# kaistmm/Audio-Mamba-AuM

Hardware: AMD Instinct MI355X
Metric: clips/sec/node AuM-Base 128x1024 fwd+bwd (higher is better)
Workload: dtype bf16; 1 GPU; AuM-Base (d_model=768, 24 Fo-Bi blocks, d_state=16, 92.1M params) 128-mel x 1024-frame clips, L=513 tokens, fwd+bwd+Adam, bf16 autocast / fp32 master weights, input = 160000-sample waveforms through the one-launch HIP frontend (log-mel + 16x16 patch embedding + position rows); per_gpu_batch=64, global_batch=64, parallelism=dp1

## Files before the change

### audio-mamba-aum_amd/aum/model.py

```python
import math

import torch
import torch.nn as nn
import torch.nn.functional as F

from mamba_ssm.modules.mamba_simple import Mamba
from mamba_ssm.ops.selective_scan_interface import _autocast_dtype, step_cache
from mamba_ssm.ops.triton.layernorm import RMSNorm, rms_norm_fn

AUM_SIZES = {"base": 768, "small": 384, "tiny": 192}


class PatchEmbed(nn.Module):

    def __init__(self, patch_size, strides, in_chans, embed_dim):
        super().__init__()
        self.proj = nn.Conv2d(in_chans, embed_dim, kernel_size=patch_size, stride=strides)
        fan_in = in_chans * patch_size[0] * patch_size[1]
        nn.init.trunc_normal_(self.proj.weight, std=math.sqrt(1.0 / fan_in) / 0.87962566103423978)
        nn.init.zeros_(self.proj.bias)

    def forward(self, x):
        Bsz, C, Fd, Td = x.shape
        ph, pw = self.proj.kernel_size
        nf, nt = Fd // ph, Td // pw
        cols = x[:, :, :nf * ph, :nt * pw].reshape(Bsz, C, nf, ph, nt, pw).permute(0, 2, 4, 1, 3, 5)
        cols = cols.reshape(Bsz * nf * nt, C * ph * pw)
        out = F.linear(cols, self.proj.weight.reshape(self.proj.out_channels, -1), self.proj.bias)
        return out.reshape(Bsz, nf * nt, -1)


class FrontendTokensFn(torch.autograd.Function):

    @staticmethod
    def forward(ctx, wave, weight, bias, pos_embed, cls_token, fe, dtype, cls_pos, time_major):
        import aum_hip
        Dm = weight.shape[0]
        w16 = weight.detach().reshape(Dm, -1).to(dtype).contiguous()
        pe = pos_embed.detach().float()
        cls_row = (cls_token.detach().float() + pe[:, :1]).reshape(Dm).contiguous()
        need = any(ctx.needs_input_grad[1:5])
        tokens, patches = aum_hip.frontend_tokens(
            wave, fe.tables.tables, fe.target_length, fe.norm_mean, fe.norm_std, w16, bias.detach().float().contiguous(),
            pe[0, 1:].contiguous(), cls_row, cls_pos, time_major=time_major, save_patches=need, aug=fe.aug, noise=fe.noise)
        ctx.save_for_backward(patches)
        ctx.cfg = (weight.shape, weight.dtype, dtype, cls_pos, time_major, fe.target_length // 16)
        return tokens

    @staticmethod
    def backward(ctx, g):
        (patches,) = ctx.saved_tensors
        wshape, wdtype, dtype, cls_pos, time_major, nt = ctx.cfg
        Bsz, _, Dm = g.shape
        gp = torch.cat((g[:, :cls_pos], g[:, cls_pos + 1:]), dim=1)
        if time_major:
            gp = gp.reshape(Bsz, nt, -1, Dm).transpose(1, 2).reshape(Bsz, -1, Dm)
        g16 = gp.to(dtype).reshape(-1, Dm)
        import aum_hip
        if g16.is_cuda and aum_hip.gemm_wgrad_supported(g16, patches):
            dweight = aum_hip.gemm_wgrad(g16, patches).to(wdtype).reshape(wshape)
        else:
            dweight = (g16.t() @ patches).to(wdtype).reshape(wshape)
        dbias = g16.sum(0).to(wdtype)
        dcls = g[:, cls_pos].sum(0)
        dpos = torch.cat((dcls[None], gp.sum(0)), dim=0)[None]
        return None, dweight, dbias, dpos.to(wdtype), dcls.reshape(1, 1, Dm).to(wdtype), None, None, None, None


class PosEmbed(nn.Module):

    def __init__(self, n_tokens, embed_dim):
        super().__init__()
        self.pos_embed = nn.Parameter(torch.zeros(1, n_tokens, embed_dim))
        nn.init.trunc_normal_(self.pos_embed, std=0.02)


class Block(nn.Module):

    def __init__(self, dim, mixer, eps):
        super().__init__()
        self.mixer = mixer
        self.norm = RMSNorm(dim, eps=eps)

    def forward(self, hidden_states, residual=None, inference_params=None, *, time_reversed=False):
        hidden_states, residual = rms_norm_fn(hidden_states, self.norm.weight, self.norm.bias, residual=residual,
                                              prenorm=True, residual_in_fp32=True, eps=self.norm.eps)
        if time_reversed:
            return self.mixer(hidden_states, inference_params=inference_params, time_reversed=True), residual
        return self.mixer(hidden_states, inference_params=inference_params), residual


class ParkedSessions:
    WAVE_KEYS = ("tail_len", "samples", "frames", "ended")

    def __init__(self, blob, columns, wave, signature):
        self.blob, self.columns, self.wave, self.signature = blob, list(columns), wave, tuple(signature)

    def __len__(self):
        return len(self.columns)

    def select(self, idx):
        idx = [int(i) for i in idx]
        if not idx or min(idx) < -len(self) or max(idx) >= len(self):
            raise IndexError(f"ParkedSessions.select: {idx} of {len(self)} sessions")
        idx = [i % len(self) for i in idx]
        if len(set(idx)) == 1:
            blob = self.blob[idx[0]:idx[0] + 1].expand(len(idx), -1)
        else:
            blob = self.blob.index_select(0, torch.tensor(idx, dtype=torch.int64).to(self.blob.device))
        wave = None if self.wave is None else {k: [v[i] for i in idx] for k, v in self.wave.items()}
        return ParkedSessions(blob, [self.columns[i] for i in idx], wave, self.signature)

    def __getitem__(self, i):
        return self.select([i])


class StreamStack:
    MAX_TOTAL = 512

    def __init__(self, model, dtype):
        import aum_hip
        self.dtype, self.depth = dtype, len(model.layers)
        self.sources = [(d, n, p, None if p is None else (p._version, p.dtype, p.device)) for d, n, p in model._stack_sources()]
        self.gens = [(layer.mixer.__dict__, layer.mixer.__dict__.get("_stream_gen", 0)) for layer in model.layers]
        m0 = model.layers[0].mixer
        self.d_model, self.dim, self.eps = m0.d_model, m0.d_inner, model.layers[0].norm.eps
        self.plans, self.keep, recs = [], [], []
        for layer in model.layers:
            mx = layer.mixer
            plan = mx.stream_params(dtype)
            w_in = aum_hip._al16(mx.in_proj.weight.detach().to(dtype).contiguous())
            w_out = aum_hip._al16(mx.out_proj.weight.detach().to(dtype).contiguous())
            nw = aum_hip._al16(aum_hip._f32c(layer.norm.weight))
            self.plans.append(plan)
            self.keep.append((w_in, w_out, nw))
            recs.append({"norm_weight": nw, "w_in": w_in, "conv_weight": plan.conv_w, "conv_bias": plan.conv_b, "wx": plan.w_x, "wdt": plan.w_dt,
                         "A": plan.A, "D": plan.D, "delta_bias": plan.dt_bias, "w_out": w_out, "conv_state": None, "state": None})
        p0 = self.plans[0]
        self.rank, self.ncols, self.ldwx, self.ldwdt = p0.w_dt.shape[1], p0.w_x.shape[0], p0.w_x.stride(0), p0.w_dt.stride(0)
        self.table = aum_hip.stream_layers_table(recs)
        self.records_ok = aum_hip.stream_layers_records_ok(self.table, self.depth)
        self.workspace = None

    def fresh(self):
        for d, n, p, sig in self.sources:
            q = d.get(n)
            if q is not p or (p is not None and (p._version, p.dtype, p.device) != sig):
                return False
        return all(d.get("_stream_gen", 0) == g for d, g in self.gens)

    def takes(self, total, max_len):
        import aum_hip
        return 1 <= max_len <= aum_hip.STREAM_BLOCK_MAX_T and 1 <= total <= self.MAX_TOTAL

    def pools_ok(self, layer_caches):
        if len(layer_caches) != self.depth:
            return False
        n = layer_caches[0][0].shape[0]
        return all(c.dtype == torch.float32 and s.dtype == torch.float32 and c.is_contiguous() and s.is_contiguous()
                   and tuple(c.shape) == (n, self.dim, 4) and tuple(s.shape) == (n, self.dim, 16) and c.data_ptr() % 16 == 0 and s.data_ptr() % 16 == 0
                   for c, s in (layer_caches[i] for i in range(self.depth)))

    def run(self, rows, layer_caches, smap, commit=True, peek=False):
        import aum_hip
        rows = rows.to(self.dtype).contiguous()
        for i in range(self.depth):
            self.table[i].conv_state, self.table[i].state = layer_caches[i][0].data_ptr(), layer_caches[i][1].data_ptr()
        need = aum_hip.stream_layers_scratch_layout(rows.shape[0], self.d_model, self.dim, self.ncols)[2]
        if self.workspace is None or self.workspace.numel() < need or self.workspace.device != rows.device:
            self.workspace = torch.empty(need, dtype=torch.uint8, device=rows.device)
        return aum_hip.stream_layers(rows, self.table, self.depth, layer_caches[0][0], smap, dim=self.dim, rank=self.rank, ncols=self.ncols,
                                     ldwx=self.ldwx, ldwdt=self.ldwdt, eps=self.eps, commit=commit, peek=peek, workspace=self.workspace,
                                     records_ok=self.records_ok)


class AudioMamba(nn.Module):
    def __init__(self, spectrogram_size=(128, 1024), patch_size=(16, 16), strides=(16, 16), depth=24, embed_dim=768,
                 channels=1, num_classes=527, norm_epsilon=1e-5, bimamba_type="v1", if_devide_out=True,
                 use_middle_cls_token=True, use_end_cls_token=False, transpose_token_sequence=False,
                 if_bidirectional=False, ssm_cfg=None, device=None, dtype=None, imagenet_pretrain=False,
                 imagenet_pretrain_path=None, imagenet_pretrain_modelkey="model", imagenet_load_middle_cls_token=True,
                 imagenet_load_double_cls_token=False, **unsupported):
        super().__init__()
        on = {k: v for k, v in unsupported.items() if v not in (None, False, 0, 0.0, -1.0)
              and k not in ("if_cls_token", "rms_norm", "fused_add_norm", "residual_in_fp32", "if_abs_pos_embed", "final_pool_type",
                            "use_PI_for_patch_embed")}
        if imagenet_load_double_cls_token:
            on["imagenet_load_double_cls_token"] = imagenet_load_double_cls_token
        if on:
            raise NotImplementedError(f"AudioMamba options outside the accelerated path: {sorted(on)}")
        if tuple(patch_size) != tuple(strides):
            raise NotImplementedError("overlapping patches are off the default path")
        self.embed_dim = self.d_model = embed_dim
        self.num_classes = num_classes
        self.use_middle_cls_token = use_middle_cls_token
        self.use_end_cls_token = use_end_cls_token
        self.transpose_token_sequence = transpose_token_sequence
        self.if_bidirectional = if_bidirectional
        if if_bidirectional and depth % 2:
            raise ValueError("if_bidirectional pairs the layers: depth must be even")
        fdim = (spectrogram_size[0] - patch_size[0]) // strides[0] + 1
        tdim = (spectrogram_size[1] - patch_size[1]) // strides[1] + 1
        self.patch_grid_size = (fdim, tdim)
        self.num_patches = fdim * tdim
        self.num_tokens = 1
        self.cls_token = nn.Parameter(torch.zeros(1, 1, embed_dim))
        self.head = nn.Linear(embed_dim, num_classes) if num_classes > 0 else nn.Identity()
        self.layers = nn.ModuleList([
            Block(embed_dim, Mamba(embed_dim, layer_idx=i, bimamba_type=bimamba_type, if_devide_out=if_devide_out,
                                   **(ssm_cfg or {})), norm_epsilon)
            for i in range(depth)])
        self.norm_f = RMSNorm(embed_dim, eps=norm_epsilon)
        if isinstance(self.head, nn.Linear):
            nn.init.trunc_normal_(self.head.weight, std=0.02)
            nn.init.zeros_(self.head.bias)
        nn.init.trunc_normal_(self.cls_token, std=0.02)
        self.apply(lambda m: _init_weights(m, depth))
        self.patch_embed = PatchEmbed(tuple(patch_size), tuple(strides), channels, embed_dim)
        self.pos_embed = PosEmbed(self.num_patches + self.num_tokens, embed_dim)
        if imagenet_pretrain:
            from .checkpoint import load_imagenet_checkpoint
            print(load_imagenet_checkpoint(self, imagenet_pretrain_path, imagenet_pretrain_modelkey,
                                           imagenet_load_middle_cls_token, imagenet_load_double_cls_token))
        if device is not None or dtype is not None:
            self.to(device=device, dtype=dtype)

    def no_weight_decay(self):
        return {"pos_embed", "cls_token"}

    def tokens(self, x):
        x = x.unsqueeze(1).transpose(2, 3)
        x = self.patch_embed(x)
        Bsz, Np, _ = x.shape
        pe = self.pos_embed.pos_embed
        pos = Np // 2 if self.use_middle_cls_token else (Np if self.use_end_cls_token else 0)
        cls = (self.cls_token + pe[:, :1]).expand(Bsz, -1, -1)
        x = x + pe[:, 1:]
        if self.transpose_token_sequence:
            nf, nt = self.patch_grid_size
            x = x.reshape(Bsz, nf, nt, -1).transpose(1, 2).reshape(Bsz, nt * nf, -1)
        return torch.cat((x[:, :pos], cls.to(x.dtype), x[:, pos:]), dim=1), pos

    def tokens_from_wave(self, wave, fe):
        import aum_hip
        dtype = torch.get_autocast_dtype(wave.device.type) if torch.is_autocast_enabled(wave.device.type) else None
        ps = self.patch_embed.proj
        if (dtype is None or tuple(ps.kernel_size) != (16, 16) or ps.in_channels != 1 or self.patch_grid_size[0] != 8
                or self.patch_grid_size[1] * 16 != fe.target_length
                or not aum_hip.frontend_tokens_supported(fe.tables.tables, fe.target_length, self.embed_dim, dtype)):
            return self.tokens(fe.spectrogram(wave))
        Np = self.num_patches
        pos = Np // 2 if self.use_middle_cls_token else (Np if self.use_end_cls_token else 0)
        tok = FrontendTokensFn.apply(wave, ps.weight, ps.bias, self.pos_embed.pos_embed, self.cls_token, fe, dtype, pos,
                                     self.transpose_token_sequence)
        return tok, pos

    def forward_features(self, x, frontend=None):
        hidden, pos = self.tokens(x) if frontend is None else self.tokens_from_wave(x, frontend)
        with step_cache([layer.mixer for layer in self.layers], _autocast_dtype()):
            hidden, residual = self._run_layers(hidden)
        return rms_norm_fn(hidden[:, pos], self.norm_f.weight, self.norm_f.bias, eps=self.norm_f.eps,
                           residual=None if residual is None else residual[:, pos], prenorm=False, residual_in_fp32=True)

    def _run_layers(self, hidden):
        residual = None
        if not self.if_bidirectional:
            for layer in self.layers:
                hidden, residual = layer(hidden, residual)
        else:
            for i in range(len(self.layers) // 2):
                hf, rf = self.layers[2 * i](hidden, residual)
                hb, rb = self.layers[2 * i + 1](hidden, residual, time_reversed=True)
                hidden, residual = hf + hb, rf + rb
        return hidden, residual

    def _check_streamable(self):
        bt = self.layers[0].mixer.bimamba_type if len(self.layers) else "none"
        if bt != "none":
            raise ValueError(f"streaming inference needs bimamba_type='none' (causal blocks), not {bt!r}")
        if self.if_bidirectional:
            raise ValueError("streaming inference needs if_bidirectional=False")
        if self.use_middle_cls_token:
            raise ValueError("streaming inference needs use_middle_cls_token=False (the cls token must close the sequence)")
        if not self.use_end_cls_token:
            raise ValueError("streaming inference needs use_end_cls_token=True (the cls token must close the sequence)")
        if not self.transpose_token_sequence:
            raise ValueError("streaming inference needs transpose_token_sequence=True (time-major token order)")

    def allocate_inference_cache(self, batch_size, max_seqlen=0, dtype=None, **kwargs):
        self._check_streamable()
        dtype = torch.float32 if dtype is None else dtype
        return {"layers": {i: layer.mixer.allocate_inference_cache(batch_size, max_seqlen, dtype=dtype, **kwargs)
                           for i, layer in enumerate(self.layers)},
                "columns": 0, "batch": batch_size}

    def _stack_sources(self):
        out = []
        for layer in self.layers:
            mx = layer.mixer
            for mod, names in ((mx, ("A_log", "D")), (mx.conv1d, ("weight", "bias")), (mx.x_proj, ("weight",)), (mx.dt_proj, ("weight", "bias")),
                               (mx.in_proj, ("weight", "bias")), (mx.out_proj, ("weight", "bias")), (layer.norm, ("weight", "bias"))):
                out += [(mod._parameters, n, mod._parameters.get(n)) for n in names]
        return out

    @torch.no_grad()
    def stream_stack(self, dtype=None):
        import aum_hip
        hit = self.__dict__.get("_stream_stack")
        if hit is not None and (dtype is None or dtype == hit.dtype) and hit.fresh() and (
                dtype is not None or hit.dtype == self.layers[0].mixer.in_proj.weight.dtype):
            return hit
        self._check_streamable()
        if not len(self.layers):
            raise ValueError("stream_stack: the model has no blocks")
        dtype = self.layers[0].mixer.in_proj.weight.dtype if dtype is None else dtype
        if dtype not in (torch.bfloat16, torch.float16):
            raise ValueError(f"stream_stack: the projection kernels run in bf16 or fp16, not {dtype}")
        for i, layer in enumerate(self.layers):
            mx = layer.mixer
            if mx.in_proj.bias is not None or mx.out_proj.bias is not None:
                raise ValueError(f"stream_stack: block {i} has projection biases (bias=True); the projection kernels add none")
            if getattr(layer.norm, "bias", None) is not None:
                raise ValueError(f"stream_stack: block {i}'s norm has a bias")
            if mx.d_conv != 4 or mx.d_state != 16:
                raise ValueError(f"stream_stack: block {i} has d_conv {mx.d_conv}, d_state {mx.d_state}; the middle kernel is built for 4 and 16")
            if (mx.d_model, mx.d_inner) not in aum_hip.STREAM_STACK_WIDTHS:
                raise ValueError(f"stream_stack: block {i} has widths ({mx.d_model}, {mx.d_inner}); the kernels are built for {aum_hip.STREAM_STACK_WIDTHS}")
            if layer.norm.eps != self.layers[0].norm.eps:
                raise ValueError("stream_stack: the blocks' norms differ in eps")
        stack = StreamStack(self, dtype)
        if not aum_hip.xdt_fwd_shape_ok(stack.ncols, stack.dim) or stack.rank % 8 or stack.rank + 32 > stack.ncols:
            raise ValueError(f"stream_stack: dt_rank {self.layers[0].mixer.dt_rank} gives x/dt rows of {stack.ncols} columns, which the middle kernel does not take")
        self.__dict__["_stream_stack"] = stack
        return stack

    def _stack_for(self, stack, hidden, layer_caches, seq_map, prefill, peek_every):
        if stack is None or prefill or peek_every is not None:
            return None
        if not isinstance(stack, StreamStack):
            raise TypeError("stack= takes what AudioMamba.stream_stack() returns")
        stack = self.stream_stack(stack.dtype)
        total = hidden.shape[0] * hidden.shape[1]
        max_len = hidden.shape[1] if seq_map is None else max(seq_map.lens)
        return stack if stack.takes(total, max_len) and stack.pools_ok(layer_caches) else None

    def _stream_layers(self, hidden, layer_caches, seq_map=None, commit=True, peek=False, prefill=False, peek_every=None, stack=None):
        st = self._stack_for(stack, hidden, layer_caches, seq_map, prefill, peek_every)
        if st is not None:
            return self._run_stack(st, hidden, layer_caches, seq_map, commit, peek)
        residual = None
        for i, layer in enumerate(self.layers):
            hidden, residual = rms_norm_fn(hidden, layer.norm.weight, layer.norm.bias, residual=residual, prenorm=True,
                                           residual_in_fp32=True, eps=layer.norm.eps)
            conv_state, ssm_state = layer_caches[i]
            if prefill:
                hidden, _, _ = (layer.mixer.prefill_chunk(hidden, conv_state, ssm_state) if seq_map is None else
                                layer.mixer.prefill_chunk(hidden, conv_state, ssm_state, seq_map=seq_map))
            else:
                hidden, _, _ = layer.mixer.step_chunk(hidden, conv_state, ssm_state, seq_map=seq_map, commit=commit, peek=peek,
                                                      **({} if peek_every is None else {"peek_every": peek_every}))
        return hidden, residual

    @staticmethod
    def _run_stack(st, hidden, layer_caches, seq_map, commit, peek):
        import aum_hip
        batch, T, Dm = hidden.shape
        if seq_map is not None:
            aum_hip.check_seq_map("stream_layers", seq_map, T, layer_caches[0][0].shape[0], hidden.device)
        smap = seq_map if seq_map is not None else aum_hip.fixed_seq_map(batch, T, hidden.device)
        h, r = st.run(hidden.reshape(batch * T, Dm), layer_caches, smap, commit=commit, peek=peek)
        return h.view(batch, T, Dm), r.view(batch, T, Dm)

    def _read_in_place(self, cls, cache, rows):
        import aum_hip
        n = cls.shape[0]
        if cls.device.type != "cuda" or not aum_hip.debug.stream_fused:
            return None
        smap = aum_hip.fixed_seq_map(n, 1, cls.device) if rows is None else aum_hip.seq_map((1,) * n, rows, device=cls.device)
        try:
            hidden, residual = self._stream_layers(cls.reshape(1, n, -1), cache["layers"], smap, commit=False)
        except NotImplementedError:
            return None
        return hidden.reshape(n, 1, -1), residual.reshape(n, 1, -1)

    def allocate_stream_pool(self, sessions, dtype=None):
        if int(sessions) < 1:
            raise ValueError("allocate_stream_pool: at least one session")
        pool = self.allocate_inference_cache(int(sessions), dtype=dtype)
        pool["columns"] = [0] * int(sessions)
        return pool

    @staticmethod
    def _is_pool(cache):
        return isinstance(cache["columns"], list)

    def _check_sessions(self, what, cache, sessions, writes=True):
        if writes and not self._is_pool(cache):
            raise ValueError(f"{what} takes a pool from allocate_stream_pool")
        rows = [int(r) for r in sessions]
        if writes and len(set(rows)) != len(rows):
            raise ValueError(f"{what}: the sessions {rows} are not distinct")
        if rows and (min(rows) < 0 or max(rows) >= cache["batch"]):
            raise ValueError(f"{what}: the sessions {rows} are not all rows of a cache of {cache['batch']}")
        return rows

    def _embed_columns(self, spec4d, cols):
        nf, nt = self.patch_grid_size
        x = self.patch_embed(spec4d)
        Bsz, k = x.shape[0], x.shape[1] // nf
        pe = self.pos_embed.pos_embed[:, 1:].reshape(1, nf, nt, -1)
        pe = pe[:, :, cols] if isinstance(cols, slice) else pe.index_select(2, cols)
        return (x.reshape(Bsz, nf, k, -1) + pe).transpose(1, 2).reshape(Bsz, k * nf, -1)

    def _cls_row(self):
        return self.cls_token + self.pos_embed.pos_embed[:, :1]

    def _head_rows(self, hidden, residual, return_features):
        f = rms_norm_fn(hidden, self.norm_f.weight, self.norm_f.bias, eps=self.norm_f.eps, residual=residual, prenorm=False,
                        residual_in_fp32=True)
        return f if return_features else self.head(f)

# ... 435 lines not shown
```

### audio-mamba-aum_amd/aum_hip/__init__.py

```python
import ctypes as C
import math
import os
import typing

import torch

_HERE = os.path.dirname(os.path.abspath(__file__))
_SO = os.path.join(_HERE, "libaum_hip.so")

AUM_F32, AUM_BF16, AUM_F16 = 0, 1, 2
SCAN_SOFTPLUS, SCAN_REVERSE, SCAN_GENERIC, SCAN_ROWPAIR, SCAN_ACCUMULATE = 1, 2, 4, 8, 16
SCAN_DELTA_ACTIVATED = 32
XDT_DELTA_SOFTPLUS = 1
CONV_SILU, CONV_REVERSE = 1, 2
_DT = {torch.float32: AUM_F32, torch.bfloat16: AUM_BF16, torch.float16: AUM_F16}
_ERR = {-1: "AUM_E_NULL", -2: "AUM_E_SHAPE", -3: "AUM_E_DTYPE", -4: "AUM_E_UNSUPPORTED", -5: "AUM_E_WORKSPACE",
        -6: "AUM_E_LAUNCH"}

_i64, _i32, _u32, _vp, _fp = C.c_int64, C.c_int32, C.c_uint32, C.c_void_p, C.c_void_p
ABI_VERSION = 13


class _Debug:

# ... 145 lines not shown


SUM_MAX_JOBS = 8


class SumJob(C.Structure):
    _fields_ = [("src", C.c_void_p), ("dst", C.c_void_p), ("outer", C.c_int64), ("inner", C.c_int64), ("tr_cols", C.c_int32), ("reserved", C.c_int32)]


class ConvUpdateArgs(C.Structure):
    _fields_ = [("x", C.c_void_p), ("conv_state", C.c_void_p), ("weight", C.c_void_p), ("bias", C.c_void_p), ("out", C.c_void_p),
                ("batch", C.c_int32), ("dim", C.c_int32), ("width", C.c_int32), ("dtype", C.c_int32), ("flags", C.c_uint32)]


class StateUpdateArgs(C.Structure):
    _fields_ = [("state", C.c_void_p), ("x", C.c_void_p), ("dt", C.c_void_p), ("z", C.c_void_p), ("B", C.c_void_p), ("C", C.c_void_p),
                ("A", C.c_void_p), ("D", C.c_void_p), ("dt_bias", C.c_void_p), ("out", C.c_void_p),
                ("batch", C.c_int32), ("dim", C.c_int32), ("dstate", C.c_int32), ("dtype", C.c_int32), ("flags", C.c_uint32)]


class ConvTmChunkArgs(C.Structure):
    _fields_ = ([(n, _vp) for n in ("x", "conv_state", "weight", "bias", "y")] + [(n, _i64) for n in ("x_bs", "x_ts", "y_bs", "y_ts")]
                + [(n, _i32) for n in ("batch", "dim", "len", "width", "dtype")] + [("flags", _u32)])


class ScanTmChunkArgs(C.Structure):
    _fields_ = ([(n, _vp) for n in ("u", "delta", "z", "B", "C", "A", "D", "delta_bias", "state", "out")]
                + [(n, _i64) for n in ("u_bs", "u_ts", "delta_bs", "delta_ts", "z_bs", "z_ts", "B_bs", "B_ts", "C_bs", "C_ts", "out_bs", "out_ts")]
                + [(n, _i32) for n in ("batch", "dim", "len", "dstate", "dtype")] + [("flags", _u32)])


class ConvTmChunkVarArgs(C.Structure):
    _fields_ = ([(n, _vp) for n in ("x", "conv_state", "weight", "bias", "y", "cu_seqlens", "state_indices")] + [(n, _i64) for n in ("x_ts", "y_ts")]
                + [(n, _i32) for n in ("total", "nseq", "nrows", "dim", "width", "dtype")] + [("flags", _u32)])


class ScanTmChunkVarArgs(C.Structure):
    _fields_ = ([(n, _vp) for n in ("u", "delta", "z", "B", "C", "A", "D", "delta_bias", "state", "out", "cu_seqlens", "state_indices")]
                + [(n, _i64) for n in ("u_ts", "delta_ts", "z_ts", "B_ts", "C_ts", "out_ts")]
                + [(n, _i32) for n in ("total", "nseq", "nrows", "dim", "dstate", "dtype")] + [("flags", _u32)])


class ConvTmChunkPeeksArgs(C.Structure):
    _fields_ = [("base", ConvTmChunkVarArgs), ("peek_every", _i32), ("reserved", _i32)]


class ScanTmChunkPeeksArgs(C.Structure):
    _fields_ = [("base", ScanTmChunkVarArgs), ("peek_every", _i32), ("reserved", _i32)]


class ScanTmPeeksFwdArgs(C.Structure):
    _fields_ = [("base", ScanTmChunkVarArgs), ("ckpt", _vp), ("ckpt_bytes", _i64), ("peek_every", _i32), ("reserved", _i32)]


class ScanTmPeeksBwdArgs(C.Structure):
    _fields_ = ([("base", ScanTmChunkVarArgs)] + [(n, _vp) for n in ("ckpt", "du", "ddelta", "dz", "workspace")]
                + [(n, _i64) for n in ("ckpt_bytes", "workspace_bytes", "du_ts", "ddelta_ts", "dz_ts")] + [("peek_every", _i32), ("reserved", _i32)])


class ConvTmPeeksBwdArgs(C.Structure):
    _fields_ = ([(n, _vp) for n in ("x", "dy", "weight", "bias", "dx", "workspace", "cu_seqlens")]
                + [(n, _i64) for n in ("workspace_bytes", "x_ts", "dy_ts", "dx_ts")]
                + [(n, _i32) for n in ("total", "nseq", "dim", "width", "dtype")] + [("flags", _u32), ("peek_every", _i32), ("reserved", _i32)])


class ConvTmPrefillVarArgs(C.Structure):
    _fields_ = ([(n, _vp) for n in ("x", "conv_state", "weight", "bias", "y", "cu_seqlens", "state_indices")] + [(n, _i64) for n in ("x_ts", "y_ts")]
                + [(n, _i32) for n in ("total", "nseq", "nrows", "dim", "width", "dtype")] + [("flags", _u32), ("max_len", _i32)])


class ScanTmFwdStateVarArgs(C.Structure):
    _fields_ = ([(n, _vp) for n in ("u", "delta", "z", "B", "C", "A", "D", "delta_bias", "state", "out", "cu_seqlens", "state_indices")]
                + [(n, _i64) for n in ("u_ts", "delta_ts", "z_ts", "B_ts", "C_ts", "out_ts")]
                + [(n, _i32) for n in ("total", "nseq", "nrows", "dim", "dstate", "dtype")] + [("flags", _u32)]
                + [(n, _i32) for n in ("range_len", "max_len", "reserved")] + [("carry", _vp), ("carry_bytes", _i64)])


class StreamBlockArgs(C.Structure):
    _fields_ = ([(n, _vp) for n in ("x", "z", "conv_state", "state", "conv_weight", "conv_bias", "wx", "wdt", "A", "D", "delta_bias", "y", "scratch",
                                    "cu_seqlens", "state_indices")]
                + [(n, _i64) for n in ("x_ts", "z_ts", "y_ts", "scratch_bytes")]
                + [(n, _i32) for n in ("total", "nseq", "nrows", "max_len", "dim", "width", "dstate", "rank", "ncols", "ldwx", "ldwdt", "dtype")]
                + [("flags", _u32)])


class DtProjArgs(C.Structure):
    _fields_ = ([(n, _vp) for n in ("x", "w", "out")] + [("ntok", _i64)] + [(n, _i32) for n in ("dim", "rank", "ldx", "ldw", "ldo", "dtype")])


class XdtArgs(C.Structure):
    _fields_ = ([(n, _vp) for n in ("u", "wx", "wdt", "x_dbl", "delta")] + [("ntok", _i64)]
                + [(n, _i32) for n in ("dim", "rank", "ncols", "ldu", "ldwx", "ldwdt", "ldx", "ldd", "dtype")]
                + [("delta_bias", _vp), ("flags", _u32)])


PARK_MAX_TENSORS = 64
PARK_RESTORE = 1


class ParkArgs(C.Structure):
    _fields_ = ([("base", _vp * PARK_MAX_TENSORS)] + [(n, _i64 * PARK_MAX_TENSORS) for n in ("row_stride", "row_bytes", "blob_off")]
                + [("rows", _vp), ("blob", _vp), ("blob_stride", _i64), ("n_tensors", _i32), ("n_sessions", _i32), ("flags", _u32)])


class StreamInArgs(C.Structure):
    _fields_ = ([(n, _vp) for n in ("hidden", "residual_in", "norm_weight", "w_in", "residual_out", "xz")] + [("hidden_ts", _i64), ("xz_ts", _i64)]
                + [(n, _i32) for n in ("total", "d_model", "dim", "ldw", "dtype")] + [("eps", C.c_float)])


class StreamOutArgs(C.Structure):
    _fields_ = ([(n, _vp) for n in ("y", "w_out", "out")] + [("y_ts", _i64), ("out_ts", _i64)]
                + [(n, _i32) for n in ("total", "d_model", "dim", "ldw", "dtype", "reserved")])


STREAM_LAYER_POINTERS = ("norm_weight", "w_in", "conv_weight", "conv_bias", "wx", "wdt", "A", "D", "delta_bias", "w_out", "conv_state", "state")


class StreamLayer(C.Structure):
    _fields_ = [(n, _vp) for n in STREAM_LAYER_POINTERS]


class StreamLayersArgs(C.Structure):
    _fields_ = ([(n, _vp) for n in ("layers", "hidden", "residual_in", "hidden_out", "residual_out", "workspace", "cu_seqlens", "state_indices")]
                + [("hidden_ts", _i64), ("workspace_bytes", _i64)]
                + [(n, _i32) for n in ("depth", "total", "nseq", "nrows", "max_len", "d_model", "dim", "rank", "ncols", "ldwx", "ldwdt", "dtype")]
                + [("flags", _u32), ("eps", C.c_float)])


_SIGNATURES = {name: ([_vp, _vp], C.c_int) for name in (
    "aum_selective_scan_fwd", "aum_selective_scan_bwd", "aum_causal_conv1d_fwd", "aum_causal_conv1d_bwd", "aum_rmsnorm_fwd", "aum_rmsnorm_bwd",
    "aum_fbank_fwd", "aum_frontend_tokens_fwd", "aum_stft_logmel_fwd", "aum_spec_time_warp", "aum_proj_fwd", "aum_proj_bwd_data",
    "aum_proj_bwd_weight", "aum_scan_tm_fwd", "aum_scan_tm_bwd", "aum_scan_tm_seg_fwd", "aum_scan_tm_seg_bwd", "aum_conv1d_tm_fwd",
    "aum_conv1d_tm_bwd", "aum_gemm_tn", "aum_gemm_wgrad", "aum_dtproj_tm_fwd", "aum_xdt_tm_fwd", "aum_xdt_tm_bwd", "aum_causal_conv1d_update",
    "aum_selective_state_update", "aum_conv1d_tm_chunk", "aum_scan_tm_chunk", "aum_conv1d_tm_chunk_var", "aum_scan_tm_chunk_var", "aum_stream_block_tm", "aum_scan_tm_fwd_state",
    "aum_conv1d_tm_prefill_var", "aum_scan_tm_fwd_state_var", "aum_conv1d_tm_chunk_peeks", "aum_scan_tm_chunk_peeks", "aum_fbank_stream_fwd",
    "aum_scan_tm_peeks_fwd_ckpt", "aum_scan_tm_peeks_bwd", "aum_conv1d_tm_peeks_bwd", "aum_stream_park", "aum_stream_in_tm", "aum_stream_out_tm",
    "aum_stream_layers")}
_SIGNATURES.update({
    "aum_abi_version": ([], C.c_int), "aum_scan_max_single_pass_len": ([], C.c_int),
    "aum_selective_scan_workspace_bytes": ([_i32] * 6, _i64), "aum_selective_scan_ckpt_bytes": ([_i32] * 4, _i64),
    "aum_selective_scan_lane_ckpt_bytes": ([_i32] * 5, _i64), "aum_scan_tm_workspace_bytes": ([_i32] * 5, _i64),
    "aum_scan_tm_seg_carry_bytes": ([_i32] * 6, _i64), "aum_scan_tm_seg_workspace_bytes": ([_i32] * 6, _i64),
    "aum_rmsnorm_bwd_partials": ([_i32], C.c_int), "aum_rmsnorm_bwd_partial_rows": ([_i32, _i32, _u32], C.c_int),
    "aum_scan_tm_nck": ([_i32], _i32), "aum_scan_tm_ckpt_rows": ([_i32], _i32), "aum_conv1d_tm_nparts": ([_i32, _i32], _i32),
    "aum_proj_bwd_weight_splits": ([_i32, _i64], C.c_int), "aum_hbm_copy": ([_vp, _vp, _i64, _vp], C.c_int),
    "aum_selftest_wave_scan": ([_vp, _vp, C.c_int, _vp], C.c_int), "aum_selftest_wave_sum32": ([_vp, _vp, _vp], C.c_int),
    "aum_sum_rows": ([_vp, _vp, _i64, _i64, _i64, _i32, _vp], C.c_int), "aum_sum_rows_multi": ([_vp, _i32, _vp], C.c_int),
    "aum_cast_bank": ([_vp, _i32, _i32, _i32, _vp, _vp, _i32, _vp], C.c_int),
    "aum_stream_block_scratch_bytes": ([_i32] * 3, _i64), "aum_stream_block_max_len": ([], _i32),
    "aum_scan_tm_fwd_state_var_carry_bytes": ([_i32] * 4, _i64),
    "aum_scan_tm_peeks_ckpt_bytes": ([_i32] * 4, _i64), "aum_scan_tm_peeks_bwd_workspace_bytes": ([_i32] * 4, _i64),
    "aum_conv1d_tm_peeks_bwd_workspace_bytes": ([_i32] * 3, _i64),
    "aum_stream_layers_scratch_bytes": ([_i32] * 4, _i64),
})
EXPORTS = list(_SIGNATURES)


class Lib:

    def __init__(self, path, host=False):
        if not os.path.exists(path):
            raise ImportError(
                f"{path} not found: the HIP extension is not built.  Run `python audio-mamba-aum_amd/csrc/build.py` "
                "(hipcc, gfx950).  There is no CPU fallback on the product path.")
        self.path, self.host = path, host
        self.c = C.CDLL(path)
        for name, (argtypes, restype) in _SIGNATURES.items():
            fn = getattr(self.c, name)
            fn.argtypes, fn.restype = argtypes, restype
        if self.c.aum_abi_version() != ABI_VERSION:
            raise RuntimeError(f"{path}: ABI version {self.c.aum_abi_version()}, this binding speaks {ABI_VERSION} -- rebuild the library "
                               "(python audio-mamba-aum_amd/csrc/build.py)")
        self.max_single_pass_len = int(self.c.aum_scan_max_single_pass_len())

    def stream(self, t):
        if self.host:
            return None
        return C.c_void_p(torch.cuda.current_stream(t.device).cuda_stream)

    def check_tensor(self, t):
        if t is None:
            return
        if self.host:
            if t.device.type != "cpu":
                raise RuntimeError("lane-array (test) library takes host tensors")
        elif t.device.type != "cuda":
            raise RuntimeError("libaum_hip.so needs device (HIP) tensors; there is no CPU path in the product library")


_product = None


def get():
    global _product
    if _product is None:
        so = _SO
        if os.environ.get("AUM_DEBUG") == "1" and os.environ.get("AUM_HIP_LIB"):
            so = os.environ["AUM_HIP_LIB"]
        _product = Lib(so, host=False)
    return _product


def _chk(rc, what):
    if rc != 0:
        raise RuntimeError(f"{what} failed: {_ERR.get(rc, rc)}")


class LaunchTimer:

    def __init__(self):
        self.enabled = False
        self.only = None
        self.every = 1
        self.records = {}
        self.seen = {}

    def reset(self):
        self.records = {}
        self.seen = {}

    def want(self, name):
        n = self.seen.get(name, 0)
        self.seen[name] = n + 1
        return n % self.every == 0

    def summary(self):
        torch.cuda.synchronize()
        out = {}
        for name, evs in self.records.items():
            ms = [a.elapsed_time(b) for a, b, _ in evs]
            out[name] = {"launches": len(ms), "avg_ms": sum(ms) / max(len(ms), 1), "meta": evs[-1][2] if evs else None}
        return out


timer = LaunchTimer()


def C_byref(s):
    return C.cast(C.byref(s), C.c_void_p)


def _launch(fn, args, stream_tensor, lib, name, meta=None):
    if timer.enabled and not lib.host and (timer.only is None or name in timer.only) and timer.want(name):
        a, b = torch.cuda.Event(enable_timing=True), torch.cuda.Event(enable_timing=True)
        a.record()
        rc = fn(C_byref(args), lib.stream(stream_tensor))
        b.record()
        timer.records.setdefault(name, []).append((a, b, meta))
    else:
        rc = fn(C_byref(args), lib.stream(stream_tensor))
    _chk(rc, name)


def _ptr(t):
    return None if t is None else t.data_ptr()


def _unit(t, name):
    if t is not None and t.stride(-1) != 1 and t.shape[-1] != 1:
        raise RuntimeError(f"{name}: the time axis must be unit-stride (SSI:19-30)")


def _f32c(t):
    return None if t is None else t.detach().to(torch.float32).contiguous()


def _bc3(t):
    if t.dim() == 4:
        if t.shape[1] != 1:
            raise RuntimeError("only one B/C group is supported (G=1), as used by Mamba (SSI:473-493)")
        t = t[:, 0]
    return t


def _alloc(batch, dim, length, dtype, device, dmajor):
    if dmajor:
        return torch.empty((dim, batch, length), dtype=dtype, device=device).permute(1, 0, 2)
    return torch.empty((batch, dim, length), dtype=dtype, device=device)


def scan_ckpt(u, dstate, lib=None):
    lib = lib or get()
    batch, dim, length = u.shape
    if debug.rowpair or debug.no_ckpt:
        return None
    if lib.c.aum_selective_scan_ckpt_bytes(batch, dim, length, dstate) <= 0:
        return None
    return torch.empty((batch, dim, length // 512, dstate), dtype=torch.float32, device=u.device)


def scan_lane_ckpt(u, dstate, bidir, lib=None):
    lib = lib or get()
    batch, dim, length = u.shape
    if debug.rowpair or debug.no_lane_ckpt:
        return None
    if lib.c.aum_selective_scan_lane_ckpt_bytes(batch, dim, length, dstate, int(bool(bidir))) <= 0:
        return None
    return torch.empty((batch, dim, 2 if bidir else 1, dstate, 64), dtype=torch.float32, device=u.device)


def scan_accumulates(u, dstate, lib=None):
    lib = lib or get()
    batch, dim, length = u.shape
    if debug.rowpair or debug.no_accumulate:
        return False
    return lib.c.aum_selective_scan_ckpt_bytes(batch, dim, length, dstate) > 0
# ... 53 lines not shown
    B, C = _bc3(B), _bc3(C)
    for n, t in (("u", u), ("delta", delta), ("z", z), ("B", B), ("C", C), ("dout", dout), ("out_pre", out_pre)):
        _unit(t, n)
        lib.check_tensor(t)
    batch, dim, length = u.shape
    dstate = A.shape[1]
    dev = u.device
    A, A_b, D, delta_bias = _f32c(A), _f32c(A_b), _f32c(D), _f32c(delta_bias)
    acc = accumulate_into
    du = acc["du"] if acc else _alloc(batch, dim, length, u.dtype, dev, dmajor)
    ddelta = acc["ddelta"] if acc else _alloc(batch, dim, length, u.dtype, dev, dmajor)
    dz = None
    if z is not None:
        dz = acc["dz"] if acc else dz_out if dz_out is not None else _alloc(batch, dim, length, u.dtype, dev, dmajor)
        _unit(dz, "dz")
    f32 = dict(dtype=torch.float32, device=dev)
    nA, nBC = dim * dstate, batch * dstate * length
    sizes = [nA, nA if A_b is not None else 0, dim if D is not None and not acc else 0,
             dim if delta_bias is not None and not acc else 0, 0 if acc else nBC, 0 if acc else nBC]
    zbuf = torch.zeros((sum(sizes),), **f32)
    parts = torch.split(zbuf, sizes)
    dA = parts[0].view(dim, dstate)
    dA_b = parts[1].view(dim, dstate) if A_b is not None else None
    dD = parts[2] if D is not None else None
    dbias = parts[3] if delta_bias is not None else None
    dB = parts[4].view(batch, dstate, length) if not acc else None
    dC = parts[5].view(batch, dstate, length) if not acc else None
    if acc:
        assert A_b is None
        dB, dC, dD, dbias = acc["dB"], acc["dC"], acc["dD"], acc["ddelta_bias"]
    ws_bytes = int(lib.c.aum_selective_scan_workspace_bytes(batch, dim, length, dstate, int(A_b is not None), 1))
    ws = torch.empty((max(ws_bytes, 4) // 4,), **f32) if ws_bytes else None
    a = ScanBwdArgs()
    a.u, a.delta, a.z, a.B, a.C, a.dout, a.out_pre = map(_ptr, (u, delta, z, B, C, dout, out_pre))
    a.A, a.A_b, a.D, a.delta_bias = _ptr(A), _ptr(A_b), _ptr(D), _ptr(delta_bias)
    a.du, a.ddelta, a.dz = _ptr(du), _ptr(ddelta), _ptr(dz)
    a.dA, a.dA_b, a.dB, a.dC, a.dD, a.ddelta_bias = map(_ptr, (dA, dA_b, dB, dC, dD, dbias))
    a.workspace, a.workspace_bytes = _ptr(ws), ws_bytes
    if x_ck is not None:
        assert x_ck.dtype == torch.float32 and x_ck.is_contiguous() and x_ck.shape == (batch, dim, length // 512, dstate)
        a.x_ck = _ptr(x_ck)
    if x_lane is not None:
        assert x_lane.dtype == torch.float32 and x_lane.is_contiguous() and x_lane.shape == (batch, dim, 2 if A_b is not None else 1, dstate, 64)
        lib.check_tensor(x_lane)
        a.x_lane = _ptr(x_lane)
    a.u_bs, a.u_ds = u.stride(0), u.stride(1)
    a.delta_bs, a.delta_ds = delta.stride(0), delta.stride(1)
    if z is not None:
        a.z_bs, a.z_ds = z.stride(0), z.stride(1)
        a.out_bs, a.out_ds = out_pre.stride(0), out_pre.stride(1)
        a.dz_bs, a.dz_ds = dz.stride(0), dz.stride(1)
    a.B_bs, a.B_ns, a.C_bs, a.C_ns = B.stride(0), B.stride(1), C.stride(0), C.stride(1)
    a.dout_bs, a.dout_ds = dout.stride(0), dout.stride(1)
    a.du_bs, a.du_ds = du.stride(0), du.stride(1)
    a.ddelta_bs, a.ddelta_ds = ddelta.stride(0), ddelta.stride(1)
    a.dB_bs, a.dB_ns, a.dC_bs, a.dC_ns = dB.stride(0), dB.stride(1), dC.stride(0), dC.stride(1)
    a.batch, a.dim, a.len, a.dstate, a.dtype = batch, dim, length, dstate, _DT[u.dtype]
    a.flags = ((SCAN_SOFTPLUS if delta_softplus else 0) | (SCAN_REVERSE if reverse else 0) | (SCAN_GENERIC if generic else 0)
               | (SCAN_ROWPAIR if rowpair or debug.rowpair else 0)
               | (SCAN_ACCUMULATE if acc else 0)
               | (debug.ablate << 16))
    _launch(lib.c.aum_selective_scan_bwd, a, u, lib, "scan_bwd_bidir" if A_b is not None else "scan_bwd",
            (batch, dim, length, dstate, u.element_size(), True))
    return dict(du=du, ddelta=ddelta, dA=dA, dA_b=dA_b, dB=dB, dC=dC, dD=dD, dz=dz, ddelta_bias=dbias)


SCAN_TM_CK = 8


def scan_tm_supported(dim, dstate):
    return dstate == 16 and dim % 64 == 0


def _tm3(t, name, last):
    if t.dim() != 3 or t.shape[2] != last or (t.stride(2) != 1 and last != 1):
        raise RuntimeError(f"{name}: expected (batch, len, {last}) with the last axis contiguous (token-major)")
    ts = t.stride(1) if t.shape[1] > 1 else last
    bs = t.stride(0) if t.shape[0] > 1 else ts * t.shape[1]
    return bs, ts


def scan_tm_ckpt(batch, length, dim, dstate, bidir, device, lib=None, dtype=torch.float32):
    lib = lib or get()
    nck = int(lib.c.aum_scan_tm_nck(length))
    rows = int(lib.c.aum_scan_tm_ckpt_rows(_DT[dtype])) if dstate == 16 else dstate
    return torch.empty((2 if bidir else 1, batch, max(nck, 1), rows, dim), dtype=torch.float32, device=device)


SCAN_TM_MAX_SEGMENTS = 32


def scan_tm_segments(batch, dim, length, bidir, training=False, nsimd=None, device=None):
    nsimd = 4 * cu_count(device) if nsimd is None else nsimd
    per_dir = batch * (dim // 64)
    waves = per_dir * (2 if bidir else 1)
    if per_dir <= 0 or waves * 2 > nsimd or length < 1024:
        return 1
    want = -(-nsimd * 3 // per_dir)
    seg = min(want, length // 128, SCAN_TM_MAX_SEGMENTS)
    return seg if seg >= 2 else 1


def scan_tm_fwd(u, delta, A, B, C, D=None, z=None, delta_bias=None, delta_softplus=False, reverse=False, A_b=None,
                want_out_pre=False, ckpt=None, out=None, lib=None, segments=1, delta_activated=False):
    lib = lib or get()
    batch, length, dim = u.shape
    dstate = A.shape[1]
    for t in (u, delta, z, B, C):
        lib.check_tensor(t)
    if u.dtype not in _DT or delta.dtype != u.dtype or (z is not None and z.dtype != u.dtype):
        raise RuntimeError("u, delta, z must share one dtype in {fp32, bf16, fp16}")
    if B.dtype != u.dtype or C.dtype != u.dtype:
        raise RuntimeError("B, C must have u's dtype")
    A, A_b, D, delta_bias = _f32c(A), _f32c(A_b), _f32c(D), _f32c(delta_bias)
    a = ScanTmFwdArgs()
    a.u_bs, a.u_ts = _tm3(u, "u", dim)
    a.delta_bs, a.delta_ts = _tm3(delta, "delta", dim)
    if z is not None:
        a.z_bs, a.z_ts = _tm3(z, "z", dim)
    a.B_bs, a.B_ts = _tm3(B, "B", dstate)
    a.C_bs, a.C_ts = _tm3(C, "C", dstate)
    if out is None:
        out = torch.empty((batch, length, dim), dtype=u.dtype, device=u.device)
    out_pre = torch.empty((batch, length, dim), dtype=u.dtype, device=u.device) if want_out_pre else None
    a.out_bs, a.out_ts = _tm3(out, "out", dim)
    if out_pre is not None:
        a.pre_bs, a.pre_ts = _tm3(out_pre, "out_pre", dim)
    a.u, a.delta, a.z, a.B, a.C = _ptr(u), _ptr(delta), _ptr(z), _ptr(B), _ptr(C)
    a.A, a.A_b, a.D, a.delta_bias = _ptr(A), _ptr(A_b), _ptr(D), _ptr(delta_bias)
    a.out, a.out_pre = _ptr(out), _ptr(out_pre)
    if ckpt is not None:
        assert ckpt.dtype == torch.float32 and ckpt.is_contiguous()
        rows = int(lib.c.aum_scan_tm_ckpt_rows(_DT[u.dtype])) if dstate == 16 else dstate
        assert ckpt.numel() >= (2 if A_b is not None else 1) * batch * max(int(lib.c.aum_scan_tm_nck(length)), 1) * rows * dim, "ckpt too small"
        lib.check_tensor(ckpt)
        a.ckpt = _ptr(ckpt)
    a.batch, a.dim, a.len, a.dstate, a.dtype = batch, dim, length, dstate, _DT[u.dtype]
    a.flags = (SCAN_SOFTPLUS if delta_softplus else 0) | (SCAN_REVERSE if reverse else 0) | (SCAN_DELTA_ACTIVATED if delta_activated else 0)
    if segments > 1:
        sa = ScanTmSegFwdArgs()
        sa.base = a
        sa.segments = int(segments)
        sa.carry_bytes = int(lib.c.aum_scan_tm_seg_carry_bytes(batch, dim, length, dstate, int(A_b is not None), int(segments)))
        if sa.carry_bytes <= 0:
            raise RuntimeError(f"scan_tm_fwd: segments={segments} not supported for this shape")
        carry = torch.empty((sa.carry_bytes // 4,), dtype=torch.float32, device=u.device)
        sa.carry = _ptr(carry)
        _launch(lib.c.aum_scan_tm_seg_fwd, sa, u, lib, "scan_tm_seg_fwd_bidir" if A_b is not None else "scan_tm_seg_fwd",
                (batch, dim, length, dstate, u.element_size(), want_out_pre, int(segments)))
        return out, out_pre
    _launch(lib.c.aum_scan_tm_fwd, a, u, lib, "scan_tm_fwd_bidir" if A_b is not None else "scan_tm_fwd",
            (batch, dim, length, dstate, u.element_size(), want_out_pre))
    return out, out_pre


def scan_state_supported(t, batch, dim, dstate):
    return t is None or (t.dim() == 3 and tuple(t.shape) == (batch, dim, dstate) and t.dtype == torch.float32 and t.is_contiguous()
                         and t.data_ptr() % 16 == 0)


def scan_tm_fwd_state_supported(u, delta, A, B, C, D=None, z=None, delta_bias=None, delta_softplus=False, delta_activated=False,
                                state_in=None, state_out=None, segments=1):
    if u.dim() != 3 or A.dim() != 2 or u.shape[1] < 1 or not scan_tm_supported(u.shape[2], A.shape[1]) or u.dtype not in _DT:
        return False
    batch, length, dim = u.shape
    dstate, es = A.shape[1], u.element_size()
    if not (1 <= int(segments) <= SCAN_TM_MAX_SEGMENTS) or A.shape[0] != dim:
        return False
    for t, last in ((u, dim), (delta, dim), (z, dim), (B, dstate), (C, dstate)):
        if t is None:
            continue
        if t.dtype != u.dtype or t.dim() != 3 or tuple(t.shape) != (batch, length, last) or (t.stride(2) != 1 and last != 1):
            return False
        bs, ts = _tm3(t, "operand", last)
        if last == dim and (t.data_ptr() % 16 or (ts * es) % 16 or (bs * es) % 16):
            return False
        if last == dstate and es == 2 and (t.data_ptr() % 4 or ts % 2 or bs % 2):
            return False
        if ts < 0 or ts * es * length >= 2 ** 31:
            return False
    if delta_activated and (es == 4 or z is None):
        return False
    return scan_state_supported(state_in, batch, dim, dstate) and scan_state_supported(state_out, batch, dim, dstate)


def scan_tm_fwd_state(u, delta, A, B, C, D=None, z=None, delta_bias=None, delta_softplus=False, delta_activated=False, state_in=None,
                      state_out=None, segments=1, out=None, lib=None):
    lib = lib or get()
    for t in (u, delta, z, B, C, state_in, state_out, out):
        lib.check_tensor(t)
    if not scan_tm_fwd_state_supported(u, delta, A, B, C, D, z, delta_bias, delta_softplus, delta_activated, state_in, state_out, segments):
        raise RuntimeError(f"scan_tm_fwd_state: unsupported operands u {tuple(u.shape)} {u.dtype} strides {u.stride()}, A {tuple(A.shape)}, state_in "
                           f"{None if state_in is None else (tuple(state_in.shape), state_in.dtype)}, state_out "
                           f"{None if state_out is None else (tuple(state_out.shape), state_out.dtype)}, segments {segments} "
                           "(need token-major 16-byte rows of one dtype, dim % 64 == 0, dstate 16, fp32 contiguous (batch, dim, 16) states)")
    batch, length, dim = u.shape
    dstate = A.shape[1]
    A, D, delta_bias = _f32c(A), _f32c(D), _f32c(delta_bias)
    for t in (A, D, delta_bias):
        lib.check_tensor(t)
    if out is None:
        out = torch.empty((batch, length, dim), dtype=u.dtype, device=u.device)
    if out.dtype != u.dtype or tuple(out.shape) != (batch, length, dim):
        raise RuntimeError("scan_tm_fwd_state: out must have u's shape and dtype")
    sa = ScanTmFwdStateArgs()
    a = sa.base
    a.u_bs, a.u_ts = _tm3(u, "u", dim)
    a.delta_bs, a.delta_ts = _tm3(delta, "delta", dim)
    if z is not None:
        a.z_bs, a.z_ts = _tm3(z, "z", dim)
    a.B_bs, a.B_ts = _tm3(B, "B", dstate)
    a.C_bs, a.C_ts = _tm3(C, "C", dstate)
    a.out_bs, a.out_ts = _tm3(out, "out", dim)
    a.u, a.delta, a.z, a.B, a.C = _ptr(u), _ptr(delta), _ptr(z), _ptr(B), _ptr(C)
    a.A, a.D, a.delta_bias, a.out = _ptr(A), _ptr(D), _ptr(delta_bias), _ptr(out)
    a.batch, a.dim, a.len, a.dstate, a.dtype = batch, dim, length, dstate, _DT[u.dtype]
    a.flags = (SCAN_SOFTPLUS if delta_softplus else 0) | (SCAN_DELTA_ACTIVATED if delta_activated else 0)
    sa.state_in, sa.state_out, sa.segments = _ptr(state_in), _ptr(state_out), int(segments)
    carry = None
    if segments > 1:
        sa.carry_bytes = int(lib.c.aum_scan_tm_seg_carry_bytes(batch, dim, length, dstate, 0, int(segments)))
        carry = torch.empty((sa.carry_bytes // 4,), dtype=torch.float32, device=u.device)
        sa.carry = _ptr(carry)
    _launch(lib.c.aum_scan_tm_fwd_state, sa, u, lib, "scan_tm_fwd_state", (batch, dim, length, dstate, u.element_size(), int(segments)))
    return out


def scan_tm_bwd(u, delta, A, B, C, D, z, delta_bias, dout, out_pre, ckpt, delta_softplus=False, reverse=False, A_b=None, dz_out=None,
                lib=None, segments=1, want_dA_xA=False, param_out=None, delta_activated=False):
    lib = lib or get()
    batch, length, dim = u.shape
    dstate = A.shape[1]
    dev = u.device
    for t in (u, delta, z, B, C, dout, out_pre, ckpt):
        lib.check_tensor(t)
    if u.dtype not in _DT:
        raise RuntimeError("u must be fp32, bf16 or fp16")
    for name, t in (("delta", delta), ("z", z), ("B", B), ("C", C), ("dout", dout), ("out_pre", out_pre), ("dz_out", dz_out)):
        if t is not None and t.dtype != u.dtype:
            raise RuntimeError(f"{name} must have u's dtype ({u.dtype}), got {t.dtype}")
    for name, t in (("delta", delta), ("z", z), ("dout", dout), ("out_pre", out_pre), ("dz_out", dz_out)):
        if t is not None and tuple(t.shape) != (batch, length, dim):
            raise RuntimeError(f"{name}: expected shape {(batch, length, dim)}, got {tuple(t.shape)}")
    if z is not None and out_pre is None:
        raise RuntimeError("out_pre (the forward's pre-gate sum) is required when z is given")
    A, A_b, D, delta_bias = _f32c(A), _f32c(A_b), _f32c(D), _f32c(delta_bias)
    bidir = A_b is not None
    if ckpt is None or ckpt.dtype != torch.float32 or not ckpt.is_contiguous():
        raise RuntimeError("ckpt: the contiguous fp32 tensor scan_tm_fwd filled")
    rows_ = int(lib.c.aum_scan_tm_ckpt_rows(_DT[u.dtype])) if dstate == 16 else dstate
    if ckpt.numel() < (2 if bidir else 1) * batch * max(int(lib.c.aum_scan_tm_nck(length)), 1) * rows_ * dim:
        raise RuntimeError("ckpt too small for this launch")
    du = torch.empty((batch, length, dim), dtype=u.dtype, device=dev)
    ddelta = torch.empty((batch, length, dim), dtype=u.dtype, device=dev)
    dz = None
    if z is not None:
        dz = dz_out if dz_out is not None else torch.empty((batch, length, dim), dtype=u.dtype, device=dev)
    f32 = dict(dtype=torch.float32, device=dev)
    dBC = torch.empty((batch, length, 2 * dstate), **f32)
    po = param_out or {}
    dA = torch.empty((dim, dstate), **f32)
    dA_b = torch.empty((dim, dstate), **f32) if bidir else None
    dD = _sum_out(po.get("dD"), (dim,), dev) if D is not None else None
    dbias = _sum_out(po.get("ddelta_bias"), (dim,), dev) if delta_bias is not None else None
    dA_xA = _sum_out(po.get("dA_xA"), (dim, dstate), dev) if want_dA_xA else None
    dA_b_xA = _sum_out(po.get("dA_b_xA"), (dim, dstate), dev) if want_dA_xA and bidir else None
    if segments > 1:
        ws_bytes = int(lib.c.aum_scan_tm_seg_workspace_bytes(batch, dim, length, dstate, int(bidir), int(segments)))
        if ws_bytes <= 0:
            raise RuntimeError(f"scan_tm_bwd: segments={segments} not supported for this shape")
    else:
        ws_bytes = int(lib.c.aum_scan_tm_workspace_bytes(batch, dim, length, dstate, int(bidir)))
    ws = torch.empty((max(ws_bytes, 4) // 4,), **f32)
    a = ScanTmBwdArgs()
    a.u, a.delta, a.z, a.B, a.C, a.dout, a.out_pre = map(_ptr, (u, delta, z, B, C, dout, out_pre))
    a.A, a.A_b, a.D, a.delta_bias, a.ckpt = _ptr(A), _ptr(A_b), _ptr(D), _ptr(delta_bias), _ptr(ckpt)
    a.du, a.ddelta, a.dz = _ptr(du), _ptr(ddelta), _ptr(dz)
    a.dA, a.dA_b, a.dBC, a.dD, a.ddelta_bias = map(_ptr, (dA, dA_b, dBC, dD, dbias))
    a.dA_xA, a.dA_b_xA = _ptr(dA_xA), _ptr(dA_b_xA)
    a.workspace, a.workspace_bytes = _ptr(ws), ws_bytes
    a.u_bs, a.u_ts = _tm3(u, "u", dim)
    a.delta_bs, a.delta_ts = _tm3(delta, "delta", dim)
    a.B_bs, a.B_ts = _tm3(B, "B", dstate)
    a.C_bs, a.C_ts = _tm3(C, "C", dstate)
    a.dout_bs, a.dout_ts = _tm3(dout, "dout", dim)
    a.du_bs, a.du_ts = _tm3(du, "du", dim)
    a.ddelta_bs, a.ddelta_ts = _tm3(ddelta, "ddelta", dim)
    if z is not None:
        a.z_bs, a.z_ts = _tm3(z, "z", dim)
        a.pre_bs, a.pre_ts = _tm3(out_pre, "out_pre", dim)
        a.dz_bs, a.dz_ts = _tm3(dz, "dz", dim)
    a.batch, a.dim, a.len, a.dstate, a.dtype = batch, dim, length, dstate, _DT[u.dtype]
    a.flags = (SCAN_SOFTPLUS if delta_softplus else 0) | (SCAN_REVERSE if reverse else 0) | (SCAN_DELTA_ACTIVATED if delta_activated else 0)
    if segments > 1:
        sa = ScanTmSegBwdArgs()
        sa.base = a
        sa.segments = int(segments)
        _launch(lib.c.aum_scan_tm_seg_bwd, sa, u, lib, "scan_tm_seg_bwd_bidir" if bidir else "scan_tm_seg_bwd",
                (batch, dim, length, dstate, u.element_size(), True, int(segments)))
    else:
        _launch(lib.c.aum_scan_tm_bwd, a, u, lib, "scan_tm_bwd_bidir" if bidir else "scan_tm_bwd", (batch, dim, length, dstate, u.element_size(), True))
    return dict(du=du, ddelta=ddelta, dz=dz, dBC=dBC, dA=dA, dA_b=dA_b, dD=dD, ddelta_bias=dbias, dA_xA=dA_xA, dA_b_xA=dA_b_xA, _ws=ws)


GEMM_BN, GEMM_BK = 256, 64

# ... 1773 lines not shown
```

### audio-mamba-aum_amd/csrc/aum_api_tm.inc

```
#include "scan_tm_kernels.h"
#include "conv_tm_kernels.h"
#include "stream_tm_kernels.h"
#include "stream_train_kernels.h"
#include "stream_block_kernels.h"
#include "stream_prefill_kernels.h"

namespace aum {

#ifndef AUM_SCANT_FWD_MINW
#define AUM_SCANT_FWD_MINW 3
#endif

int scan_tm_fwd_f32(const AumScanTmFwdArgs& a, aum_stream_t s);
int scan_tm_fwd_bf16(const AumScanTmFwdArgs& a, aum_stream_t s);
int scan_tm_fwd_f16(const AumScanTmFwdArgs& a, aum_stream_t s);
int scan_tm_bwd_f32(const AumScanTmBwdArgs& a, const ScanTBwdOut& wo, aum_stream_t s);
int scan_tm_bwd_bf16(const AumScanTmBwdArgs& a, const ScanTBwdOut& wo, aum_stream_t s);
int scan_tm_bwd_f16(const AumScanTmBwdArgs& a, const ScanTBwdOut& wo, aum_stream_t s);
int scan_tm_seg_fwd_f32(const AumScanTmFwdArgs& a, const ScanTSeg& sg, int phase, aum_stream_t s);
int scan_tm_seg_fwd_bf16(const AumScanTmFwdArgs& a, const ScanTSeg& sg, int phase, aum_stream_t s);
int scan_tm_seg_fwd_f16(const AumScanTmFwdArgs& a, const ScanTSeg& sg, int phase, aum_stream_t s);
int scan_tm_fwd_state_f32(const AumScanTmFwdArgs& a, const ScanTState& st, const ScanTSeg* sg, int phase, aum_stream_t s);
int scan_tm_fwd_state_bf16(const AumScanTmFwdArgs& a, const ScanTState& st, const ScanTSeg* sg, int phase, aum_stream_t s);
int scan_tm_fwd_state_f16(const AumScanTmFwdArgs& a, const ScanTState& st, const ScanTSeg* sg, int phase, aum_stream_t s);
int scan_tm_fwd_state_var_f32(const AumScanTmFwdArgs& a, const ScanTVar& v, const ScanTSeg* sg, int phase, aum_stream_t s);
int scan_tm_fwd_state_var_bf16(const AumScanTmFwdArgs& a, const ScanTVar& v, const ScanTSeg* sg, int phase, aum_stream_t s);
int scan_tm_fwd_state_var_f16(const AumScanTmFwdArgs& a, const ScanTVar& v, const ScanTSeg* sg, int phase, aum_stream_t s);
int scan_tm_seg_bwd_f32(const AumScanTmBwdArgs& a, const ScanTBwdOut& wo, const ScanTSeg& sg, int phase, aum_stream_t s);
int scan_tm_seg_bwd_bf16(const AumScanTmBwdArgs& a, const ScanTBwdOut& wo, const ScanTSeg& sg, int phase, aum_stream_t s);
int scan_tm_seg_bwd_f16(const AumScanTmBwdArgs& a, const ScanTBwdOut& wo, const ScanTSeg& sg, int phase, aum_stream_t s);

struct ScanTWs { int64_t dbc, dA, dD, dbias, carry, total, trace; int nparts, ndir; };
static ScanTWs scant_ws_layout(int batch, int dim, int len, int dstate, bool bidir, int nseg = 1) {
    ScanTWs w;
    w.ndir = bidir ? 2 : 1;
    w.nparts = dim / WAVE * w.ndir;
    w.dbc = 0;
    w.dA = w.dbc + (int64_t)batch * len * w.nparts * 2 * dstate;
    w.dD = w.dA + (int64_t)w.ndir * batch * nseg * dstate * dim;
    w.dbias = w.dD + (int64_t)w.ndir * batch * nseg * dim;
    w.carry = w.dbias + (int64_t)w.ndir * batch * nseg * dim;
    if (nseg > 1) w.total = w.carry + scant_seg_carry_floats(batch, dim, nseg, bidir);
    else w.total = w.carry + (bidir ? (int64_t)scant_bwd_wgs<true>(batch * (dim / WAVE)) * 2 * (2 * dstate + 2) * WAVE : 0);
    w.trace = 0;
#ifdef AUM_SCANT_TRACE
    w.trace = (w.total + 1) / 2 * 2;
    w.total = w.trace + (int64_t)(bidir ? scant_bwd_wgs<true>(batch * (dim / WAVE)) : scant_bwd_wgs<false>(batch * (dim / WAVE))) * SCANT_NW * 16 * 2;
#endif
    return w;
}

template <class T> using ScanTFwdLds = Lds<float, SCANT_NW * scant_lds_wave_floats<T>()>;
template <class T> using ScanTBwdLds = Lds<float, SCANT_NW * scant_bwd_lds_wave_floats<T>()>;
#if AUM_API_PART == 5 || AUM_API_PART == 0
#ifndef AUM_EMU
template <class T, bool SP, bool HAS_Z, bool HAS_PRE, bool BIDIR>
__global__ __launch_bounds__(SCANT_NW * 64, AUM_SCANT_FWD_MINW) void k_scant_fwd(AumScanTmFwdArgs a) {
    __shared__ __attribute__((aligned(16))) float lds[ScanTFwdLds<T>::n];
#ifdef AUM_SCANT_TRACE
    unsigned long long* tr = reinterpret_cast<unsigned long long*>(a.ckpt) + ((size_t)blockIdx.x * SCANT_NW + threadIdx.x / 64) * 12;
    const unsigned long long t_begin = __builtin_amdgcn_s_memrealtime();
    a.ckpt = nullptr;
    unsigned long long tacc[8] = {0, 0, 0, 0, 0, 0, 0, 0};
    scant_fwd<T, SP, HAS_Z, HAS_PRE, BIDIR>(a, (int)blockIdx.x, lds, tacc);
    if ((threadIdx.x & 63) == 0) {
        tr[0] = __builtin_amdgcn_s_getreg((31 << 11) | 4);
        tr[1] = __builtin_amdgcn_s_getreg((31 << 11) | 20);
        tr[2] = t_begin;
        tr[3] = __builtin_amdgcn_s_memrealtime();
        for (int k = 0; k < 8; ++k) tr[4 + k] = tacc[k];
    }
#else
    scant_fwd<T, SP, HAS_Z, HAS_PRE, BIDIR>(a, (int)blockIdx.x, lds);
#endif
}
#endif
template <class T, bool SP, bool HAS_Z, bool HAS_PRE, bool BIDIR> static int launch_scant_fwd(const AumScanTmFwdArgs& a, aum_stream_t s) {
    constexpr int UPW = scant_units_per_wg<BIDIR>();
    const int grid = (a.batch * (a.dim / WAVE) + UPW - 1) / UPW;
    return AUM_LAUNCH(grid, SCANT_NW * 64, s, (ScanTFwdLds<T>{}), (k_scant_fwd<T, SP, HAS_Z, HAS_PRE, BIDIR>), (scant_fwd<T, SP, HAS_Z, HAS_PRE, BIDIR>(a, wg, lds)), a);
}
template <class T> static int scan_tm_fwd_t(const AumScanTmFwdArgs& a, aum_stream_t s) {
    return with_bool((a.flags & AUM_SCAN_SOFTPLUS) != 0, [&](auto sp) { return with_bool(a.z != nullptr, [&](auto hz) {
        return with_bool(a.out_pre != nullptr, [&](auto pre) { return with_bool(a.A_b != nullptr, [&](auto bidir) {
            return launch_scant_fwd<T, sp, hz, pre, bidir>(a, s); }); }); }); });
}
#ifndef AUM_EMU
template <class T, int PHASE, bool SP, bool HAS_Z, bool HAS_PRE>
__global__ __launch_bounds__(SCANT_NW * 64, AUM_SCANT_FWD_MINW) void k_scant_seg_fwd(AumScanTmFwdArgs a, ScanTSeg sg) {
    __shared__ __attribute__((aligned(16))) float lds[ScanTFwdLds<T>::n];
    scant_seg_fwd<T, PHASE, SP, HAS_Z, HAS_PRE>(a, sg, (int)blockIdx.x, lds);
}
#endif
template <class T, int PHASE, bool SP, bool HAS_Z, bool HAS_PRE> static int launch_scant_seg_fwd(const AumScanTmFwdArgs& a, const ScanTSeg& sg, aum_stream_t s) {
    const int grid = (a.batch * (a.dim / WAVE) * sg.nseg * sg.ndl + SCANT_NW - 1) / SCANT_NW;
    return AUM_LAUNCH(grid, SCANT_NW * 64, s, (ScanTFwdLds<T>{}), (k_scant_seg_fwd<T, PHASE, SP, HAS_Z, HAS_PRE>), (scant_seg_fwd<T, PHASE, SP, HAS_Z, HAS_PRE>(a, sg, wg, lds)), a, sg);
}
template <class T> static int scan_tm_seg_fwd_t(const AumScanTmFwdArgs& a, const ScanTSeg& sg, int phase, aum_stream_t s) {
    return with_bool((a.flags & AUM_SCAN_SOFTPLUS) != 0, [&](auto sp) {
        if (phase == 3) return launch_scant_seg_fwd<T, 3, sp, false, false>(a, sg, s);
        return with_bool(a.z != nullptr, [&](auto hz) {
            if (phase == 4) return launch_scant_seg_fwd<T, 4, sp, hz, false>(a, sg, s);
            return with_bool(a.out_pre != nullptr, [&](auto pre) {
                return with_int<0, 1, 2>(phase, [&](auto ph) { return launch_scant_seg_fwd<T, ph, sp, hz, pre>(a, sg, s); }); });
        });
    });
}
#ifndef AUM_EMU
template <class T, bool SP, bool HAS_Z>
__global__ __launch_bounds__(SCANT_NW * 64, AUM_SCANT_FWD_MINW) void k_scant_fwd_state(AumScanTmFwdArgs a, ScanTState st) {
    __shared__ __attribute__((aligned(16))) float lds[ScanTFwdLds<T>::n];
    scant_fwd_state<T, SP, HAS_Z>(a, st, (int)blockIdx.x, lds);
}
template <class T, int PHASE, bool SP, bool HAS_Z>
__global__ __launch_bounds__(SCANT_NW * 64, AUM_SCANT_FWD_MINW) void k_scant_seg_fwd_state(AumScanTmFwdArgs a, ScanTSeg sg, ScanTState st) {
    __shared__ __attribute__((aligned(16))) float lds[ScanTFwdLds<T>::n];
    scant_seg_fwd_state<T, PHASE, SP, HAS_Z>(a, sg, st, (int)blockIdx.x, lds);
}
#endif
template <class T, bool SP, bool HAS_Z> static int launch_scant_fwd_state(const AumScanTmFwdArgs& a, const ScanTState& st, aum_stream_t s) {
    const int grid = (a.batch * (a.dim / WAVE) + SCANT_NW - 1) / SCANT_NW;
    return AUM_LAUNCH(grid, SCANT_NW * 64, s, (ScanTFwdLds<T>{}), (k_scant_fwd_state<T, SP, HAS_Z>), (scant_fwd_state<T, SP, HAS_Z>(a, st, wg, lds)), a, st);
}
template <class T, int PHASE, bool SP, bool HAS_Z>
static int launch_scant_seg_fwd_state(const AumScanTmFwdArgs& a, const ScanTSeg& sg, const ScanTState& st, aum_stream_t s) {
    const int grid = (a.batch * (a.dim / WAVE) * sg.nseg + SCANT_NW - 1) / SCANT_NW;
    return AUM_LAUNCH(grid, SCANT_NW * 64, s, (ScanTFwdLds<T>{}), (k_scant_seg_fwd_state<T, PHASE, SP, HAS_Z>), (scant_seg_fwd_state<T, PHASE, SP, HAS_Z>(a, sg, st, wg, lds)), a, sg, st);
}
template <class T> static int scan_tm_fwd_state_t(const AumScanTmFwdArgs& a, const ScanTState& st, const ScanTSeg* sg, int phase, aum_stream_t s) {
    if (sg && phase != 3 && phase != 0) return AUM_E_UNSUPPORTED;
    return with_bool((a.flags & AUM_SCAN_SOFTPLUS) != 0, [&](auto sp) {
        if (sg && phase == 3) return launch_scant_seg_fwd_state<T, 3, sp, false>(a, *sg, st, s);
        return with_bool(a.z != nullptr, [&](auto hz) {
            return sg ? launch_scant_seg_fwd_state<T, 0, sp, hz>(a, *sg, st, s) : launch_scant_fwd_state<T, sp, hz>(a, st, s);
        });
    });
}
#ifndef AUM_EMU
template <class T, bool SP, bool HAS_Z>
__global__ __launch_bounds__(SCANT_NW * 64, AUM_SCANT_FWD_MINW) void k_scant_fwd_state_var(AumScanTmFwdArgs a, ScanTVar v) {
    __shared__ __attribute__((aligned(16))) float lds[ScanTFwdLds<T>::n];
    scant_fwd_state_var<T, SP, HAS_Z>(a, v, (int)blockIdx.x, lds);
}
template <class T, int PHASE, bool SP, bool HAS_Z>
__global__ __launch_bounds__(SCANT_NW * 64, AUM_SCANT_FWD_MINW) void k_scant_seg_fwd_state_var(AumScanTmFwdArgs a, ScanTSeg sg, ScanTVar v) {
    __shared__ __attribute__((aligned(16))) float lds[ScanTFwdLds<T>::n];
    scant_seg_fwd_state_var<T, PHASE, SP, HAS_Z>(a, sg, v, (int)blockIdx.x, lds);
}
#endif
template <class T, bool SP, bool HAS_Z> static int launch_scant_fwd_state_var(const AumScanTmFwdArgs& a, const ScanTVar& v, aum_stream_t s) {
    const int grid = (v.nseq * (a.dim / WAVE) + SCANT_NW - 1) / SCANT_NW;
    return AUM_LAUNCH(grid, SCANT_NW * 64, s, (ScanTFwdLds<T>{}), (k_scant_fwd_state_var<T, SP, HAS_Z>), (scant_fwd_state_var<T, SP, HAS_Z>(a, v, wg, lds)), a, v);
}
template <class T, int PHASE, bool SP, bool HAS_Z>
static int launch_scant_seg_fwd_state_var(const AumScanTmFwdArgs& a, const ScanTSeg& sg, const ScanTVar& v, aum_stream_t s) {
    const int grid = (v.nseq * (a.dim / WAVE) * sg.nseg + SCANT_NW - 1) / SCANT_NW;
    return AUM_LAUNCH(grid, SCANT_NW * 64, s, (ScanTFwdLds<T>{}), (k_scant_seg_fwd_state_var<T, PHASE, SP, HAS_Z>), (scant_seg_fwd_state_var<T, PHASE, SP, HAS_Z>(a, sg, v, wg, lds)), a, sg, v);
}
template <class T> static int scan_tm_fwd_state_var_t(const AumScanTmFwdArgs& a, const ScanTVar& v, const ScanTSeg* sg, int phase, aum_stream_t s) {
    if (sg && phase != 3 && phase != 0) return AUM_E_UNSUPPORTED;
    return with_bool((a.flags & AUM_SCAN_SOFTPLUS) != 0, [&](auto sp) {
        if (sg && phase == 3) return launch_scant_seg_fwd_state_var<T, 3, sp, false>(a, *sg, v, s);
        return with_bool(a.z != nullptr, [&](auto hz) {
            return sg ? launch_scant_seg_fwd_state_var<T, 0, sp, hz>(a, *sg, v, s) : launch_scant_fwd_state_var<T, sp, hz>(a, v, s);
        });
    });
}
#if AUM_HAS_DTYPE(0)
int scan_tm_fwd_f32(const AumScanTmFwdArgs& a, aum_stream_t s) { return scan_tm_fwd_t<float>(a, s); }
int scan_tm_seg_fwd_f32(const AumScanTmFwdArgs& a, const ScanTSeg& sg, int phase, aum_stream_t s) { return scan_tm_seg_fwd_t<float>(a, sg, phase, s); }
int scan_tm_fwd_state_f32(const AumScanTmFwdArgs& a, const ScanTState& st, const ScanTSeg* sg, int phase, aum_stream_t s) { return scan_tm_fwd_state_t<float>(a, st, sg, phase, s); }
int scan_tm_fwd_state_var_f32(const AumScanTmFwdArgs& a, const ScanTVar& v, const ScanTSeg* sg, int phase, aum_stream_t s) { return scan_tm_fwd_state_var_t<float>(a, v, sg, phase, s); }
#endif
#if AUM_HAS_DTYPE(1)
int scan_tm_fwd_bf16(const AumScanTmFwdArgs& a, aum_stream_t s) { return scan_tm_fwd_t<bf16_t>(a, s); }
int scan_tm_seg_fwd_bf16(const AumScanTmFwdArgs& a, const ScanTSeg& sg, int phase, aum_stream_t s) { return scan_tm_seg_fwd_t<bf16_t>(a, sg, phase, s); }
int scan_tm_fwd_state_bf16(const AumScanTmFwdArgs& a, const ScanTState& st, const ScanTSeg* sg, int phase, aum_stream_t s) { return scan_tm_fwd_state_t<bf16_t>(a, st, sg, phase, s); }
int scan_tm_fwd_state_var_bf16(const AumScanTmFwdArgs& a, const ScanTVar& v, const ScanTSeg* sg, int phase, aum_stream_t s) { return scan_tm_fwd_state_var_t<bf16_t>(a, v, sg, phase, s); }
#endif
#if AUM_HAS_DTYPE(2)
int scan_tm_fwd_f16(const AumScanTmFwdArgs& a, aum_stream_t s) { return scan_tm_fwd_t<f16_t>(a, s); }
int scan_tm_seg_fwd_f16(const AumScanTmFwdArgs& a, const ScanTSeg& sg, int phase, aum_stream_t s) { return scan_tm_seg_fwd_t<f16_t>(a, sg, phase, s); }
int scan_tm_fwd_state_f16(const AumScanTmFwdArgs& a, const ScanTState& st, const ScanTSeg* sg, int phase, aum_stream_t s) { return scan_tm_fwd_state_t<f16_t>(a, st, sg, phase, s); }
int scan_tm_fwd_state_var_f16(const AumScanTmFwdArgs& a, const ScanTVar& v, const ScanTSeg* sg, int phase, aum_stream_t s) { return scan_tm_fwd_state_var_t<f16_t>(a, v, sg, phase, s); }
#endif
#endif

#ifndef AUM_SCANT_BWD_MINW
#define AUM_SCANT_BWD_MINW 2
#endif
#if AUM_API_PART == 6 || AUM_API_PART == 0
#ifndef AUM_EMU
template <class T, int SP, bool HAS_Z, bool BIDIR>
__global__ __launch_bounds__(SCANT_NW * 64, AUM_SCANT_BWD_MINW) void k_scant_bwd(AumScanTmBwdArgs a, ScanTBwdOut wo) {
    __shared__ __attribute__((aligned(16))) float lds[ScanTBwdLds<T>::n];
#ifdef AUM_SCANT_TRACE
    unsigned long long* tr = wo.trace + ((size_t)blockIdx.x * SCANT_NW + threadIdx.x / 64) * 16;
    const unsigned long long t_begin = __builtin_amdgcn_s_memrealtime();
    unsigned long long tacc[12] = {0, 0, 0, 0, 0, 0, 0, 0, 0, 0, 0, 0};
    scant_bwd<T, SP, HAS_Z, BIDIR>(a, wo, (int)blockIdx.x, lds, tacc);
    if ((threadIdx.x & 63) == 0) {
        tr[0] = __builtin_amdgcn_s_getreg((31 << 11) | 4);
        tr[1] = __builtin_amdgcn_s_getreg((31 << 11) | 20);
        tr[2] = t_begin;
        tr[3] = __builtin_amdgcn_s_memrealtime();
        for (int k = 0; k < 12; ++k) tr[4 + k] = tacc[k];
    }
#else
    scant_bwd<T, SP, HAS_Z, BIDIR>(a, wo, (int)blockIdx.x, lds);
#endif
}
#endif
template <class T, int SP, bool HAS_Z, bool BIDIR> static int launch_scant_bwd(const AumScanTmBwdArgs& a, const ScanTBwdOut& wo, aum_stream_t s) {
    const int grid = scant_bwd_wgs<BIDIR>(a.batch * (a.dim / WAVE));
    return AUM_LAUNCH(grid, SCANT_NW * 64, s, (ScanTBwdLds<T>{}), (k_scant_bwd<T, SP, HAS_Z, BIDIR>), (scant_bwd<T, SP, HAS_Z, BIDIR>(a, wo, wg, lds)), a, wo);
}
template <class T> static int scan_tm_bwd_t(const AumScanTmBwdArgs& a, const ScanTBwdOut& wo, aum_stream_t s) {
    if (a.flags & AUM_SCAN_DELTA_ACTIVATED) {
        if constexpr (sizeof(T) == 2)
            return with_bool(a.A_b != nullptr, [&](auto bidir) { return launch_scant_bwd<T, SCANT_SP_ACT, true, bidir>(a, wo, s); });
        return AUM_E_UNSUPPORTED;
    }
    return with_bool((a.flags & AUM_SCAN_SOFTPLUS) != 0, [&](auto sp) { return with_bool(a.z != nullptr, [&](auto hz) {
        return with_bool(a.A_b != nullptr, [&](auto bidir) { return launch_scant_bwd<T, sp ? SCANT_SP_IN : SCANT_SP_NONE, hz, bidir>(a, wo, s); }); }); });
}
#ifndef AUM_EMU
template <class T, int PHASE, int SP, bool HAS_Z>
__global__ __launch_bounds__(SCANT_NW * 64, AUM_SCANT_BWD_MINW) void k_scant_seg_bwd(AumScanTmBwdArgs a, ScanTBwdOut wo, ScanTSeg sg) {
    __shared__ __attribute__((aligned(16))) float lds[ScanTBwdLds<T>::n];
    scant_seg_bwd<T, PHASE, SP, HAS_Z>(a, wo, sg, (int)blockIdx.x, lds);
}
#endif
template <class T, int PHASE, int SP, bool HAS_Z>
static int launch_scant_seg_bwd(const AumScanTmBwdArgs& a, const ScanTBwdOut& wo, const ScanTSeg& sg, aum_stream_t s) {
    const int grid = (a.batch * (a.dim / WAVE) * sg.nseg + SCANT_NW - 1) / SCANT_NW;
    return AUM_LAUNCH(grid, SCANT_NW * 64, s, (ScanTBwdLds<T>{}), (k_scant_seg_bwd<T, PHASE, SP, HAS_Z>), (scant_seg_bwd<T, PHASE, SP, HAS_Z>(a, wo, sg, wg, lds)), a, wo, sg);
}
template <class T> static int scan_tm_seg_bwd_t(const AumScanTmBwdArgs& a, const ScanTBwdOut& wo, const ScanTSeg& sg, int phase, aum_stream_t s) {
    if (a.flags & AUM_SCAN_DELTA_ACTIVATED) {
        if constexpr (sizeof(T) == 2) return with_int<0, 1, 2>(phase, [&](auto ph) { return launch_scant_seg_bwd<T, ph, SCANT_SP_ACT, true>(a, wo, sg, s); });
        return AUM_E_UNSUPPORTED;
    }
    return with_bool((a.flags & AUM_SCAN_SOFTPLUS) != 0, [&](auto sp) { return with_bool(a.z != nullptr, [&](auto hz) {
        return with_int<0, 1, 2>(phase, [&](auto ph) { return launch_scant_seg_bwd<T, ph, sp ? SCANT_SP_IN : SCANT_SP_NONE, hz>(a, wo, sg, s); }); }); });
}
#if AUM_HAS_DTYPE(0)
int scan_tm_bwd_f32(const AumScanTmBwdArgs& a, const ScanTBwdOut& wo, aum_stream_t s) { return scan_tm_bwd_t<float>(a, wo, s); }
int scan_tm_seg_bwd_f32(const AumScanTmBwdArgs& a, const ScanTBwdOut& wo, const ScanTSeg& sg, int phase, aum_stream_t s) { return scan_tm_seg_bwd_t<float>(a, wo, sg, phase, s); }
#endif
#if AUM_HAS_DTYPE(1)
int scan_tm_bwd_bf16(const AumScanTmBwdArgs& a, const ScanTBwdOut& wo, aum_stream_t s) { return scan_tm_bwd_t<bf16_t>(a, wo, s); }
int scan_tm_seg_bwd_bf16(const AumScanTmBwdArgs& a, const ScanTBwdOut& wo, const ScanTSeg& sg, int phase, aum_stream_t s) { return scan_tm_seg_bwd_t<bf16_t>(a, wo, sg, phase, s); }
#endif
#if AUM_HAS_DTYPE(2)
int scan_tm_bwd_f16(const AumScanTmBwdArgs& a, const ScanTBwdOut& wo, aum_stream_t s) { return scan_tm_bwd_t<f16_t>(a, wo, s); }
int scan_tm_seg_bwd_f16(const AumScanTmBwdArgs& a, const ScanTBwdOut& wo, const ScanTSeg& sg, int phase, aum_stream_t s) { return scan_tm_seg_bwd_t<f16_t>(a, wo, sg, phase, s); }
#endif
#endif

}

#if AUM_API_PART == 3 || AUM_API_PART == 0
AUM_API int32_t aum_scan_tm_nck(int32_t len) { return len > 0 ? scant_nck(len) : 0; }
AUM_API int32_t aum_scan_tm_ckpt_rows(int32_t dtype) {
    return dtype == AUM_F32 ? scant_ck_rows<float>() : (dtype == AUM_BF16 || dtype == AUM_F16) ? scant_ck_rows<bf16_t>() : 0;
}

static bool scan_tm_act_ok(uint32_t flags, int32_t dtype, const void* z) { return !(flags & AUM_SCAN_DELTA_ACTIVATED) || (dtype != AUM_F32 && z); }
template <class A> static A scan_tm_fwd_resolve(const A& a) {
    A r = a;
    if (a.flags & AUM_SCAN_DELTA_ACTIVATED) {
        r.delta_bias = nullptr;
        r.flags &= ~(AUM_SCAN_SOFTPLUS | AUM_SCAN_DELTA_ACTIVATED);
    }
    return r;
}
static int scan_tm_fwd_check(const AumScanTmFwdArgs* a) {
    if (!a) return AUM_E_NULL;
    if (!a->u || !a->delta || !a->B || !a->C || !a->A || !a->out) return AUM_E_NULL;
    if (a->batch <= 0 || a->dim <= 0 || a->len <= 0 || a->dstate <= 0) return AUM_E_SHAPE;
    if (a->dtype < 0 || a->dtype > 2) return AUM_E_DTYPE;
    if (!scant_supported(a->dim, a->dstate)) return AUM_E_UNSUPPORTED;
    if (!scan_tm_act_ok(a->flags, a->dtype, a->z)) return AUM_E_UNSUPPORTED;
    if (a->A_b && (a->flags & AUM_SCAN_REVERSE)) return AUM_E_UNSUPPORTED;
    if (a->dtype != AUM_F32) {
        if ((a->B_bs | a->B_ts | a->C_bs | a->C_ts) & 1) return AUM_E_UNSUPPORTED;
        if ((((uintptr_t)a->B) | ((uintptr_t)a->C)) & 3) return AUM_E_UNSUPPORTED;
    }
    {
        const int64_t es = a->dtype == AUM_F32 ? 4 : 2, lim = ((int64_t)1 << 31) - 1;
        const int64_t ts[] = {a->u_ts, a->delta_ts, a->z ? a->z_ts : 0, a->out_ts, a->out_pre ? a->pre_ts : 0, a->B_ts, a->C_ts};
        for (int64_t t : ts)
            if (t < 0 || t * es * a->len > lim) return AUM_E_UNSUPPORTED;
        if ((int64_t)scant_nck(a->len) * a->dstate * a->dim * 4 > lim) return AUM_E_UNSUPPORTED;
        const uintptr_t ptrs = (uintptr_t)a->u | (uintptr_t)a->delta | (uintptr_t)a->z | (uintptr_t)a->out | (uintptr_t)a->out_pre;
        const int64_t strides = a->u_bs | a->u_ts | a->delta_bs | a->delta_ts | (a->z ? (a->z_bs | a->z_ts) : 0) | a->out_bs | a->out_ts |
                                (a->out_pre ? (a->pre_bs | a->pre_ts) : 0);
        if ((ptrs & 15) || ((strides * es) & 15)) return AUM_E_UNSUPPORTED;
    }
    return AUM_OK;
}
AUM_API int aum_scan_tm_fwd(const AumScanTmFwdArgs* a, void* stream) {
    const int rc = scan_tm_fwd_check(a);
    if (rc != AUM_OK) return rc;
    aum_stream_t s = (aum_stream_t)stream;
    const AumScanTmFwdArgs k = scan_tm_fwd_resolve(*a);
    return AUM_BY_DTYPE_X(k.dtype, scan_tm_fwd, k, s);
}
static int scan_tm_seg_fwd_any(const AumScanTmFwdArgs& a, const ScanTSeg& sg, int phase, aum_stream_t s) {
    return AUM_BY_DTYPE_X(a.dtype, scan_tm_seg_fwd, a, sg, phase, s);
}
AUM_API int64_t aum_scan_tm_seg_carry_bytes(int32_t batch, int32_t dim, int32_t len, int32_t dstate, int32_t bidirectional, int32_t segments) {
    if (batch <= 0 || dim <= 0 || len <= 0 || segments < 2 || !scant_supported(dim, dstate)) return 0;
    return scant_seg_carry_floats(batch, dim, segments, bidirectional != 0) * (int64_t)sizeof(float);
}
AUM_API int aum_scan_tm_seg_fwd(const AumScanTmSegFwdArgs* sa, void* stream) {
    if (!sa) return AUM_E_NULL;
    const AumScanTmFwdArgs* a = &sa->base;
    const int rc = scan_tm_fwd_check(a);
    if (rc != AUM_OK) return rc;
    if (sa->segments < 2 || sa->segments > AUM_SCAN_TM_MAX_SEGMENTS) return AUM_E_SHAPE;
    if (!sa->carry) return AUM_E_NULL;
    const bool bidir = a->A_b != nullptr;
    if (sa->carry_bytes < scant_seg_carry_floats(a->batch, a->dim, sa->segments, bidir) * (int64_t)sizeof(float)) return AUM_E_WORKSPACE;
    aum_stream_t s = (aum_stream_t)stream;
    ScanTSeg sg;
    sg.carry = sa->carry;
    sg.nseg = sa->segments;
    sg.seg_len = scant_seg_len(a->len, sa->segments);
    sg.dir0 = 0;
    sg.ndl = bidir ? 2 : 1;
    const AumScanTmFwdArgs k = scan_tm_fwd_resolve(*a);
    int r = scan_tm_seg_fwd_any(k, sg, 3, s);
    if (r != AUM_OK) return r;
    sg.ndl = 1;
    if (!bidir) return scan_tm_seg_fwd_any(k, sg, 0, s);
    r = scan_tm_seg_fwd_any(k, sg, 1, s);
    if (r != AUM_OK) return r;
    sg.dir0 = 1;
    return scan_tm_seg_fwd_any(k, sg, 2, s);
}
AUM_API int aum_scan_tm_fwd_state(const AumScanTmFwdStateArgs* sa, void* stream) {
    if (!sa) return AUM_E_NULL;
    const AumScanTmFwdArgs* a = &sa->base;
    const int rc = scan_tm_fwd_check(a);
    if (rc != AUM_OK) return rc;
    if (a->A_b || a->ckpt || a->out_pre || (a->flags & AUM_SCAN_REVERSE)) return AUM_E_UNSUPPORTED;
    if ((((uintptr_t)sa->state_in) | ((uintptr_t)sa->state_out)) & 15) return AUM_E_UNSUPPORTED;
    if ((int64_t)a->dim * a->dstate * 4 > (((int64_t)1 << 31) - 1)) return AUM_E_UNSUPPORTED;
    if (sa->segments < 1 || sa->segments > AUM_SCAN_TM_MAX_SEGMENTS) return AUM_E_SHAPE;
    aum_stream_t s = (aum_stream_t)stream;
    const AumScanTmFwdArgs k = scan_tm_fwd_resolve(*a);
    const ScanTState st = {sa->state_in, sa->state_out};
    auto run = [&](const ScanTSeg* sg, int phase) {
        return AUM_BY_DTYPE_X(k.dtype, scan_tm_fwd_state, k, st, sg, phase, s);
    };
    if (sa->segments == 1) return run(nullptr, 0);
    if (!sa->carry) return AUM_E_NULL;
    if (sa->carry_bytes < scant_seg_carry_floats(a->batch, a->dim, sa->segments, false) * (int64_t)sizeof(float)) return AUM_E_WORKSPACE;
    ScanTSeg sg;
    sg.carry = sa->carry;
    sg.nseg = sa->segments;
    sg.seg_len = scant_seg_len(a->len, sa->segments);
    sg.dir0 = 0;
    sg.ndl = 1;
    const int r = run(&sg, 3);
    if (r != AUM_OK) return r;
    return run(&sg, 0);
}
AUM_API int64_t aum_scan_tm_workspace_bytes(int32_t batch, int32_t dim, int32_t len, int32_t dstate, int32_t bidirectional) {
    if (batch <= 0 || dim <= 0 || len <= 0 || dstate <= 0 || !scant_supported(dim, dstate)) return 0;
    return scant_ws_layout(batch, dim, len, dstate, bidirectional != 0).total * (int64_t)sizeof(float);
}

struct ScanTReduceArgs {
    const float* ws;
    float *dBC, *dA, *dA_b, *dD, *dbias;
    const float *A, *A_b;
    float *dAx, *dAx_b;
    int64_t o_dA, o_dD, o_dbias;
    int32_t batch, pbatch, dim, len, dstate, nparts, ndir;
    int32_t nsum;
};
#ifndef AUM_EMU
__global__ __launch_bounds__(256) void k_scant_bwd_reduce(ScanTReduceArgs a) {
    const int64_t ntok = (int64_t)a.batch * a.len;
    const int k4 = 2 * a.dstate / 4;
    const int64_t n_bc = ntok * k4;
    const int64_t n_a = (int64_t)a.ndir * a.dim * a.dstate;
    const int64_t n_d = 2 * (int64_t)a.dim;
    for (int64_t i = (int64_t)blockIdx.x * blockDim.x + threadIdx.x; i < n_bc + n_a + n_d; i += (int64_t)gridDim.x * blockDim.x) {
        if (i < n_bc) {
            const int64_t tok = i / k4;
            const int c = (int)(i % k4);
            const float4* src = reinterpret_cast<const float4*>(a.ws) + (tok * a.nparts) * k4 + c;
            float4 acc = make_float4(0.f, 0.f, 0.f, 0.f);
#pragma unroll 8
            for (int q = 0; q < a.nsum; ++q) {
                const float4 v = src[(int64_t)q * k4];
                acc.x += v.x; acc.y += v.y; acc.z += v.z; acc.w += v.w;
            }
            reinterpret_cast<float4*>(a.dBC)[i] = acc;
        } else if (i < n_bc + n_a) {
            const int64_t r = i - n_bc;
            const int d = (int)(r / ((int64_t)a.dim * a.dstate));
            const int64_t en = r % ((int64_t)a.dim * a.dstate);
            const int e = (int)(en / a.dstate), n = (int)(en % a.dstate);
            const float* src = a.ws + a.o_dA + (int64_t)d * a.pbatch * a.dstate * a.dim + (int64_t)n * a.dim + e;
            float acc = 0.f;
#pragma unroll 16
            for (int b = 0; b < a.pbatch; ++b) acc += src[(int64_t)b * a.dstate * a.dim];
            (d ? a.dA_b : a.dA)[en] = acc;
            float* px = d ? a.dAx_b : a.dAx;
            if (px) px[en] = acc * (d ? a.A_b : a.A)[en];
        } else {
            const int64_t r = i - n_bc - n_a;
            const bool is_bias = r >= a.dim;
            const int e = (int)(r % a.dim);
            float* dst = is_bias ? a.dbias : a.dD;
            if (!dst) continue;
            const float* src = a.ws + (is_bias ? a.o_dbias : a.o_dD) + e;
            float acc = 0.f;
#pragma unroll 16
            for (int q = 0; q < a.ndir * a.pbatch; ++q) acc += src[(int64_t)q * a.dim];
            dst[e] = acc;
        }
    }
}
#endif
#ifdef AUM_EMU
static void scant_reduce_host(const ScanTReduceArgs& a) {
    const int64_t ntok = (int64_t)a.batch * a.len;
    const int K = 2 * a.dstate;
    for (int64_t tok = 0; tok < ntok; ++tok)
        for (int k = 0; k < K; ++k) {
            float acc = 0.f;
            for (int q = 0; q < a.nsum; ++q) acc += a.ws[(tok * a.nparts + q) * K + k];
            a.dBC[tok * K + k] = acc;
        }
    for (int d = 0; d < a.ndir; ++d)
        for (int e = 0; e < a.dim; ++e)
            for (int n = 0; n < a.dstate; ++n) {
                float acc = 0.f;
                for (int b = 0; b < a.pbatch; ++b) acc += a.ws[a.o_dA + (((int64_t)d * a.pbatch + b) * a.dstate + n) * a.dim + e];
                (d ? a.dA_b : a.dA)[(int64_t)e * a.dstate + n] = acc;
                float* px = d ? a.dAx_b : a.dAx;
                if (px) px[(int64_t)e * a.dstate + n] = acc * (d ? a.A_b : a.A)[(int64_t)e * a.dstate + n];
            }
    for (int e = 0; e < a.dim; ++e) {
        float accD = 0.f, accb = 0.f;
        for (int q = 0; q < a.ndir * a.pbatch; ++q) {
            accD += a.ws[a.o_dD + (int64_t)q * a.dim + e];
            accb += a.ws[a.o_dbias + (int64_t)q * a.dim + e];
        }
        if (a.dD) a.dD[e] = accD;
        if (a.dbias) a.dbias[e] = accb;
    }
}
#endif
static int scant_reduce_launch(const ScanTReduceArgs& a, aum_stream_t s) {
// ... 679 lines not shown
```

### audio-mamba-aum_amd/csrc/scan_tm_kernels.h

```cpp
#pragma once
#include "scan_kernels.h"

namespace aum {

#ifndef AUM_SCANT_ABL
#define AUM_SCANT_ABL 0
#endif
#ifndef AUM_SCANT_FWD_PAIRS
#define AUM_SCANT_FWD_PAIRS 1
#endif
constexpr int SCANT_N = 16;
constexpr int SCANT_CK = AUM_SCAN_TM_CK;
constexpr int SCANT_G = SCANT_CK / 2;
AUM_HOSTDEV constexpr int scant_nblocks(int len) { return (len + SCANT_CK - 1) / SCANT_CK; }
AUM_HOSTDEV constexpr int scant_nck(int len) { return scant_nblocks(len + SCANT_CK - 1) - 1; }
#ifdef AUM_SCANT_CK_F32
template <class T> AUM_HOSTDEV constexpr int scant_ck_rows() { return SCANT_N; }
#else
template <class T> AUM_HOSTDEV constexpr int scant_ck_rows() { return sizeof(T) == 2 ? SCANT_N / 2 : SCANT_N; }
#endif
AUM_HOSTDEV bool scant_supported(int dim, int dstate) { return dstate == SCANT_N && dim % WAVE == 0; }

template <bool V> struct ScanTTag { static constexpr bool value = V; };
template <class T> struct ScanTTile {
    static constexpr int ES = (int)sizeof(T);
    static constexpr int ROWB = WAVE * ES;
    static constexpr int NLD = ES / 2;
    static constexpr int FLOATS = SCANT_CK * ROWB / 4;
};
constexpr int SCANT_BC_ROW = 2 * SCANT_N;
constexpr int SCANT_BC_BLOCK = SCANT_CK * SCANT_BC_ROW;
template <class T> AUM_HOSTDEV constexpr int scant_lds_wave_floats() { return 6 * ScanTTile<T>::FLOATS + 2 * SCANT_BC_BLOCK; }

template <class T> struct ScanTStage { vq q[ScanTTile<T>::NLD]; };
struct ScanTRaw { vi u, d, z, part; };

template <class T, int N, int PHASE, bool SP, bool HAS_Z, bool HAS_PRE>
AUM_DEV void scant_fwd_run(const AumScanTmFwdArgs& p, int b, int e0, int dir, int t0, int tstep, int it0, int it1, const float* Aptr,
                           float dmul, vf2 (&x)[N / 2], float* lds, unsigned long long* scant_trace_acc = nullptr, vf2* pacc = nullptr) {
    using TL = ScanTTile<T>;
    constexpr int ES = TL::ES, ROWB = TL::ROWB, NLD = TL::NLD;
    static_assert(N == 16 && SCANT_CK == 8, "lane = (row, chunk) staging below assumes 8 steps x 8 chunks / state pairs");
    constexpr bool CARRY = PHASE >= 3;
    constexpr bool LD_Z = HAS_Z && PHASE != 1 && PHASE != 3, LD_PART = PHASE == 2, ST_PRE = HAS_PRE && PHASE != 1 && !CARRY;
    const int L = p.len;
    const vi lane = lane_id();
    const vi ec = lane + e0;
    vf2 A2[N / 2];
    AUM_UNROLL
    for (int j = 0; j < N / 2; ++j) A2[j] = mk2(gload_u(Aptr, ec * N + 2 * j) * LOG2E, gload_u(Aptr, ec * N + 2 * j + 1) * LOG2E);
    const vf biasv = p.delta_bias ? gload_u(p.delta_bias, ec) : splat(0.f);
    const vf Dv = p.D ? gload_u(p.D, ec) * dmul : splat(0.f);
    const gbuf<T> ubuf = make_gbuf(row_ptr<T>(p.u, (int64_t)b * p.u_bs));
    const gbuf<T> dbuf = make_gbuf(row_ptr<T>(p.delta, (int64_t)b * p.delta_bs));
    const gbuf<T> zbuf = make_gbuf(HAS_Z ? row_ptr<T>(p.z, (int64_t)b * p.z_bs) : row_ptr<T>(p.u, 0));
    const gbuf<T> obuf = make_gbuf(row_ptr<T>(p.out, (int64_t)b * p.out_bs));
    const gbuf<T> pbuf = make_gbuf(HAS_PRE ? row_ptr<T>(p.out_pre, (int64_t)b * p.pre_bs) : row_ptr<T>(p.out, 0));
    const gbuf<T> Bbuf = make_gbuf(row_ptr<T>(p.B, (int64_t)b * p.B_bs));
    const gbuf<T> Cbuf = make_gbuf(row_ptr<T>(p.C, (int64_t)b * p.C_bs));
    const int nck = scant_nck(L);
    const bool want_ck = p.ckpt != nullptr;
    constexpr int CKR = scant_ck_rows<T>();
    const gbuf<float> ckbuf = make_gbuf(want_ck ? p.ckpt + ((int64_t)dir * p.batch + b) * nck * CKR * p.dim : (const float*)Aptr);
    const int u_tb = (int)p.u_ts * ES, d_tb = (int)p.delta_ts * ES, z_tb = HAS_Z ? (int)p.z_ts * ES : 0, o_tb = (int)p.out_ts * ES,
              p_tb = HAS_PRE ? (int)p.pre_ts * ES : 0, B_tb = (int)p.B_ts * ES, C_tb = (int)p.C_ts * ES;
    auto tok = [&](int it) { return t0 + it * tstep; };
    float* t_u = lds;
    float* t_d = lds + TL::FLOATS;
    float* t_z = lds + 2 * TL::FLOATS;
    float* t_p = lds + 3 * TL::FLOATS;
    float* t_o = lds + 4 * TL::FLOATS;
    float* t_pre = lds + 5 * TL::FLOATS;
    float* t_bc = lds + 6 * TL::FLOATS;
    const vi st_r = lane >> 3, st_c = lane & 7;
    const vi st_i = tstep > 0 ? st_r : (SCANT_CK - 1) - st_r;
    const vi st_gcol = st_c * 16 + e0 * ES;
    const vi st_lds = st_i * ROWB + st_c * 16;
    const vi el_off = lane * ES;
    const vi bc_slot = st_i * SCANT_BC_ROW + st_c * 2;
    const vi vo4 = ec * 4;

    struct Next { ScanTStage<T> u, d, z, part; vpair_raw bp, cp; };
    auto request = [&](int blk, Next& n) {
        const int base = blk * SCANT_CK;
        const bool inside = base >= it0 && base + SCANT_CK <= it1;
        vi rowt;
        int t_lo = 0;
        if (inside) {
            t_lo = tstep > 0 ? tok(base) : tok(base + SCANT_CK - 1);
            rowt = st_r;
        } else {
            const vi it = vmax_i(vmin_i(st_i + base, it1 - 1), it0);
            rowt = it * tstep + t0;
        }
        AUM_UNROLL
        for (int i = 0; i < NLD; ++i) {
            const vi col = st_gcol + 128 * i;
            if (!(AUM_SCANT_ABL & 8)) {
                n.u.q[i] = gbuf_load16(ubuf, rowt * u_tb + col, t_lo * u_tb);
                n.d.q[i] = gbuf_load16(dbuf, rowt * d_tb + col, t_lo * d_tb);
                if (LD_Z) n.z.q[i] = gbuf_load16(zbuf, rowt * z_tb + col, t_lo * z_tb);
                if (LD_PART) n.part.q[i] = gbuf_load16(obuf, rowt * o_tb + col, t_lo * o_tb);
            } else {
                AUM_UNROLL
                for (int k = 0; k < 4; ++k) n.u.q[i].w[k] = n.d.q[i].w[k] = n.z.q[i].w[k] = n.part.q[i].w[k] = spl_i(0x3c003c00);
            }
        }
        n.bp = gbuf_load_pair_raw(Bbuf, rowt * B_tb + st_c * (2 * ES), t_lo * B_tb);
        n.cp = gbuf_load_pair_raw(Cbuf, rowt * C_tb + st_c * (2 * ES), t_lo * C_tb);
    };
    auto park = [&](int blk, const Next& n) {
        AUM_UNROLL
        for (int i = 0; i < NLD; ++i) {
            const vi off = st_lds + 128 * i;
            lds_write16(t_u, off, n.u.q[i]);
            lds_write16(t_d, off, n.d.q[i]);
            if (LD_Z) lds_write16(t_z, off, n.z.q[i]);
            if (LD_PART) lds_write16(t_p, off, n.part.q[i]);
        }
        float* bc = t_bc + (blk & 1) * SCANT_BC_BLOCK;
        vf b0, b1, c0, c1;
        pair_raw_to_f32<T>(n.bp, b0, b1);
        pair_raw_to_f32<T>(n.cp, c0, c1);
        if (AUM_SCANT_ABL & 2) b0 = b1 = c0 = c1 = splat(1.f);
        lds_write2(bc, bc_slot, b0, b1);
        lds_write2(bc, bc_slot + N, c0, c1);
        wave_lds_fence();
    };
    auto flush = [&](int blk) {
        if ((AUM_SCANT_ABL & 4) || CARRY) return;
        const int base = blk * SCANT_CK;
        const bool inside = base >= it0 && base + SCANT_CK <= it1;
        wave_lds_fence();
        vi rowt;
        int t_lo = 0;
        vm valid = lane >= 0;
        if (inside) {
            t_lo = tstep > 0 ? tok(base) : tok(base + SCANT_CK - 1);
            rowt = st_r;
        } else {
            const vi it = st_i + base;
            valid = (it >= it0) && (it < it1);
            rowt = vmax_i(vmin_i(it, it1 - 1), it0) * tstep + t0;
        }
        AUM_UNROLL
        for (int i = 0; i < NLD; ++i) {
            const vi off = st_lds + 128 * i, col = st_gcol + 128 * i;
            const vq qo = lds_read16(t_o, off);
            if (inside) {
                gbuf_store16(obuf, rowt * o_tb + col, t_lo * o_tb, qo);
                if (ST_PRE) gbuf_store16(pbuf, rowt * p_tb + col, t_lo * p_tb, lds_read16(t_pre, off));
            } else if (any_lane(valid)) {
                vq qp = qo;
                if (ST_PRE) qp = lds_read16(t_pre, off);
                gbuf_store16_m(obuf, rowt * o_tb + col, 0, qo, valid);
                if (ST_PRE) gbuf_store16_m(pbuf, rowt * p_tb + col, 0, qp, valid);
            }
        }
    };
    auto read_B = [&](const float* bcrow, vf2 (&Bp)[N / 2]) {
        AUM_UNROLL
        for (int k = 0; k < N / 4; ++k) {
            vf q[4];
            if (AUM_SCANT_ABL & 16) q[0] = q[1] = q[2] = q[3] = splat(1.f);
            else lds_read4_u(bcrow, 4 * k, q);
            Bp[2 * k] = mk2(q[0], q[1]);
            Bp[2 * k + 1] = mk2(q[2], q[3]);
        }
    };
    auto read_raw = [&](int s, ScanTRaw& r) {
        const vi off = el_off + s * ROWB;
        if (AUM_SCANT_ABL & 16) {
            r.u = r.d = r.z = r.part = lane + s;
            return;
        }
        r.u = lds_read_raw<T>(t_u, off);
        r.d = lds_read_raw<T>(t_d, off);
        if (LD_Z) r.z = lds_read_raw<T>(t_z, off);
        if (LD_PART) r.part = lds_read_raw<T>(t_p, off);
    };
    auto delta_of = [&](const ScanTRaw& r) {
        vf dl = raw_to_f32<T>(r.d) + biasv;
        if (SP) dl = vsoftplus(dl);
        return dl;
    };
    vf dsum = splat(0.f);
    auto step = [&](int s, const float* bc, bool prefetch, const ScanTRaw& r, vf dl, vf2 (&Bp)[N / 2], ScanTRaw& rn, vf& dln, vf2 (&Bn)[N / 2]) {
        const float* bcrow = bc + s * SCANT_BC_ROW;
        vf2 Cp[N / 2];
        if (!CARRY) {
            AUM_UNROLL
            for (int k = 0; k < N / 4; ++k) {
                vf q[4];
                if (AUM_SCANT_ABL & 16) q[0] = q[1] = q[2] = q[3] = splat(1.f);
                else lds_read4_u(bcrow, N + 4 * k, q);
                Cp[2 * k] = mk2(q[0], q[1]);
                Cp[2 * k + 1] = mk2(q[2], q[3]);
            }
        }
        if (prefetch) {
            read_B(bcrow + SCANT_BC_ROW, Bn);
            read_raw(s + 1, rn);
        }
        AUM_SCHED_FENCE();
        const vf uu = raw_to_f32<T>(r.u);
        const vf du = dl * uu;
        const vf2 dl2 = spl2(dl), du2 = spl2(du);
        vf2 a[N / 2];
        AUM_UNROLL
        for (int j = 0; j < N / 2; ++j) a[j] = dl2 * A2[j];
        if (CARRY) {
            AUM_UNROLL
            for (int j = 0; j < N / 2; ++j) a[j] = vexp2_2(a[j]);
            if (PHASE == 3) {
                AUM_UNROLL
                for (int j = 0; j < N / 2; ++j) x[j] = vfma2(a[j], x[j], du2 * Bp[j]);
            } else {
                vf dy = uu;
                if (LD_Z) {
                    const vf zz = raw_to_f32<T>(r.z);
                    dy = uu * (zz * vsigmoid(zz));
                }
                const vf2 dy2 = spl2(dy);
                AUM_UNROLL
                for (int j = 0; j < N / 2; ++j) x[j] = a[j] * vfma2(dy2, Bp[j], x[j]);
            }
            dsum = dsum + dl;
            if (prefetch) dln = delta_of(rn);
            return;
        }
        vf zz = splat(0.f), ez = splat(0.f);
        if (LD_Z) {
            zz = raw_to_f32<T>(r.z);
            ez = zz * (-LOG2E);
        }
        AUM_UNROLL
        for (int j = 0; j < N / 2; ++j) Bp[j] = du2 * Bp[j];
        if (!(AUM_SCANT_ABL & 1)) {
            AUM_UNROLL
            for (int j = 0; j < N / 2; ++j) a[j] = vexp2_2(a[j]);
        }
        if (LD_Z) ez = vexp2(ez);
        AUM_UNROLL
        for (int j = 0; j < N / 2; ++j) x[j] = vfma2(a[j], x[j], Bp[j]);
        vf sg = splat(1.f);
        if (LD_Z) sg = vrcp(ez + 1.0f);
        vf2 y2[4];
        AUM_UNROLL
        for (int j = 0; j < 4; ++j) y2[j] = x[j] * Cp[j];
        AUM_UNROLL
        for (int j = 4; j < N / 2; ++j) y2[j & 3] = vfma2(x[j], Cp[j], y2[j & 3]);
        if (prefetch) dln = delta_of(rn);
        const vf2 ysum = (y2[0] + y2[1]) + (y2[2] + y2[3]);
        const vf ys = lo2(ysum) + hi2(ysum);
        const vi off = el_off + s * ROWB;
        if (PHASE == 1) {
            if (!(AUM_SCANT_ABL & 32)) lds_write_elem<T>(t_o, off, ys);
            else x[0] = x[0] + spl2(ys * 1e-30f);
            return;
        }
        vf tot = vfma(uu, Dv, ys);
        if (PHASE == 2) tot = tot + raw_to_f32<T>(r.part);
        if (ST_PRE && !(AUM_SCANT_ABL & 32)) lds_write_elem<T>(t_pre, off, tot);
        if (HAS_Z) tot = tot * (zz * sg);
        if (!(AUM_SCANT_ABL & 32)) lds_write_elem<T>(t_o, off, tot);
        else x[0] = x[0] + spl2(tot * 1e-30f);
    };
    auto steps4 = [&](int s0, const float* bc, vf2 (&Bq)[N / 2], bool more_b) {
        vi ru[4], rd[4], rz[4], rp[4];
        AUM_UNROLL
        for (int q = 0; q < 4; ++q) {
            const vi off = el_off + (s0 + q) * ROWB;
            ru[q] = lds_read_raw<T>(t_u, off);
            rd[q] = lds_read_raw<T>(t_d, off);
            if (LD_Z) rz[q] = lds_read_raw<T>(t_z, off);
            if (LD_PART) rp[q] = lds_read_raw<T>(t_p, off);
        }
        vf2 Pd[2], Pu[2], Us[2], G[2];
        const vf2 bias2 = spl2(biasv), Dv2 = spl2(Dv);
        AUM_UNROLL
        for (int i = 0; i < 2; ++i) {
            Us[i] = mk2(raw_to_f32<T>(ru[2 * i]), raw_to_f32<T>(ru[2 * i + 1]));
            vf2 d = mk2(raw_to_f32<T>(rd[2 * i]), raw_to_f32<T>(rd[2 * i + 1])) + bias2;
            if (SP) d = vsoftplus2(d);
            Pd[i] = d;
            Pu[i] = d * Us[i];
            if (LD_Z) {
                const vf2 zz = mk2(raw_to_f32<T>(rz[2 * i]), raw_to_f32<T>(rz[2 * i + 1]));
                G[i] = zz * vsigmoid2(zz);
            }
        }
        vf ys_even = splat(0.f);
        AUM_UNROLL
        for (int q = 0; q < 4; ++q) {
            const int s = s0 + q;
// ... 18 lines not shown
            for (int j = 0; j < N / 2; ++j) Bq[j] = du2 * Bq[j];
            AUM_UNROLL
            for (int j = 0; j < N / 2; ++j) a[j] = vexp2_2(a[j]);
            AUM_UNROLL
            for (int j = 0; j < N / 2; ++j) x[j] = vfma2(a[j], x[j], Bq[j]);
            vf2 y2[4];
            AUM_UNROLL
            for (int j = 0; j < 4; ++j) y2[j] = x[j] * Cp[j];
            AUM_UNROLL
            for (int j = 4; j < N / 2; ++j) y2[j & 3] = vfma2(x[j], Cp[j], y2[j & 3]);
            const vf2 ysum = (y2[0] + y2[1]) + (y2[2] + y2[3]);
            const vf ys = lo2(ysum) + hi2(ysum);
            if (PHASE == 1) {
                lds_write_elem<T>(t_o, el_off + s * ROWB, ys);
            } else if ((q & 1) == 0) {
                ys_even = ys;
            } else {
                const int i = q >> 1;
                const vi off0 = el_off + (s - 1) * ROWB, off1 = el_off + s * ROWB;
                vf2 tot = vfma2(Us[i], Dv2, mk2(ys_even, ys));
                if (PHASE == 2) tot = tot + mk2(raw_to_f32<T>(rp[q - 1]), raw_to_f32<T>(rp[q]));
                if (ST_PRE) {
                    lds_write_elem<T>(t_pre, off0, lo2(tot));
                    lds_write_elem<T>(t_pre, off1, hi2(tot));
                }
                if (HAS_Z) tot = tot * G[i];
                lds_write_elem<T>(t_o, off0, lo2(tot));
                lds_write_elem<T>(t_o, off1, hi2(tot));
            }
            if (pf) {
                AUM_UNROLL
                for (int j = 0; j < N / 2; ++j) Bq[j] = Bn[j];
            }
        }
    };
    auto ckpt_store = [&](int blk) {
        int off = blk * CKR * p.dim * 4;
        if constexpr (CKR == N) {
            AUM_UNROLL
            for (int n = 0; n < N; ++n) {
                gbuf_store(ckbuf, vo4, off, (n & 1) ? hi2(x[n >> 1]) : lo2(x[n >> 1]));
                off += p.dim * 4;
            }
        } else {
            AUM_UNROLL
            for (int j = 0; j < N / 2; ++j) {
                gbuf_store_pair16<T>(ckbuf, vo4, off, lo2(x[j]), hi2(x[j]));
                off += p.dim * 4;
            }
        }
    };

    if (it0 >= it1) return;
    const int blk0 = it0 / SCANT_CK, blk1 = (it1 + SCANT_CK - 1) / SCANT_CK;
#if defined(AUM_SCANT_TRACE) && !defined(AUM_EMU)
#define AUM_TM_STAMP(k) do { const unsigned long long now_ = __builtin_readcyclecounter(); scant_trace_acc[k] += now_ - stamp_; stamp_ = now_; } while (0)
    unsigned long long stamp_ = __builtin_readcyclecounter();
#else
#define AUM_TM_STAMP(k) do { } while (0)
#endif
    Next nx;
    request(blk0, nx);
    park(blk0, nx);
    AUM_TM_STAMP(0);
#ifndef AUM_SCANT_PRIO
#define AUM_SCANT_PRIO 1
#endif
#ifndef AUM_SCANT_PRIO_SHIFT
#define AUM_SCANT_PRIO_SHIFT 0
#endif
#ifndef AUM_SCANT_PRIO_A
#define AUM_SCANT_PRIO_A 2
#endif
#ifndef AUM_SCANT_PRIO_B
#define AUM_SCANT_PRIO_B 1
#endif
    const int wslot = AUM_SCANT_PRIO ? wave_slot_on_simd() : 0;
    for (int blk = blk0; blk < blk1; ++blk) {
        const int base = blk * SCANT_CK;
        const bool more = blk + 1 < blk1;
        if (AUM_SCANT_PRIO) {
            const int turn = ((blk >> AUM_SCANT_PRIO_SHIFT) + wslot) % 3;
            if (turn == 0) AUM_SET_PRIO(AUM_SCANT_PRIO_A);
            else if (turn == 1) AUM_SET_PRIO(AUM_SCANT_PRIO_B);
            else AUM_SET_PRIO(0);
        }
        if (more) request(blk + 1, nx);
        AUM_TM_STAMP(1);
        const float* bc = t_bc + (blk & 1) * SCANT_BC_BLOCK;
        if (base >= it0 && base + SCANT_CK <= it1 && !CARRY && !AUM_SCANT_ABL && AUM_SCANT_FWD_PAIRS) {
            vf2 Bq[N / 2];
            read_B(bc, Bq);
            steps4(0, bc, Bq, true);
            steps4(4, bc, Bq, false);
            if (want_ck && blk < nck) ckpt_store(blk);
        } else if (base >= it0 && base + SCANT_CK <= it1) {
            ScanTRaw r;
            vf2 Bq[N / 2];
            read_raw(0, r);
            read_B(bc, Bq);
            vf dl = delta_of(r);
            AUM_UNROLL
            for (int s = 0; s < SCANT_CK; ++s) {
                ScanTRaw rn;
                vf2 Bn[N / 2];
                vf dln;
                step(s, bc, s + 1 < SCANT_CK, r, dl, Bq, rn, dln, Bn);
                if (s + 1 < SCANT_CK) {
                    r = rn;
                    dl = dln;
                    AUM_UNROLL
                    for (int j = 0; j < N / 2; ++j) Bq[j] = Bn[j];
                }
            }
            if (want_ck && !CARRY && blk < nck && !(AUM_SCANT_ABL & 64) && !((AUM_SCANT_ABL & 128) && (blk & 1) == 0)) ckpt_store(blk);
        } else {
            for (int s = 0; s < SCANT_CK; ++s) {
                if (base + s < it0 || base + s >= it1) continue;
                ScanTRaw r, rn;
                vf2 Bq[N / 2], Bn[N / 2];
                vf dln;
                read_raw(s, r);
                read_B(bc + s * SCANT_BC_ROW, Bq);
                step(s, bc, false, r, delta_of(r), Bq, rn, dln, Bn);
            }
            if (want_ck && !CARRY && blk < nck && base + SCANT_CK - 1 >= it0 && base + SCANT_CK - 1 < it1) ckpt_store(blk);
        }
        AUM_TM_STAMP(2);
        flush(blk);
        AUM_TM_STAMP(3);
        if (more) park(blk + 1, nx);
        AUM_TM_STAMP(4);
    }
#undef AUM_TM_STAMP
    if (CARRY) {
        const vf2 ds2 = spl2(dsum);
        AUM_UNROLL
        for (int j = 0; j < N / 2; ++j) pacc[j] = vexp2_2(ds2 * A2[j]);
    }
}

AUM_HOSTDEV constexpr int scant_first_half(int len, int dir) { return dir == 0 ? len / 2 : len - len / 2; }
#ifndef AUM_SCANT_GRID_SHIFT
#define AUM_SCANT_GRID_SHIFT 1
#endif
AUM_HOSTDEV constexpr int scant_grid_shift(int len, int dir) {
    return AUM_SCANT_GRID_SHIFT && len >= 8 * SCANT_CK ? (SCANT_CK - scant_first_half(len, dir) % SCANT_CK) % SCANT_CK : 0;
}

constexpr int SCANT_NW = 4;
template <bool BIDIR> AUM_HOSTDEV constexpr int scant_units_per_wg() { return BIDIR ? SCANT_NW / 2 : SCANT_NW; }
template <bool BIDIR> AUM_HOSTDEV constexpr int scant_bwd_wgs(int units) { return BIDIR ? (units + 2) / 3 : (units + SCANT_NW - 1) / SCANT_NW; }

template <class T, bool SP, bool HAS_Z, bool HAS_PRE, bool BIDIR>
AUM_DEV void scant_fwd(const AumScanTmFwdArgs& p, int wg, float* lds, unsigned long long* tacc = nullptr) {
    constexpr int N = SCANT_N;
    constexpr int NW = SCANT_NW;
    constexpr int UPW = scant_units_per_wg<BIDIR>();
    const int gpb = p.dim / WAVE;
    const int units = p.batch * gpb;
    const int L = p.len;
    vf2 x[AUM_PER_WAVE(NW)][N / 2];
    if (!BIDIR) {
        const bool rev = (p.flags & AUM_SCAN_REVERSE) != 0;
        AUM_FOR_EACH_WAVE(w, NW) {
            const int unit = wg * UPW + w;
            if (unit < units) {
                AUM_UNROLL
                for (int j = 0; j < N / 2; ++j) x[AUM_W(w)][j] = spl2(splat(0.f));
                scant_fwd_run<T, N, 0, SP, HAS_Z, HAS_PRE>(p, unit / gpb, (unit % gpb) * WAVE, 0, rev ? L - 1 : 0, rev ? -1 : 1, 0, L, p.A, 1.f,
                                                           x[AUM_W(w)], lds + w * scant_lds_wave_floats<T>(), tacc);
            }
        }
        return;
    }
    AUM_FOR_EACH_WAVE(w, NW) {
        const int unit = wg * UPW + (w >> 1), d = w & 1, io = scant_grid_shift(L, d);
        if (unit < units) {
            AUM_UNROLL
            for (int j = 0; j < N / 2; ++j) x[AUM_W(w)][j] = spl2(splat(0.f));
            scant_fwd_run<T, N, 1, SP, HAS_Z, HAS_PRE>(p, unit / gpb, (unit % gpb) * WAVE, d, d ? L - 1 + io : -io, d ? -1 : 1, io, scant_first_half(L, d) + io,
                                                       d ? p.A_b : p.A, 2.f, x[AUM_W(w)], lds + w * scant_lds_wave_floats<T>(), tacc);
        }
    }
    AUM_WG_BARRIER();
    AUM_FOR_EACH_WAVE(w, NW) {
        const int unit = wg * UPW + (w >> 1), d = w & 1, io = scant_grid_shift(L, d);
        if (unit < units)
            scant_fwd_run<T, N, 2, SP, HAS_Z, HAS_PRE>(p, unit / gpb, (unit % gpb) * WAVE, d, d ? L - 1 + io : -io, d ? -1 : 1, scant_first_half(L, d) + io, L + io,
                                                       d ? p.A_b : p.A, 2.f, x[AUM_W(w)], lds + w * scant_lds_wave_floats<T>(), tacc);
    }
}


struct ScanTSeg {
    float* carry;
    int nseg, seg_len;
    int dir0, ndl;
};
AUM_HOSTDEV constexpr int scant_seg_len(int len, int nseg) { return ((len + nseg - 1) / nseg + SCANT_CK - 1) / SCANT_CK * SCANT_CK; }
AUM_HOSTDEV constexpr int64_t scant_seg_carry_floats(int batch, int dim, int nseg, bool bidir) {
    return (int64_t)(bidir ? 2 : 1) * batch * nseg * 2 * SCANT_N * dim;
}

template <class T, int PHASE, bool SP, bool HAS_Z, bool HAS_PRE>
AUM_DEV void scant_seg_fwd(const AumScanTmFwdArgs& p, const ScanTSeg& sg, int wg, float* lds) {
    constexpr int N = SCANT_N;
    constexpr int NW = SCANT_NW;
    const int gpb = p.dim / WAVE;
    const int L = p.len;
    const int items = p.batch * gpb * sg.nseg * sg.ndl;
    const bool bidir = p.A_b != nullptr;
    vf2 x[AUM_PER_WAVE(NW)][N / 2], P[AUM_PER_WAVE(NW)][N / 2];
    AUM_FOR_EACH_WAVE(w, NW) {
        const int item = wg * NW + w;
        const int s = item < items ? (item / sg.ndl) % sg.nseg : 0;
        const bool idle = item >= items || (PHASE == 3 && s == sg.nseg - 1) || (PHASE == 4 && s == 0);
        if (!idle) {
            const int d = sg.dir0 + item % sg.ndl, unit = item / (sg.ndl * sg.nseg);
            const int b = unit / gpb, e0 = (unit % gpb) * WAVE;
            const bool rev = bidir ? d == 1 : (p.flags & AUM_SCAN_REVERSE) != 0;
            const float* Aptr = d ? p.A_b : p.A;
            const int it0 = s * sg.seg_len < L ? s * sg.seg_len : L;
            const int it1 = it0 + sg.seg_len < L ? it0 + sg.seg_len : L;
            const vi ec = lane_id() + e0;
            float* cb = sg.carry + ((int64_t)d * p.batch + b) * sg.nseg * (2 * N) * p.dim;
            float* lw = lds + w * scant_lds_wave_floats<T>();
            AUM_UNROLL
            for (int j = 0; j < N / 2; ++j) x[AUM_W(w)][j] = spl2(splat(0.f));
            if (PHASE >= 3) {
                AUM_UNROLL
                for (int j = 0; j < N / 2; ++j) P[AUM_W(w)][j] = spl2(splat(1.f));
                if (PHASE == 3)
                    scant_fwd_run<T, N, 3, SP, HAS_Z, HAS_PRE>(p, b, e0, d, rev ? L - 1 : 0, rev ? -1 : 1, it0, it1, Aptr, 1.f, x[AUM_W(w)], lw, nullptr,
                                                               P[AUM_W(w)]);
                else
                    scant_fwd_run<T, N, 4, SP, HAS_Z, HAS_PRE>(p, b, e0, d, rev ? 0 : L - 1, rev ? 1 : -1, L - it1, L - it0, Aptr, 1.f, x[AUM_W(w)], lw,
                                                               nullptr, P[AUM_W(w)]);
                float* cs = cb + (int64_t)s * (2 * N) * p.dim;
                AUM_UNROLL
                for (int n = 0; n < N; ++n) {
                    gstore(cs + (int64_t)n * p.dim, ec, (n & 1) ? hi2(P[AUM_W(w)][n >> 1]) : lo2(P[AUM_W(w)][n >> 1]), ec >= 0);
                    gstore(cs + (int64_t)(N + n) * p.dim, ec, (n & 1) ? hi2(x[AUM_W(w)][n >> 1]) : lo2(x[AUM_W(w)][n >> 1]), ec >= 0);
                }
            } else {
                for (int sp = 0; sp < s; ++sp) {
                    const float* cs = cb + (int64_t)sp * (2 * N) * p.dim;
                    AUM_UNROLL
                    for (int j = 0; j < N / 2; ++j) {
                        const vf2 pj = mk2(gload_u(cs + (int64_t)(2 * j) * p.dim, ec), gload_u(cs + (int64_t)(2 * j + 1) * p.dim, ec));
                        const vf2 xj = mk2(gload_u(cs + (int64_t)(N + 2 * j) * p.dim, ec), gload_u(cs + (int64_t)(N + 2 * j + 1) * p.dim, ec));
                        x[AUM_W(w)][j] = vfma2(pj, x[AUM_W(w)][j], xj);
                    }
                }
                scant_fwd_run<T, N, PHASE, SP, HAS_Z, HAS_PRE>(p, b, e0, d, rev ? L - 1 : 0, rev ? -1 : 1, it0, it1, Aptr, bidir ? 2.f : 1.f,
                                                               x[AUM_W(w)], lw);
            }
        }
    }
}

struct ScanTState {
    const float* in;
    float* out;
};
template <int N> AUM_DEV void scant_state_load(const float* row, vi ec, vf2 (&x)[N / 2]) {
    const gbuf<float> sbuf = make_gbuf(row);
    const vi st_off = ec * (N * 4);
    AUM_UNROLL
    for (int i = 0; i < N / 4; ++i) {
        vf t[4];
        vq_unpack<float>(gbuf_load16(sbuf, st_off + 16 * i, 0), t);
        x[2 * i] = mk2(t[0], t[1]);
        x[2 * i + 1] = mk2(t[2], t[3]);
    }
}
template <int N> AUM_DEV void scant_state_store(float* row, vi ec, const vf2 (&x)[N / 2]) {
    const gbuf<float> sbuf = make_gbuf(row);
    const vi st_off = ec * (N * 4);
    AUM_UNROLL
    for (int i = 0; i < N / 4; ++i) {
        const vf t[4] = {lo2(x[2 * i]), hi2(x[2 * i]), lo2(x[2 * i + 1]), hi2(x[2 * i + 1])};
        gbuf_store16(sbuf, st_off + 16 * i, 0, vq_pack<float>(t));
    }
}

template <class T, bool SP, bool HAS_Z>
AUM_DEV void scant_fwd_state(const AumScanTmFwdArgs& p, const ScanTState& st, int wg, float* lds) {
    constexpr int N = SCANT_N;
    constexpr int NW = SCANT_NW;
    const int gpb = p.dim / WAVE;
    const int units = p.batch * gpb;
    vf2 x[AUM_PER_WAVE(NW)][N / 2];
    AUM_FOR_EACH_WAVE(w, NW) {
        const int unit = wg * NW + w;
        if (unit < units) {
            const int b = unit / gpb, e0 = (unit % gpb) * WAVE;
            const vi ec = lane_id() + e0;
            const int64_t row = (int64_t)b * p.dim * N;
            if (st.in) {
                scant_state_load<N>(st.in + row, ec, x[AUM_W(w)]);
            } else {
                AUM_UNROLL
                for (int j = 0; j < N / 2; ++j) x[AUM_W(w)][j] = spl2(splat(0.f));
            }
            scant_fwd_run<T, N, 0, SP, HAS_Z, false>(p, b, e0, 0, 0, 1, 0, p.len, p.A, 1.f, x[AUM_W(w)], lds + w * scant_lds_wave_floats<T>());
            if (st.out) scant_state_store<N>(st.out + row, ec, x[AUM_W(w)]);
        }
    }
}

template <class T, int PHASE, bool SP, bool HAS_Z>
AUM_DEV void scant_seg_fwd_state(const AumScanTmFwdArgs& p, const ScanTSeg& sg, const ScanTState& st, int wg, float* lds) {
    static_assert(PHASE == 0 || PHASE == 3, "carry launch or main launch");
    constexpr int N = SCANT_N;
    constexpr int NW = SCANT_NW;
    const int gpb = p.dim / WAVE;
    const int L = p.len;
    const int items = p.batch * gpb * sg.nseg;
    vf2 x[AUM_PER_WAVE(NW)][N / 2], P[AUM_PER_WAVE(NW)][N / 2];
    AUM_FOR_EACH_WAVE(w, NW) {
        const int item = wg * NW + w;
        if (item < items) {
            const int s = item % sg.nseg, unit = item / sg.nseg;
            const int b = unit / gpb, e0 = (unit % gpb) * WAVE;
            const int it0 = s * sg.seg_len < L ? s * sg.seg_len : L;
            const int it1 = it0 + sg.seg_len < L ? it0 + sg.seg_len : L;
            const vi ec = lane_id() + e0;
            float* cb = sg.carry + (int64_t)b * sg.nseg * (2 * N) * p.dim;
            float* entry = cb + (int64_t)(sg.nseg - 1) * (2 * N) * p.dim + (int64_t)N * p.dim;
            float* lw = lds + w * scant_lds_wave_floats<T>();
            const int64_t row = (int64_t)b * p.dim * N;
            AUM_UNROLL
            for (int j = 0; j < N / 2; ++j) x[AUM_W(w)][j] = spl2(splat(0.f));
            if (PHASE == 3) {
                if (s == sg.nseg - 1) {
                    if (st.in) scant_state_load<N>(st.in + row, ec, x[AUM_W(w)]);
                    AUM_UNROLL
                    for (int n = 0; n < N; ++n)
                        gstore(entry + (int64_t)n * p.dim, ec, (n & 1) ? hi2(x[AUM_W(w)][n >> 1]) : lo2(x[AUM_W(w)][n >> 1]), ec >= 0);
                } else {
                    AUM_UNROLL
                    for (int j = 0; j < N / 2; ++j) P[AUM_W(w)][j] = spl2(splat(1.f));
// ... 616 lines not shown
```

### audio-mamba-aum_amd/mamba_ssm/modules/mamba_simple.py

```python
import collections
import contextlib
import math

import torch
import torch.nn as nn
import torch.nn.functional as F

from mamba_ssm.ops.selective_scan_interface import (InProjFn, bimamba_inner_fn, mamba_inner_fn, mamba_inner_fn_no_out_proj,
                                                    neg_exp, selective_scan_fn)
import mamba_ssm.ops.selective_scan_interface as ssi
from causal_conv1d import causal_conv1d_fn, causal_conv1d_update
from mamba_ssm.ops.triton.selective_state_update import selective_state_update


StreamParams = collections.namedtuple("StreamParams", "conv_w conv_b A D dt_bias w_x w_dt dtype b_off")


class Mamba(nn.Module):
    def __init__(self, d_model, d_state=16, d_conv=4, expand=2, dt_rank="auto", dt_min=0.001, dt_max=0.1,
                 dt_init="random", dt_scale=1.0, dt_init_floor=1e-4, conv_bias=True, bias=False, use_fast_path=True,
                 layer_idx=None, device=None, dtype=None, bimamba_type="none", if_devide_out=False,
                 init_layer_scale=None):
        fk = {"device": device, "dtype": dtype}
        super().__init__()
        self.d_model, self.d_state, self.d_conv, self.expand = d_model, d_state, d_conv, expand
        self.d_inner = int(expand * d_model)
        self.dt_rank = math.ceil(d_model / 16) if dt_rank == "auto" else dt_rank
        self.use_fast_path, self.layer_idx = use_fast_path, layer_idx
        self.bimamba_type, self.if_devide_out = bimamba_type, if_devide_out
        self.init_layer_scale = init_layer_scale
        if init_layer_scale is not None:
            self.gamma = nn.Parameter(init_layer_scale * torch.ones(d_model), requires_grad=True)

        self.in_proj = nn.Linear(d_model, self.d_inner * 2, bias=bias, **fk)
        self.conv1d = nn.Conv1d(self.d_inner, self.d_inner, d_conv, groups=self.d_inner, padding=d_conv - 1,
                                bias=conv_bias, **fk)
        self.activation = "silu"
        self.act = nn.SiLU()
        self.x_proj = nn.Linear(self.d_inner, self.dt_rank + 2 * d_state, bias=False, **fk)
        self.dt_proj = nn.Linear(self.dt_rank, self.d_inner, bias=True, **fk)
        self._init_dt(self.dt_proj, dt_init, dt_scale, dt_min, dt_max, dt_init_floor, fk)
        self.A_log = self._make_A_log(device)
        self.D = nn.Parameter(torch.ones(self.d_inner, device=device))
        self.D._no_weight_decay = True

        if bimamba_type in ("v1", "v2"):
            self.A_b_log = self._make_A_log(device)
        if bimamba_type == "v2":
            self.conv1d_b = nn.Conv1d(self.d_inner, self.d_inner, d_conv, groups=self.d_inner, padding=d_conv - 1,
                                      bias=conv_bias, **fk)
            self.x_proj_b = nn.Linear(self.d_inner, self.dt_rank + 2 * d_state, bias=False, **fk)
            self.dt_proj_b = nn.Linear(self.dt_rank, self.d_inner, bias=True, **fk)
            self.D_b = nn.Parameter(torch.ones(self.d_inner, device=device))
            self.D_b._no_weight_decay = True
        self.out_proj = nn.Linear(self.d_inner, d_model, bias=bias, **fk)

    def _init_dt(self, dt_proj, dt_init, dt_scale, dt_min, dt_max, dt_init_floor, fk):
        std = self.dt_rank ** -0.5 * dt_scale
        if dt_init == "constant":
            nn.init.constant_(dt_proj.weight, std)
        elif dt_init == "random":
            nn.init.uniform_(dt_proj.weight, -std, std)
        else:
            raise NotImplementedError
        dt = torch.exp(torch.rand(self.d_inner, **fk) * (math.log(dt_max) - math.log(dt_min))
                       + math.log(dt_min)).clamp(min=dt_init_floor)
        with torch.no_grad():
            dt_proj.bias.copy_(dt + torch.log(-torch.expm1(-dt)))
        dt_proj.bias._no_reinit = True

    def _make_A_log(self, device):
        A = torch.arange(1, self.d_state + 1, dtype=torch.float32, device=device).repeat(self.d_inner, 1)
        p = nn.Parameter(torch.log(A))
        p._no_weight_decay = True
        return p

    def forward(self, hidden_states, inference_params=None, *, time_reversed=False, peek_every=None):
        if peek_every is not None:
            if inference_params is not None or time_reversed:
                raise ValueError("forward(peek_every=) takes neither inference_params nor time_reversed")
            return self.forward_peeks(hidden_states, peek_every)
        conv_state = ssm_state = None
        if time_reversed and (inference_params is not None or not self.use_fast_path):
            return self.forward(hidden_states.flip([1]), inference_params).flip([1])
        if inference_params is not None:
            if self.bimamba_type != "none":
                raise NotImplementedError("inference caches only make sense for the causal (bimamba_type='none') block")
            conv_state, ssm_state = self._get_states_from_cache(inference_params, hidden_states.shape[0])
            if inference_params.seqlen_offset > 0:
                if hidden_states.dim() == 3 and hidden_states.shape[1] > 1:
                    out, _, _ = self.step_chunk(hidden_states, conv_state, ssm_state)
                else:
                    out, _, _ = self.step(hidden_states, conv_state, ssm_state)
                return out
            if self._prefill_ok(hidden_states, conv_state, ssm_state):
                conv_state.zero_()
                ssm_state.zero_()
                out, _, _ = self.prefill_chunk(hidden_states, conv_state, ssm_state)
                return out if self.init_layer_scale is None else out * self.gamma
        batch, seqlen, _ = hidden_states.shape
        tm = (ssi.TOKEN_MAJOR and self.use_fast_path and inference_params is None
              and not (ssi._REF_DZ_DROP and self.bimamba_type == "v1")
              and ssi.token_major_preferred(batch, self.d_inner, self.bimamba_type != "none", seqlen=seqlen)
              and ssi.token_major_ok(self.d_inner, self.d_state, self.d_conv, self.dt_rank,
                                     torch.get_autocast_dtype("cuda") if torch.is_autocast_enabled("cuda") else hidden_states.dtype))
        if tm:
            xz = ssi.InProjTmFn.apply(self.in_proj.weight, hidden_states.reshape(batch * seqlen, -1))
            xz = xz.view(batch, seqlen, -1).transpose(1, 2)
        else:
            xz = InProjFn.apply(self.in_proj.weight, hidden_states.reshape(batch * seqlen, -1))
            xz = xz.reshape(-1, batch, seqlen).permute(1, 0, 2)
        if self.in_proj.bias is not None:
            xz = xz + self.in_proj.bias.to(xz.dtype)[None, :, None]
        A = neg_exp(self.A_log)
        if self.use_fast_path and inference_params is None:
            if self.bimamba_type == "v1":
                A_b = neg_exp(self.A_b_log)
                out = bimamba_inner_fn(xz, self.conv1d.weight, self.conv1d.bias, self.x_proj.weight,
                                       self.dt_proj.weight, self.out_proj.weight, self.out_proj.bias, A, A_b, None,
                                       None, self.D.float(), delta_bias=self.dt_proj.bias.float(),
                                       delta_softplus=True, reverse=time_reversed)
            elif self.bimamba_type == "v2":
                A_b = neg_exp(self.A_b_log)
                two = tm and xz.is_cuda and ssi.v2_two_streams(tuple(self.parameters()), module=self)
                if two:
                    main = torch.cuda.current_stream(xz.device)
                    s_f, s_b = ssi.side_streams(xz.device)
                    s_f.wait_stream(main)
                    s_b.wait_stream(main)
                    for t_ in (xz, A, A_b):
                        t_.record_stream(s_f)
                        t_.record_stream(s_b)
                with (torch.cuda.stream(s_f) if two else contextlib.nullcontext()):
                    out_f = mamba_inner_fn_no_out_proj(xz, self.conv1d.weight, self.conv1d.bias, self.x_proj.weight,
                                                       self.dt_proj.weight, A, None, None, self.D.float(),
                                                       delta_bias=self.dt_proj.bias.float(), delta_softplus=True,
                                                       reverse=time_reversed)
                with (torch.cuda.stream(s_b) if two else contextlib.nullcontext()):
                    out_b = mamba_inner_fn_no_out_proj(xz, self.conv1d_b.weight, self.conv1d_b.bias,
                                                       self.x_proj_b.weight, self.dt_proj_b.weight, A_b, None, None,
                                                       self.D_b.float(), delta_bias=self.dt_proj_b.bias.float(),
                                                       delta_softplus=True, reverse=not time_reversed)
                if two:
                    main.wait_stream(s_f)
                    main.wait_stream(s_b)
                    out_f.record_stream(main)
                    out_b.record_stream(main)
                y = out_f + out_b
                if self.if_devide_out:
                    y = y / 2
                out = ssi.out_proj_shared(self.out_proj.weight, y, tm)
                if self.out_proj.bias is not None:
                    out = out + self.out_proj.bias.to(out.dtype)
                out = out.reshape(batch, seqlen, -1)
            else:
                out = mamba_inner_fn(xz, self.conv1d.weight, self.conv1d.bias, self.x_proj.weight,
                                     self.dt_proj.weight, self.out_proj.weight, self.out_proj.bias, A, None, None,
                                     self.D.float(), delta_bias=self.dt_proj.bias.float(), delta_softplus=True,
                                     reverse=time_reversed)
        else:
            x, z = xz.chunk(2, dim=1)
            if conv_state is not None:
                conv_state.copy_(F.pad(x, (self.d_conv - x.shape[-1], 0)))
            x = causal_conv1d_fn(x, self.conv1d.weight.reshape(self.d_inner, -1), self.conv1d.bias, self.activation)
            x_dbl = self.x_proj(x.transpose(1, 2).reshape(batch * seqlen, -1))
            dt, Bm, Cm = torch.split(x_dbl, [self.dt_rank, self.d_state, self.d_state], dim=-1)
            dt = (self.dt_proj.weight.to(dt.dtype) @ dt.t()).reshape(-1, batch, seqlen).permute(1, 0, 2)
            Bm = Bm.reshape(batch, seqlen, -1).transpose(1, 2).contiguous()
            Cm = Cm.reshape(batch, seqlen, -1).transpose(1, 2).contiguous()
            y = selective_scan_fn(x, dt.to(x.dtype), A, Bm.to(x.dtype), Cm.to(x.dtype), self.D.float(),
                                  z=z.to(x.dtype), delta_bias=self.dt_proj.bias.float(), delta_softplus=True,
                                  return_last_state=ssm_state is not None)
            if ssm_state is not None:
                y, last_state = y
                ssm_state.copy_(last_state)
            out = self.out_proj(y.transpose(1, 2))
        if self.init_layer_scale is not None:
            out = out * self.gamma
        return out

    def forward_peeks(self, hidden_states, peek_every):
        if self.bimamba_type != "none":
            raise NotImplementedError("forward(peek_every=) needs the causal (bimamba_type='none') block")
        if isinstance(peek_every, bool) or not isinstance(peek_every, int) or peek_every < 1:
            raise ValueError(f"forward: peek_every is the number of committed rows before each peek row, an int >= 1, not {peek_every!r}")
        if hidden_states.dim() != 3 or hidden_states.shape[1] < 1:
            raise ValueError("forward(peek_every=): hidden_states must be (batch, T >= 1, d_model)")
        E, N, R = self.d_inner, self.d_state, self.dt_rank
        xz = self.in_proj(hidden_states)
        x, z = xz[..., :E], xz[..., E:]
        xc = ssi.conv_peeks(x, self.conv1d.weight.reshape(E, self.d_conv), self.conv1d.bias, self.activation, peek_every)
        x_dbl = self.x_proj(xc)
        dt = F.linear(x_dbl[..., :R], self.dt_proj.weight)
        y = ssi.scan_peeks(xc, dt.to(xc.dtype), neg_exp(self.A_log), x_dbl[..., R:R + N].to(xc.dtype), x_dbl[..., R + N:R + 2 * N].to(xc.dtype),
                           self.D.float(), z.to(xc.dtype), self.dt_proj.bias.float(), True, peek_every)
        out = self.out_proj(y)
        return out if self.init_layer_scale is None else out * self.gamma

    def step(self, hidden_states, conv_state, ssm_state):
        if hidden_states.dim() != 3 or hidden_states.shape[1] != 1:
            raise ValueError("step() advances the caches by exactly one token: hidden_states must be (batch, 1, d_model)")
        E, N, R = self.d_inner, self.d_state, self.dt_rank
        x_new, z = self.in_proj(hidden_states[:, 0]).split(E, dim=-1)
        xc = causal_conv1d_update(x_new, conv_state, self.conv1d.weight.view(E, self.d_conv), self.conv1d.bias, self.activation)
        proj = self.x_proj(xc)
        dt_in, B_t, C_t = proj[:, :R], proj[:, R:R + N], proj[:, R + N:R + 2 * N]
        dt = F.linear(dt_in, self.dt_proj.weight)
        y = selective_state_update(ssm_state, xc, dt, -torch.exp(self.A_log.float()), B_t, C_t, self.D, z=z, dt_bias=self.dt_proj.bias,
                                   dt_softplus=True)
        return self.out_proj(y).unsqueeze(1), conv_state, ssm_state

    def _stream_sources(self):
        return (self.conv1d.weight, self.conv1d.bias, self.A_log, self.D, self.dt_proj.bias, self.x_proj.weight, self.dt_proj.weight)

    @torch.no_grad()
    def stream_params(self, dtype=None):
        import aum_hip
        dtype = self.in_proj.weight.dtype if dtype is None else dtype
        key = (dtype,) + tuple(None if p is None else (id(p), p._version, p.dtype, p.device) for p in self._stream_sources())
        hit = self.__dict__.get("_stream_params")
        if hit is not None and hit[0] == key:
            return hit[1]
        E, N, R = self.d_inner, self.d_state, self.dt_rank
        w_x, w_dt, b_off = self.x_proj.weight.detach().to(dtype), self.dt_proj.weight.detach().to(dtype), R
        Rp = -(-R // 8) * 8
        if Rp != R and dtype in (torch.bfloat16, torch.float16) and N == 16 and aum_hip.xdt_fwd_shape_ok(Rp + 2 * N, E):
            px, pdt = w_x.new_zeros(Rp + 2 * N, E), w_dt.new_zeros(E, Rp)
            px[:R], px[Rp:] = w_x[:R], w_x[R:]
            pdt[:, :R] = w_dt
            w_x, w_dt, b_off = px, pdt, Rp
        plan = StreamParams(aum_hip._al16(aum_hip._f32c(self.conv1d.weight.reshape(E, -1))), aum_hip._al16(aum_hip._f32c(self.conv1d.bias)),
                            -torch.exp(self.A_log.float()), aum_hip._f32c(self.D), aum_hip._f32c(self.dt_proj.bias), w_x, w_dt, dtype, b_off)
        self.__dict__["_stream_params"] = (key, plan)
        return plan

    def invalidate_stream_params(self):
        self.__dict__.pop("_stream_params", None)
        self.__dict__["_stream_gen"] = self.__dict__.get("_stream_gen", 0) + 1

    @staticmethod
    def _check_packed(what, hidden_states, conv_state, ssm_state, seq_map):
        import aum_hip
        if hidden_states.dim() != 3 or hidden_states.shape[0] != 1 or conv_state.shape[0] != ssm_state.shape[0]:
            raise ValueError(f"{what}(seq_map=): hidden_states (1, total, d_model), pools of one size, not {conv_state.shape[0]} / {ssm_state.shape[0]} rows")
        aum_hip.check_seq_map(what, seq_map, hidden_states.shape[1], conv_state.shape[0], hidden_states.device)
        return seq_map.total != 0

    def _xdt_stage(self, xc2, plan):
        import aum_hip
        N, R = self.d_state, self.dt_rank
        if xc2.is_cuda and aum_hip.xdt_tm_supported(xc2, plan.w_x, plan.w_dt):
            proj, delta = aum_hip.xdt_tm_fwd(xc2, plan.w_x, plan.w_dt, delta_bias=plan.dt_bias, delta_softplus=True)
            Bo, activated = plan.b_off, True
# ... 141 lines not shown
```

### audio-mamba-aum_amd/mamba_ssm/ops/selective_scan_interface.py

```python
import contextlib
import os

import torch
import torch.nn.functional as F

import aum_hip

_DBG = os.environ.get("AUM_DEBUG") == "1"


def _dbg_env(name, default):
    return os.environ.get(name, default) if _DBG else default


_STEP_CACHE_ON = _dbg_env("AUM_STEP_CACHE", "1") != "0"
_WGRAD_SPLIT_ON = _dbg_env("AUM_WGRAD_SPLIT", "1") != "0"
_REF_DZ_DROP = os.environ.get("AUM_REF_DZ_DROP", "0") == "1"
TOKEN_MAJOR = _dbg_env("AUM_TOKEN_MAJOR", "1") != "0"

_custom_fwd = torch.amp.custom_fwd(device_type="cuda")
_custom_bwd = torch.amp.custom_bwd(device_type="cuda")


def _autocast_dtype():
# ... 830 lines not shown
        ob, out_pre_b, _ = aum_hip.scan_fwd(conv_out, delta, A_b, Bm, Cm, D, z, delta_bias, delta_softplus, True,
                                            want_out_pre=need_bwd, dmajor=True, x_ck=ck_b, accumulate_into=of if acc else None)
        out_z = ob if acc else of + ob
    ctx.delta_softplus, ctx.reverse, ctx.bidir_fused = delta_softplus, reverse, bidir_fused
    ctx.has_out_proj = out_proj_weight is not None
    ctx.out_proj_bias_is_None = out_proj_bias is None
    ctx.B_proj_bias_is_None, ctx.C_proj_bias_is_None = B_proj_bias is None, C_proj_bias is None
    ctx.save_for_backward(xz, conv_w, conv1d_bias, x_dbl, x_proj_weight, delta_proj_weight, out_proj_weight,
                          conv_out, delta, A, A_b, Bm, Cm, D, delta_bias, out_pre, out_pre_b, out_z, ck_f, ck_b,
                          x_proj_wt, delta_proj_wt)
    if out_proj_weight is None:
        return out_z
    out = _mm_tokens_rows(_dm2d(out_z), out_proj_weight.t(), 2)
    if out_proj_bias is not None:
        out = out + out_proj_bias
    return out.reshape(Bsz, L, -1)


def _inner_backward(ctx, dout):
    if ctx.tm:
        return _inner_backward_tm(ctx, dout)
    (xz, conv_w, conv1d_bias, x_dbl, x_proj_weight, delta_proj_weight, out_proj_weight, conv_out, delta, A, A_b, Bm,
     Cm, D, delta_bias, out_pre, out_pre_b, out_z, ck_f, ck_b, x_proj_wt, delta_proj_wt) = ctx.saved_tensors
    Bsz, two_e, L = xz.shape
    E = two_e // 2
    R = delta_proj_weight.shape[1]
    N = A.shape[-1]
    x, z = xz[:, :E], xz[:, E:]
    dxz = torch.empty_like(xz)
    dx, dz = dxz[:, :E], dxz[:, E:]
    dout_proj_weight = dout_proj_bias = None
    if ctx.has_out_proj:
        dout_z, dout_proj_weight, dout_proj_bias = _out_proj_bwd(ctx, dout, out_proj_weight, None, _dm2d(out_z), None, None)
        dout_z = dout_z.reshape(E, Bsz, L).permute(1, 0, 2)
    else:
        dout_z = dout if dout.stride(-1) == 1 else dout.contiguous()
        dout_z = dout_z.to(xz.dtype)
    drop = _REF_DZ_DROP and A_b is not None
    if A_b is None or ctx.bidir_fused:
        g = aum_hip.scan_bwd(conv_out, delta, A, Bm, Cm, D, z, delta_bias, dout_z, out_pre, ctx.delta_softplus,
                             ctx.reverse if A_b is None else False, A_b=A_b, dz_out=dz, dmajor=True, x_ck=ck_f)
    else:
        g = aum_hip.scan_bwd(conv_out, delta, A, Bm, Cm, D, z, delta_bias, dout_z, out_pre, ctx.delta_softplus, False,
                             dz_out=dz, dmajor=True, x_ck=ck_f)
        acc = not drop and aum_hip.scan_accumulates(conv_out, A.shape[1])
        gb = aum_hip.scan_bwd(conv_out, delta, A_b, Bm, Cm, D, z, delta_bias, dout_z, out_pre_b, ctx.delta_softplus,
                              True, dmajor=True, x_ck=ck_b, accumulate_into=g if acc else None)
        if not acc:
            for k in ("du", "ddelta", "dB", "dC", "dD", "ddelta_bias"):
                g[k] = g[k] + gb[k]
            if not drop:
                dz.add_(gb["dz"])
        g["dA_b"] = gb["dA"]
    if drop and ctx.bidir_fused:
        gf = aum_hip.scan_bwd(conv_out, delta, A, Bm, Cm, D, z, delta_bias, dout_z,
                              aum_hip.scan_fwd(conv_out, delta, A, Bm, Cm, D, z, delta_bias, ctx.delta_softplus, False,
                                               want_out_pre=True, dmajor=True)[1],
                              ctx.delta_softplus, False, dz_out=dz, dmajor=True)
        del gf
    dconv_out, ddelta = g["du"], g["ddelta"]
    dB_proj_bias = dC_proj_bias = None
    ddelta2, dconv2 = _dm2d(ddelta), _dm2d(dconv_out)
    if ctx.proj_kernels:
        dx_dbl = aum_hip.proj_bwd_data(ddelta2, delta_proj_wt, x_proj_wt, g["dB"], g["dC"], dconv2, L)
        ddelta_proj_weight = aum_hip.proj_bwd_weight(ddelta2, x_dbl[:R], False)
        dx_proj_weight = aum_hip.proj_bwd_weight(_dm2d(conv_out), dx_dbl, True)
    else:
        dx_dbl = torch.empty_like(x_dbl)
        dx_dbl3 = dx_dbl.view(Bsz, L, -1)
        dx_dbl3[:, :, R:R + N].copy_(g["dB"].transpose(1, 2))
        dx_dbl3[:, :, R + N:R + 2 * N].copy_(g["dC"].transpose(1, 2))
        dB_proj_bias = g["dB"].sum((0, 2)) if not ctx.B_proj_bias_is_None else None
        dC_proj_bias = g["dC"].sum((0, 2)) if not ctx.C_proj_bias_is_None else None
        ddelta_proj_weight = torch.matmul(ddelta2, x_dbl[:, :R])
        dx_dbl[:, :R] = torch.matmul(ddelta2.t(), delta_proj_weight.to(ddelta2.dtype))
        dx_proj_weight = torch.matmul(dx_dbl.t(), _dm2d(conv_out).t())
        dconv2.addmm_(x_proj_weight.t().to(dx_dbl.dtype), dx_dbl.t())
    _, dconv_w, dconv_b = aum_hip.conv1d_bwd(x, conv_w, conv1d_bias, dconv_out, True, ctx.reverse, dx_out=dx)
    return dict(dxz=dxz, dconv_w=dconv_w.reshape(E, 1, -1), dconv_b=dconv_b, dx_proj_w=dx_proj_weight,
                ddt_proj_w=ddelta_proj_weight, dout_proj_w=dout_proj_weight, dout_proj_b=dout_proj_bias,
                dA=g["dA"], dA_b=g.get("dA_b"), dD=g["dD"], ddelta_bias=g["ddelta_bias"],
                dB_proj_bias=dB_proj_bias, dC_proj_bias=dC_proj_bias)


def _check_variable_bc(B, C):
    if B is not None or C is not None:
        raise NotImplementedError("the fused HIP path implements input-dependent B and C (B=None, C=None), "
                                  "the only form mamba_simple.Mamba passes (MS:208-209)")


class MambaInnerFnNoOutProj(torch.autograd.Function):

    @staticmethod
    @_custom_fwd
    def forward(ctx, xz, conv1d_weight, conv1d_bias, x_proj_weight, delta_proj_weight, A, B=None, C=None, D=None,
                delta_bias=None, B_proj_bias=None, C_proj_bias=None, delta_softplus=True, checkpoint_lvl=1,
                reverse=False):
        _check_variable_bc(B, C)
        return _inner_forward(ctx, xz, conv1d_weight, conv1d_bias, x_proj_weight, delta_proj_weight, None, None, A,
                              None, D, delta_bias, B_proj_bias, C_proj_bias, delta_softplus, reverse)

    @staticmethod
    @_custom_bwd
    def backward(ctx, dout):
        g = _inner_backward(ctx, dout)
        return (g["dxz"], g["dconv_w"], g["dconv_b"], g["dx_proj_w"], g["ddt_proj_w"], g["dA"], None, None, g["dD"],
                g["ddelta_bias"], g["dB_proj_bias"], g["dC_proj_bias"], None, None, None)


class MambaInnerFn(torch.autograd.Function):

    @staticmethod
    @_custom_fwd
    def forward(ctx, xz, conv1d_weight, conv1d_bias, x_proj_weight, delta_proj_weight, out_proj_weight, out_proj_bias,
                A, B=None, C=None, D=None, delta_bias=None, B_proj_bias=None, C_proj_bias=None, delta_softplus=True,
                checkpoint_lvl=1, reverse=False):
        _check_variable_bc(B, C)
        return _inner_forward(ctx, xz, conv1d_weight, conv1d_bias, x_proj_weight, delta_proj_weight, out_proj_weight,
                              out_proj_bias, A, None, D, delta_bias, B_proj_bias, C_proj_bias, delta_softplus, reverse)

    @staticmethod
    @_custom_bwd
    def backward(ctx, dout):
        g = _inner_backward(ctx, dout)
        return (g["dxz"], g["dconv_w"], g["dconv_b"], g["dx_proj_w"], g["ddt_proj_w"], g["dout_proj_w"],
                g["dout_proj_b"], g["dA"], None, None, g["dD"], g["ddelta_bias"], g["dB_proj_bias"],
                g["dC_proj_bias"], None, None, None)


class BiMambaInnerFn(torch.autograd.Function):

    @staticmethod
    @_custom_fwd
    def forward(ctx, xz, conv1d_weight, conv1d_bias, x_proj_weight, delta_proj_weight, out_proj_weight, out_proj_bias,
                A, A_b, B=None, C=None, D=None, delta_bias=None, B_proj_bias=None, C_proj_bias=None,
                delta_softplus=True, checkpoint_lvl=1, reverse=False):
        _check_variable_bc(B, C)
        ctx.swapped = bool(reverse)
        if reverse:
            A, A_b = A_b, A
        return _inner_forward(ctx, xz, conv1d_weight, conv1d_bias, x_proj_weight, delta_proj_weight, out_proj_weight,
                              out_proj_bias, A, A_b, D, delta_bias, B_proj_bias, C_proj_bias, delta_softplus, bool(reverse))

    @staticmethod
    @_custom_bwd
    def backward(ctx, dout):
        g = _inner_backward(ctx, dout)
        dA, dA_b = (g["dA_b"], g["dA"]) if ctx.swapped else (g["dA"], g["dA_b"])
        return (g["dxz"], g["dconv_w"], g["dconv_b"], g["dx_proj_w"], g["ddt_proj_w"], g["dout_proj_w"],
                g["dout_proj_b"], dA, dA_b, None, None, g["dD"], g["ddelta_bias"], g["dB_proj_bias"],
                g["dC_proj_bias"], None, None, None)


def mamba_inner_fn(xz, conv1d_weight, conv1d_bias, x_proj_weight, delta_proj_weight, out_proj_weight, out_proj_bias,
                   A, B=None, C=None, D=None, delta_bias=None, B_proj_bias=None, C_proj_bias=None,
                   delta_softplus=True, reverse=False):
    return MambaInnerFn.apply(xz, conv1d_weight, conv1d_bias, x_proj_weight, delta_proj_weight, out_proj_weight,
                              out_proj_bias, A, B, C, D, delta_bias, B_proj_bias, C_proj_bias, delta_softplus, 1, reverse)


def bimamba_inner_fn(xz, conv1d_weight, conv1d_bias, x_proj_weight, delta_proj_weight, out_proj_weight, out_proj_bias,
                     A, A_b, B=None, C=None, D=None, delta_bias=None, B_proj_bias=None, C_proj_bias=None,
                     delta_softplus=True, reverse=False):
    return BiMambaInnerFn.apply(xz, conv1d_weight, conv1d_bias, x_proj_weight, delta_proj_weight, out_proj_weight,
                                out_proj_bias, A, A_b, B, C, D, delta_bias, B_proj_bias, C_proj_bias, delta_softplus, 1, reverse)


def mamba_inner_fn_no_out_proj(xz, conv1d_weight, conv1d_bias, x_proj_weight, delta_proj_weight, A, B=None, C=None,
                               D=None, delta_bias=None, B_proj_bias=None, C_proj_bias=None, delta_softplus=True,
                               reverse=False):
    return MambaInnerFnNoOutProj.apply(xz, conv1d_weight, conv1d_bias, x_proj_weight, delta_proj_weight, A, B, C, D,
                                       delta_bias, B_proj_bias, C_proj_bias, delta_softplus, 1, reverse)


def _conv_ref(x, weight, bias):
    w = weight.reshape(weight.shape[0], -1)
    y = F.conv1d(x, w[:, None, :], bias, padding=w.shape[1] - 1, groups=x.shape[1])[..., :x.shape[-1]]
    return F.silu(y)


def _inner_pre_ref(xz, conv1d_weight, conv1d_bias, x_proj_weight, delta_proj_weight, N, B_proj_bias, C_proj_bias):
    Bsz, two_e, L = xz.shape
    E = two_e // 2
    R = delta_proj_weight.shape[1]
    x, z = xz[:, :E], xz[:, E:]
    xc = _conv_ref(x, conv1d_weight, conv1d_bias)
    proj = xc.transpose(1, 2).reshape(Bsz * L, E) @ x_proj_weight.t()
    delta = (proj[:, :R] @ delta_proj_weight.t()).reshape(Bsz, L, E).transpose(1, 2)
    Bm, Cm = proj[:, R:R + N], proj[:, R + N:R + 2 * N]
    if B_proj_bias is not None:
        Bm = Bm + B_proj_bias.to(Bm.dtype)
    if C_proj_bias is not None:
        Cm = Cm + C_proj_bias.to(Cm.dtype)
    Bm = Bm.reshape(Bsz, L, N).transpose(1, 2).contiguous()
    Cm = Cm.reshape(Bsz, L, N).transpose(1, 2).contiguous()
    return xc, z, delta, Bm, Cm


def mamba_inner_ref(xz, conv1d_weight, conv1d_bias, x_proj_weight, delta_proj_weight, out_proj_weight, out_proj_bias,
                    A, B=None, C=None, D=None, delta_bias=None, B_proj_bias=None, C_proj_bias=None,
                    delta_softplus=True):
    xc, z, delta, Bm, Cm = _inner_pre_ref(xz, conv1d_weight, conv1d_bias, x_proj_weight, delta_proj_weight,
                                          A.shape[-1], B_proj_bias, C_proj_bias)
    y = selective_scan_ref(xc, delta, A, Bm if B is None else B, Cm if C is None else C, D, z=z,
                           delta_bias=delta_bias, delta_softplus=True)
    return F.linear(y.transpose(1, 2), out_proj_weight, out_proj_bias)


def bimamba_inner_ref(xz, conv1d_weight, conv1d_bias, x_proj_weight, delta_proj_weight, out_proj_weight,
                      out_proj_bias, A, A_b, B=None, C=None, D=None, delta_bias=None, B_proj_bias=None,
                      C_proj_bias=None, delta_softplus=True):
    xc, z, delta, Bm, Cm = _inner_pre_ref(xz, conv1d_weight, conv1d_bias, x_proj_weight, delta_proj_weight,
                                          A.shape[-1], B_proj_bias, C_proj_bias)
    Bm = Bm if B is None else B
    Cm = Cm if C is None else C
    y = selective_scan_ref(xc, delta, A, Bm, Cm, D, z=z, delta_bias=delta_bias, delta_softplus=True)
    fl = lambda t: t.flip([-1])
    y_b = selective_scan_ref(fl(xc), fl(delta), A_b, fl(Bm), fl(Cm), D, fl(z), delta_bias, delta_softplus=True)
    return F.linear((y + fl(y_b)).transpose(1, 2), out_proj_weight, out_proj_bias)


def selective_scan_update(state, u, delta, A, B, C, D=None, z=None, delta_bias=None, delta_softplus=False, delta_activated=False, *, seq_map=None):
    if seq_map is not None:
        if u.dim() != 3 or u.shape[0] != 1 or state.dim() != 3:
            raise ValueError("selective_scan_update: with seq_map the operands are (1, total, .) and state the pool (nrows, dim, dstate)")
        aum_hip.check_seq_map("selective_scan_update", seq_map, u.shape[1], state.shape[0], u.device)
    dty = u.dtype
    delta, B, C = delta.to(dty), B.to(dty), C.to(dty)
    z = None if z is None else z.to(dty)
    if u.dim() != 3 or delta.shape != u.shape or B.dim() != 3 or B.shape != C.shape or B.shape[:2] != u.shape[:2] or (z is not None and z.shape != u.shape):
        raise RuntimeError("selective_scan_update: u, delta, z (batch, seqlen, dim); B, C (batch, seqlen, dstate)")
    return aum_hip.scan_stream(state, u, delta, A, B, C, D, z, delta_bias, delta_softplus, delta_activated, seq_map)
```

### include/aum_hip.h

```cpp
#ifndef AUM_HIP_H
#define AUM_HIP_H

#include <stdint.h>

#ifdef __cplusplus
extern "C" {
#endif

#define AUM_ABI_VERSION 13

enum { AUM_F32 = 0, AUM_BF16 = 1, AUM_F16 = 2 };

enum {
    AUM_OK = 0,
    AUM_E_NULL = -1,
    AUM_E_SHAPE = -2,
    AUM_E_DTYPE = -3,
    AUM_E_UNSUPPORTED = -4,
    AUM_E_WORKSPACE = -5,
    AUM_E_LAUNCH = -6
};

#define AUM_SCAN_SOFTPLUS 1u
#define AUM_SCAN_REVERSE 2u
// ... 2 lines not shown
#define AUM_SCAN_ACCUMULATE 16u
#define AUM_SCAN_DELTA_ACTIVATED 32u
#define AUM_CONV_SILU 1u
#define AUM_CONV_REVERSE 2u
#define AUM_CONV_GENERIC 4u
#define AUM_GEMM_LOCKSTEP 1u
#define AUM_GEMM_PIPELINED 32u
#define AUM_GEMM_PACED 256u
#define AUM_NORM_PRENORM 1u
#define AUM_NORM_GENERIC 2u

typedef struct AumScanFwdArgs {
    const void *u, *delta, *z, *B, *C;
    const float *A, *A_b, *D, *delta_bias;
    void *out, *out_pre;
    float *last_state;
    void *workspace;
    int64_t workspace_bytes;
    int64_t u_bs, u_ds;
    int64_t delta_bs, delta_ds;
    int64_t z_bs, z_ds;
    int64_t B_bs, B_ns;
    int64_t C_bs, C_ns;
    int64_t out_bs, out_ds;
    int32_t batch, dim, len, dstate;
    int32_t dtype;
    uint32_t flags;
    float *x_ck;
    float *x_lane;
} AumScanFwdArgs;

typedef struct AumScanBwdArgs {
    const void *u, *delta, *z, *B, *C, *dout, *out_pre;
    const float *A, *A_b, *D, *delta_bias;
    void *du, *ddelta, *dz;
    float *dA, *dA_b, *dB, *dC, *dD, *ddelta_bias;
    void *workspace;
    int64_t workspace_bytes;
    int64_t u_bs, u_ds, delta_bs, delta_ds, z_bs, z_ds, B_bs, B_ns, C_bs, C_ns;
    int64_t dout_bs, dout_ds, out_bs, out_ds;
    int64_t du_bs, du_ds, ddelta_bs, ddelta_ds, dz_bs, dz_ds;
    int64_t dB_bs, dB_ns, dC_bs, dC_ns;
    int32_t batch, dim, len, dstate;
    int32_t dtype;
    uint32_t flags;
    const float *x_ck;
    const float *x_lane;
} AumScanBwdArgs;

int aum_selective_scan_fwd(const AumScanFwdArgs* args, void* stream);
int aum_selective_scan_bwd(const AumScanBwdArgs* args, void* stream);
int aum_scan_max_single_pass_len(void);
int64_t aum_selective_scan_workspace_bytes(int32_t batch, int32_t dim, int32_t len, int32_t dstate, int32_t bidirectional,
                                           int32_t backward);
int64_t aum_selective_scan_ckpt_bytes(int32_t batch, int32_t dim, int32_t len, int32_t dstate);
int64_t aum_selective_scan_lane_ckpt_bytes(int32_t batch, int32_t dim, int32_t len, int32_t dstate, int32_t bidirectional);

typedef struct AumConvArgs {
    const void *x, *dy;
    const float *weight, *bias;
    void *y;
    void *dx;
    float *dweight, *dbias;
    int64_t x_bs, x_ds, y_bs, y_ds, dy_bs, dy_ds, dx_bs, dx_ds;
    int32_t batch, dim, len, width;
    int32_t dtype;
    uint32_t flags;
} AumConvArgs;

int aum_causal_conv1d_fwd(const AumConvArgs* args, void* stream);
int aum_causal_conv1d_bwd(const AumConvArgs* args, void* stream);

typedef struct AumNormArgs {
    const void *x, *residual, *dy, *dresidual_out;
    const float *weight, *rstd_in;
    void *y, *residual_out, *dx, *dresidual_in;
    float *rstd_out, *dweight_partial;
    int64_t row_stride_x, row_stride_res, row_stride_y, row_stride_res_out;
    int64_t row_stride_dy, row_stride_dres_out, row_stride_dx, row_stride_dres_in;
    float eps;
    int32_t rows, cols;
    int32_t x_dtype, res_dtype, y_dtype;
    uint32_t flags;
} AumNormArgs;

int aum_rmsnorm_fwd(const AumNormArgs* args, void* stream);
int aum_rmsnorm_bwd(const AumNormArgs* args, void* stream);
int aum_rmsnorm_bwd_partials(int32_t rows);
int aum_rmsnorm_bwd_partial_rows(int32_t rows, int32_t cols, uint32_t flags);

typedef struct AumFbankArgs {
    const float *wave, *window, *twiddle, *mel_start_f, *mel_count_f, *mel_w;
    float *out;
    int64_t wave_bs, out_bs;
    int32_t batch, n_samples, win, shift, padded, num_frames, target_length, num_mel, mel_wstride;
    float preemph, norm_mean, norm_inv2std, log_floor;
    const float *aug, *noise;
} AumFbankArgs;
#define AUM_FBANK_AUG 8
int aum_fbank_fwd(const AumFbankArgs* args, void* stream);

typedef struct AumFrontendArgs {
    AumFbankArgs fbank;
    const void *weight;
    const float *bias, *pos, *cls_row;
    void *tokens, *patches;
    int64_t tokens_bs;
    int32_t dim, cls_pos, dtype, out_dtype;
    uint32_t flags;
} AumFrontendArgs;
#define AUM_FRONTEND_TIME_MAJOR 1u
int aum_frontend_tokens_fwd(const AumFrontendArgs* args, void* stream);

typedef struct AumFbankStreamArgs {
    AumFbankArgs fbank;
    const int32_t *cu_samples, *cu_frames, *tail_len, *idx, *first_frame, *n_real;
    float *tails;
    int32_t total_samples, total_frames, nseq, nrows, cap, reserved;
} AumFbankStreamArgs;
int aum_fbank_stream_fwd(const AumFbankStreamArgs* args, void* stream);

typedef struct AumProjArgs {
    const void *act, *w_x, *w_dt;
    void *x_dbl, *out_act;
    const float *dB, *dC;
    int64_t dB_bs, dB_ns, dC_bs, dC_ns;
    int64_t ntok;
    int32_t dim, dt_rank, dstate, len, dtype;
    int32_t w_ld;
} AumProjArgs;
int aum_proj_fwd(const AumProjArgs* args, void* stream);
int aum_proj_bwd_data(const AumProjArgs* args, void* stream);
typedef struct AumProjWArgs {
    const void *x, *y;
    float* out;
    int64_t ntok;
    int32_t dim, nrows, nsplit, transpose_out, dtype;
} AumProjWArgs;
int aum_proj_bwd_weight(const AumProjWArgs* args, void* stream);
int aum_proj_bwd_weight_splits(int32_t dim, int64_t ntok);

#define AUM_SCAN_TM_CK 8
typedef struct AumScanTmFwdArgs {
    const void *u, *delta, *z, *B, *C;
    const float *A, *A_b, *D, *delta_bias;
    void *out, *out_pre;
    float *ckpt;
    int64_t u_bs, u_ts, delta_bs, delta_ts, z_bs, z_ts, B_bs, B_ts, C_bs, C_ts, out_bs, out_ts, pre_bs, pre_ts;
    int32_t batch, dim, len, dstate;
    int32_t dtype;
    uint32_t flags;
} AumScanTmFwdArgs;
int aum_scan_tm_fwd(const AumScanTmFwdArgs* args, void* stream);
int32_t aum_scan_tm_nck(int32_t len);
int32_t aum_scan_tm_ckpt_rows(int32_t dtype);

typedef struct AumScanTmBwdArgs {
    const void *u, *delta, *z, *B, *C, *dout, *out_pre;
    const float *A, *A_b, *D, *delta_bias;
    const float *ckpt;
    void *du, *ddelta, *dz;
    float *dA, *dA_b, *dBC, *dD, *ddelta_bias;
    void *workspace;
    int64_t workspace_bytes;
    int64_t u_bs, u_ts, delta_bs, delta_ts, z_bs, z_ts, B_bs, B_ts, C_bs, C_ts, dout_bs, dout_ts, pre_bs, pre_ts;
    int64_t du_bs, du_ts, ddelta_bs, ddelta_ts, dz_bs, dz_ts;
    int32_t batch, dim, len, dstate;
    int32_t dtype;
    uint32_t flags;
    float *dA_xA, *dA_b_xA;
} AumScanTmBwdArgs;
int aum_scan_tm_bwd(const AumScanTmBwdArgs* args, void* stream);
int64_t aum_scan_tm_workspace_bytes(int32_t batch, int32_t dim, int32_t len, int32_t dstate, int32_t bidirectional);

#define AUM_SCAN_TM_MAX_SEGMENTS 32
typedef struct AumScanTmSegFwdArgs {
    AumScanTmFwdArgs base;
    float* carry;
    int64_t carry_bytes;
    int32_t segments;
    int32_t reserved;
} AumScanTmSegFwdArgs;
typedef struct AumScanTmSegBwdArgs {
    AumScanTmBwdArgs base;
    int32_t segments;
    int32_t reserved;
} AumScanTmSegBwdArgs;
int aum_scan_tm_seg_fwd(const AumScanTmSegFwdArgs* args, void* stream);
int aum_scan_tm_seg_bwd(const AumScanTmSegBwdArgs* args, void* stream);
int64_t aum_scan_tm_seg_carry_bytes(int32_t batch, int32_t dim, int32_t len, int32_t dstate, int32_t bidirectional, int32_t segments);
int64_t aum_scan_tm_seg_workspace_bytes(int32_t batch, int32_t dim, int32_t len, int32_t dstate, int32_t bidirectional, int32_t segments);

typedef struct AumScanTmFwdStateArgs {
    AumScanTmFwdArgs base;
    const float* state_in;
    float* state_out;
    float* carry;
    int64_t carry_bytes;
    int32_t segments;
    int32_t reserved;
} AumScanTmFwdStateArgs;
int aum_scan_tm_fwd_state(const AumScanTmFwdStateArgs* args, void* stream);

typedef struct AumConvTmArgs {
    const void *x, *dy;
    const float *weight, *bias;
    void *y;
    void *dx;
    float *dw_part, *db_part;
    int64_t x_bs, x_ts, y_bs, y_ts, dy_bs, dy_ts, dx_bs, dx_ts;
    int32_t batch, dim, len, width;
    int32_t dtype;
    uint32_t flags;
} AumConvTmArgs;
int aum_conv1d_tm_fwd(const AumConvTmArgs* args, void* stream);
int aum_conv1d_tm_bwd(const AumConvTmArgs* args, void* stream);
int32_t aum_conv1d_tm_nparts(int32_t batch, int32_t len);

typedef struct AumGemmArgs {
    const void *a, *b;
    void *c;
    int32_t m, n, k;
    int32_t lda, ldb, ldc;
    int32_t dtype;
    uint32_t flags;
} AumGemmArgs;
int aum_gemm_tn(const AumGemmArgs* args, void* stream);

typedef struct AumGemmWArgs {
    const void *y, *x;
    float* part;
    int64_t t;
    int64_t ldy, ldx;
    int32_t n, k, splits;
    int32_t dtype;
} AumGemmWArgs;
int aum_gemm_wgrad(const AumGemmWArgs* args, void* stream);

typedef struct AumDtProjArgs {
    const void *x, *w;
    void *out;
    int64_t ntok;
    int32_t dim, rank;
    int32_t ldx, ldw, ldo;
    int32_t dtype;
} AumDtProjArgs;
int aum_dtproj_tm_fwd(const AumDtProjArgs* args, void* stream);

typedef struct AumXdtArgs {
    const void *u, *wx, *wdt;
    void *x_dbl, *delta;
    int64_t ntok;
    int32_t dim, rank, ncols;
    int32_t ldu, ldwx, ldwdt, ldx, ldd;
    int32_t dtype;
    const float* delta_bias;
    uint32_t flags;
} AumXdtArgs;
#define AUM_XDT_DELTA_SOFTPLUS 1u
int aum_xdt_tm_fwd(const AumXdtArgs* args, void* stream);

typedef struct AumXdtBwdArgs {
    const void *ddelta;
    const float *dbc;
    const void *wdt_t, *wx_t;
    void *du, *dx_dbl;
    int64_t ntok;
    int32_t dim, rank, ncols;
    int32_t ldd, lddbc, ldwdt, ldwx, ldu, ldx;
    int32_t dtype;
} AumXdtBwdArgs;
int aum_xdt_tm_bwd(const AumXdtBwdArgs* args, void* stream);

typedef struct AumConvUpdateArgs {
    const void* x;
    float* conv_state;
    const float *weight, *bias;
    void* out;
    int32_t batch, dim, width;
    int32_t dtype;
    uint32_t flags;
} AumConvUpdateArgs;
int aum_causal_conv1d_update(const AumConvUpdateArgs* args, void* stream);
typedef struct AumStateUpdateArgs {
    float* state;
    const void *x, *dt, *z, *B, *C;
    const float *A, *D, *dt_bias;
    void* out;
    int32_t batch, dim, dstate;
    int32_t dtype;
    uint32_t flags;
} AumStateUpdateArgs;
int aum_selective_state_update(const AumStateUpdateArgs* args, void* stream);

typedef struct AumConvTmChunkArgs {
    const void* x;
    float* conv_state;
    const float *weight, *bias;
    void* y;
    int64_t x_bs, x_ts, y_bs, y_ts;
    int32_t batch, dim, len, width;
    int32_t dtype;
    uint32_t flags;
} AumConvTmChunkArgs;
int aum_conv1d_tm_chunk(const AumConvTmChunkArgs* args, void* stream);
typedef struct AumScanTmChunkArgs {
// ... 231 lines not shown
```

Measured before the change: 1103 clips/s.

## Compute only the middle cls-token row in the last Mamba block

Only the middle cls-token row is read after the final layer. The last Fo-Bi block now runs a dedicated path that computes the z gate and out_proj for that row alone, with a one-row scan kernel for inference. In training, the full scan still runs, but out_proj and the z projection are limited to one row, which cuts GEMM work in the last layer. The change adds a large custom autograd function and kernel variant, with some risk to correctness in the backward zero-padding of dout.

```diff
diff --git a/audio-mamba-aum_amd/aum/model.py b/audio-mamba-aum_amd/aum/model.py
--- a/audio-mamba-aum_amd/aum/model.py
+++ b/audio-mamba-aum_amd/aum/model.py
@@ -82,9 +82,11 @@
         self.mixer = mixer
         self.norm = RMSNorm(dim, eps=eps)
 
-    def forward(self, hidden_states, residual=None, inference_params=None, *, time_reversed=False):
+    def forward(self, hidden_states, residual=None, inference_params=None, *, time_reversed=False, only_row=None):
         hidden_states, residual = rms_norm_fn(hidden_states, self.norm.weight, self.norm.bias, residual=residual,
                                               prenorm=True, residual_in_fp32=True, eps=self.norm.eps)
+        if only_row is not None and inference_params is None and not time_reversed and self.mixer.takes_only_row(hidden_states, only_row):
+            return self.mixer(hidden_states, only_row=only_row), residual
         if time_reversed:
             return self.mixer(hidden_states, inference_params=inference_params, time_reversed=True), residual
         return self.mixer(hidden_states, inference_params=inference_params), residual
@@ -258,15 +260,16 @@
     def forward_features(self, x, frontend=None):
         hidden, pos = self.tokens(x) if frontend is None else self.tokens_from_wave(x, frontend)
         with step_cache([layer.mixer for layer in self.layers], _autocast_dtype()):
-            hidden, residual = self._run_layers(hidden)
-        return rms_norm_fn(hidden[:, pos], self.norm_f.weight, self.norm_f.bias, eps=self.norm_f.eps,
+            hidden, residual = self._run_layers(hidden, only_row=pos if self.use_middle_cls_token and not self.use_end_cls_token else None)
+        one_row = residual is not None and hidden.shape[1] != residual.shape[1]
+        return rms_norm_fn(hidden[:, 0 if one_row else pos], self.norm_f.weight, self.norm_f.bias, eps=self.norm_f.eps,
                            residual=None if residual is None else residual[:, pos], prenorm=False, residual_in_fp32=True)
 
-    def _run_layers(self, hidden):
+    def _run_layers(self, hidden, only_row=None):
         residual = None
         if not self.if_bidirectional:
-            for layer in self.layers:
-                hidden, residual = layer(hidden, residual)
+            for i, layer in enumerate(self.layers):
+                hidden, residual = layer(hidden, residual, only_row=only_row if i + 1 == len(self.layers) else None)
         else:
             for i in range(len(self.layers) // 2):
                 hf, rf = self.layers[2 * i](hidden, residual)
diff --git a/audio-mamba-aum_amd/aum_hip/__init__.py b/audio-mamba-aum_amd/aum_hip/__init__.py
--- a/audio-mamba-aum_amd/aum_hip/__init__.py
+++ b/audio-mamba-aum_amd/aum_hip/__init__.py
@@ -321,6 +321,7 @@
     "aum_scan_tm_peeks_ckpt_bytes": ([_i32] * 4, _i64), "aum_scan_tm_peeks_bwd_workspace_bytes": ([_i32] * 4, _i64),
     "aum_conv1d_tm_peeks_bwd_workspace_bytes": ([_i32] * 3, _i64),
     "aum_stream_layers_scratch_bytes": ([_i32] * 4, _i64),
+    "aum_scan_tm_fwd_row": ([_vp, _i32, _vp], C.c_int),
 })
 EXPORTS = list(_SIGNATURES)
 
@@ -680,6 +681,74 @@
     _launch(lib.c.aum_scan_tm_fwd, a, u, lib, "scan_tm_fwd_bidir" if A_b is not None else "scan_tm_fwd",
             (batch, dim, length, dstate, u.element_size(), want_out_pre))
     return out, out_pre
+
+
+def scan_tm_fwd_row_supported(u, delta, A, B, C, z, A_b, row, delta_activated):
+    if A_b is None or z is None or not delta_activated or u.dim() != 3 or u.dtype not in (torch.bfloat16, torch.float16):
+        return False
+    batch, length, dim = u.shape
+    dstate, es = A.shape[1], 2
+    if not scan_tm_supported(dim, dstate) or row != length // 2 or tuple(z.shape) != (batch, 1, dim) or z.dtype != u.dtype or z.stride(2) != 1:
+        return False
+    if z.data_ptr() % 16 or (batch > 1 and (z.stride(0) * es) % 16):
+        return False
+    for t, last in ((u, dim), (delta, dim), (B, dstate), (C, dstate)):
+        if t.dtype != u.dtype or tuple(t.shape) != (batch, length, last) or t.stride(2) != 1:
+            return False
+        bs, ts = _tm3(t, "operand", last)
+        if last == dim and (t.data_ptr() % 16 or (ts * es) % 16 or (bs * es) % 16):
+            return False
+        if last == dstate and (t.data_ptr() % 4 or ts % 2 or bs % 2):
+            return False
+        if ts < 0 or ts * es * length >= 2 ** 31:
+            return False
+    return True
+
+
+def scan_tm_fwd_row(u, delta, A, B, C, D, z_row, A_b, row, want_out_pre=False, ckpt=None, out=None, out_pre=None, lib=None):
+    lib = lib or get()
+    batch, length, dim = u.shape
+    dstate = A.shape[1]
+    for t in (u, delta, z_row, B, C, out, out_pre, ckpt):
+        lib.check_tensor(t)
+    if not scan_tm_fwd_row_supported(u, delta, A, B, C, z_row, A_b, row, True):
+        raise RuntimeError(f"scan_tm_fwd_row: unsupported operands u {tuple(u.shape)} {u.dtype}, z_row {None if z_row is None else tuple(z_row.shape)}, "
+                           f"row {row} (need the Fo-Bi block's 16-bit token-major operands, z one row per clip, row == len // 2)")
+    A, A_b, D = _f32c(A), _f32c(A_b), _f32c(D)
+    a = ScanTmFwdArgs()
+    a.u_bs, a.u_ts = _tm3(u, "u", dim)
+    a.delta_bs, a.delta_ts = _tm3(delta, "delta", dim)
+    a.B_bs, a.B_ts = _tm3(B, "B", dstate)
+    a.C_bs, a.C_ts = _tm3(C, "C", dstate)
+    a.z_bs, a.z_ts = (z_row.stride(0) if batch > 1 else dim), 0
+    rows = []
+    for name, t, want in (("out", out, True), ("out_pre", out_pre, want_out_pre)):
+        if not want:
+            rows.append((None, 0, 0))
+        elif t is None:
+            t = torch.empty((batch, 1, dim), dtype=u.dtype, device=u.device)
+            rows.append((t, dim, 0))
+        else:
+            if tuple(t.shape) != (batch, length, dim) or t.dtype != u.dtype:
+                raise RuntimeError(f"scan_tm_fwd_row: {name} must be (batch, len, dim) in u's dtype")
+            bs, ts = _tm3(t, name, dim)
+            rows.append((t[:, row:row + 1], bs, ts))
+    (o, a.out_bs, a.out_ts), (pre, a.pre_bs, a.pre_ts) = rows
+    a.u, a.delta, a.B, a.C = _ptr(u), _ptr(delta), _ptr(B), _ptr(C)
+    a.A, a.A_b, a.D = _ptr(A), _ptr(A_b), _ptr(D)
+    a.z = _ptr(z_row)
+    a.out = _ptr(o) - row * a.out_ts * u.element_size()
+    a.out_pre = None if pre is None else _ptr(pre) - row * a.pre_ts * u.element_size()
+    if ckpt is not None:
+        assert ckpt.dtype == torch.float32 and ckpt.is_contiguous()
+        nrows = int(lib.c.aum_scan_tm_ckpt_rows(_DT[u.dtype]))
+        assert ckpt.numel() >= 2 * batch * max(int(lib.c.aum_scan_tm_nck(length)), 1) * nrows * dim, "ckpt too small"
+        a.ckpt = _ptr(ckpt)
+    a.batch, a.dim, a.len, a.dstate, a.dtype = batch, dim, length, dstate, _DT[u.dtype]
+    a.flags = SCAN_DELTA_ACTIVATED
+    _launch(lambda args, stream: lib.c.aum_scan_tm_fwd_row(args, int(row), stream), a, u, lib, "scan_tm_fwd_row",
+            (batch, dim, length, dstate, u.element_size(), want_out_pre))
+    return o, pre
 
 
 def scan_state_supported(t, batch, dim, dstate):
diff --git a/audio-mamba-aum_amd/csrc/aum_api_tm.inc b/audio-mamba-aum_amd/csrc/aum_api_tm.inc
--- a/audio-mamba-aum_amd/csrc/aum_api_tm.inc
+++ b/audio-mamba-aum_amd/csrc/aum_api_tm.inc
@@ -17,6 +17,9 @@
 int scan_tm_bwd_f32(const AumScanTmBwdArgs& a, const ScanTBwdOut& wo, aum_stream_t s);
 int scan_tm_bwd_bf16(const AumScanTmBwdArgs& a, const ScanTBwdOut& wo, aum_stream_t s);
 int scan_tm_bwd_f16(const AumScanTmBwdArgs& a, const ScanTBwdOut& wo, aum_stream_t s);
+int scan_tm_fwd_row_f32(const AumScanTmFwdArgs& a, aum_stream_t s);
+int scan_tm_fwd_row_bf16(const AumScanTmFwdArgs& a, aum_stream_t s);
+int scan_tm_fwd_row_f16(const AumScanTmFwdArgs& a, aum_stream_t s);
 int scan_tm_seg_fwd_f32(const AumScanTmFwdArgs& a, const ScanTSeg& sg, int phase, aum_stream_t s);
 int scan_tm_seg_fwd_bf16(const AumScanTmFwdArgs& a, const ScanTSeg& sg, int phase, aum_stream_t s);
 int scan_tm_seg_fwd_f16(const AumScanTmFwdArgs& a, const ScanTSeg& sg, int phase, aum_stream_t s);
@@ -86,6 +89,22 @@
             return launch_scant_fwd<T, sp, hz, pre, bidir>(a, s); }); }); }); });
 }
 #ifndef AUM_EMU
+template <class T, bool HAS_PRE>
+__global__ __launch_bounds__(SCANT_NW * 64, AUM_SCANT_FWD_MINW) void k_scant_fwd_row(AumScanTmFwdArgs a) {
+    __shared__ __attribute__((aligned(16))) float lds[ScanTFwdLds<T>::n];
+    scant_fwd<T, false, true, HAS_PRE, true, true>(a, (int)blockIdx.x, lds);
+}
+#endif
+template <class T> static int scan_tm_fwd_row_t(const AumScanTmFwdArgs& a, aum_stream_t s) {
+    if constexpr (sizeof(T) == 2) {
+        constexpr int UPW = scant_units_per_wg<true>();
+        const int grid = (a.batch * (a.dim / WAVE) + UPW - 1) / UPW;
+        return with_bool(a.out_pre != nullptr, [&](auto pre) {
+            return AUM_LAUNCH(grid, SCANT_NW * 64, s, (ScanTFwdLds<T>{}), (k_scant_fwd_row<T, pre>), (scant_fwd<T, false, true, pre, true, true>(a, wg, lds)), a); });
+    }
+    return AUM_E_UNSUPPORTED;
+}
+#ifndef AUM_EMU
 template <class T, int PHASE, bool SP, bool HAS_Z, bool HAS_PRE>
 __global__ __launch_bounds__(SCANT_NW * 64, AUM_SCANT_FWD_MINW) void k_scant_seg_fwd(AumScanTmFwdArgs a, ScanTSeg sg) {
     __shared__ __attribute__((aligned(16))) float lds[ScanTFwdLds<T>::n];
@@ -168,18 +187,21 @@
 }
 #if AUM_HAS_DTYPE(0)
 int scan_tm_fwd_f32(const AumScanTmFwdArgs& a, aum_stream_t s) { return scan_tm_fwd_t<float>(a, s); }
+int scan_tm_fwd_row_f32(const AumScanTmFwdArgs& a, aum_stream_t s) { return scan_tm_fwd_row_t<float>(a, s); }
 int scan_tm_seg_fwd_f32(const AumScanTmFwdArgs& a, const ScanTSeg& sg, int phase, aum_stream_t s) { return scan_tm_seg_fwd_t<float>(a, sg, phase, s); }
 int scan_tm_fwd_state_f32(const AumScanTmFwdArgs& a, const ScanTState& st, const ScanTSeg* sg, int phase, aum_stream_t s) { return scan_tm_fwd_state_t<float>(a, st, sg, phase, s); }
 int scan_tm_fwd_state_var_f32(const AumScanTmFwdArgs& a, const ScanTVar& v, const ScanTSeg* sg, int phase, aum_stream_t s) { return scan_tm_fwd_state_var_t<float>(a, v, sg, phase, s); }
 #endif
 #if AUM_HAS_DTYPE(1)
 int scan_tm_fwd_bf16(const AumScanTmFwdArgs& a, aum_stream_t s) { return scan_tm_fwd_t<bf16_t>(a, s); }
+int scan_tm_fwd_row_bf16(const AumScanTmFwdArgs& a, aum_stream_t s) { return scan_tm_fwd_row_t<bf16_t>(a, s); }
 int scan_tm_seg_fwd_bf16(const AumScanTmFwdArgs& a, const ScanTSeg& sg, int phase, aum_stream_t s) { return scan_tm_seg_fwd_t<bf16_t>(a, sg, phase, s); }
 int scan_tm_fwd_state_bf16(const AumScanTmFwdArgs& a, const ScanTState& st, const ScanTSeg* sg, int phase, aum_stream_t s) { return scan_tm_fwd_state_t<bf16_t>(a, st, sg, phase, s); }
 int scan_tm_fwd_state_var_bf16(const AumScanTmFwdArgs& a, const ScanTVar& v, const ScanTSeg* sg, int phase, aum_stream_t s) { return scan_tm_fwd_state_var_t<bf16_t>(a, v, sg, phase, s); }
 #endif
 #if AUM_HAS_DTYPE(2)
 int scan_tm_fwd_f16(const AumScanTmFwdArgs& a, aum_stream_t s) { return scan_tm_fwd_t<f16_t>(a, s); }
+int scan_tm_fwd_row_f16(const AumScanTmFwdArgs& a, aum_stream_t s) { return scan_tm_fwd_row_t<f16_t>(a, s); }
 int scan_tm_seg_fwd_f16(const AumScanTmFwdArgs& a, const ScanTSeg& sg, int phase, aum_stream_t s) { return scan_tm_seg_fwd_t<f16_t>(a, sg, phase, s); }
 int scan_tm_fwd_state_f16(const AumScanTmFwdArgs& a, const ScanTState& st, const ScanTSeg* sg, int phase, aum_stream_t s) { return scan_tm_fwd_state_t<f16_t>(a, st, sg, phase, s); }
 int scan_tm_fwd_state_var_f16(const AumScanTmFwdArgs& a, const ScanTVar& v, const ScanTSeg* sg, int phase, aum_stream_t s) { return scan_tm_fwd_state_var_t<f16_t>(a, v, sg, phase, s); }
@@ -306,6 +328,14 @@
     aum_stream_t s = (aum_stream_t)stream;
     const AumScanTmFwdArgs k = scan_tm_fwd_resolve(*a);
     return AUM_BY_DTYPE_X(k.dtype, scan_tm_fwd, k, s);
+}
+AUM_API int aum_scan_tm_fwd_row(const AumScanTmFwdArgs* a, int32_t row, void* stream) {
+    const int rc = scan_tm_fwd_check(a);
+    if (rc != AUM_OK) return rc;
+    if (!a->A_b || !a->z || a->dtype == AUM_F32 || !(a->flags & AUM_SCAN_DELTA_ACTIVATED)) return AUM_E_UNSUPPORTED;
+    if (row != scant_first_half(a->len, 0)) return AUM_E_UNSUPPORTED;
+    const AumScanTmFwdArgs k = scan_tm_fwd_resolve(*a);
+    return AUM_BY_DTYPE_X(k.dtype, scan_tm_fwd_row, k, (aum_stream_t)stream);
 }
 static int scan_tm_seg_fwd_any(const AumScanTmFwdArgs& a, const ScanTSeg& sg, int phase, aum_stream_t s) {
     return AUM_BY_DTYPE_X(a.dtype, scan_tm_seg_fwd, a, sg, phase, s);
diff --git a/audio-mamba-aum_amd/csrc/scan_tm_kernels.h b/audio-mamba-aum_amd/csrc/scan_tm_kernels.h
--- a/audio-mamba-aum_amd/csrc/scan_tm_kernels.h
+++ b/audio-mamba-aum_amd/csrc/scan_tm_kernels.h
@@ -35,7 +35,7 @@
 template <class T> struct ScanTStage { vq q[ScanTTile<T>::NLD]; };
 struct ScanTRaw { vi u, d, z, part; };
 
-template <class T, int N, int PHASE, bool SP, bool HAS_Z, bool HAS_PRE>
+template <class T, int N, int PHASE, bool SP, bool HAS_Z, bool HAS_PRE, bool ROW = false>
 AUM_DEV void scant_fwd_run(const AumScanTmFwdArgs& p, int b, int e0, int dir, int t0, int tstep, int it0, int it1, const float* Aptr,
                            float dmul, vf2 (&x)[N / 2], float* lds, unsigned long long* scant_trace_acc = nullptr, vf2* pacc = nullptr) {
     using TL = ScanTTile<T>;
@@ -130,7 +130,9 @@
     auto flush = [&](int blk) {
         if ((AUM_SCANT_ABL & 4) || CARRY) return;
         const int base = blk * SCANT_CK;
-        const bool inside = base >= it0 && base + SCANT_CK <= it1;
+        constexpr bool ROW1 = ROW && PHASE == 1;
+        if (ROW1 && (tstep > 0 || base + SCANT_CK < it1)) return;
+        const bool inside = !ROW1 && base >= it0 && base + SCANT_CK <= it1;
         wave_lds_fence();
         vi rowt;
         int t_lo = 0;
@@ -140,7 +142,7 @@
             rowt = st_r;
         } else {
             const vi it = st_i + base;
-            valid = (it >= it0) && (it < it1);
+            valid = (it >= (ROW1 ? it1 - 1 : it0)) && (it < it1);
             rowt = vmax_i(vmin_i(it, it1 - 1), it0) * tstep + t0;
         }
         AUM_UNROLL
@@ -465,8 +467,9 @@
 template <bool BIDIR> AUM_HOSTDEV constexpr int scant_units_per_wg() { return BIDIR ? SCANT_NW / 2 : SCANT_NW; }
 template <bool BIDIR> AUM_HOSTDEV constexpr int scant_bwd_wgs(int units) { return BIDIR ? (units + 2) / 3 : (units + SCANT_NW - 1) / SCANT_NW; }
 
-template <class T, bool SP, bool HAS_Z, bool HAS_PRE, bool BIDIR>
+template <class T, bool SP, bool HAS_Z, bool HAS_PRE, bool BIDIR, bool ROW = false>
 AUM_DEV void scant_fwd(const AumScanTmFwdArgs& p, int wg, float* lds, unsigned long long* tacc = nullptr) {
+    static_assert(BIDIR || !ROW, "the one-row mode is the Fo-Bi pair's");
     constexpr int N = SCANT_N;
     constexpr int NW = SCANT_NW;
     constexpr int UPW = scant_units_per_wg<BIDIR>();
@@ -492,16 +495,17 @@
         if (unit < units) {
             AUM_UNROLL
             for (int j = 0; j < N / 2; ++j) x[AUM_W(w)][j] = spl2(splat(0.f));
-            scant_fwd_run<T, N, 1, SP, HAS_Z, HAS_PRE>(p, unit / gpb, (unit % gpb) * WAVE, d, d ? L - 1 + io : -io, d ? -1 : 1, io, scant_first_half(L, d) + io,
-                                                       d ? p.A_b : p.A, 2.f, x[AUM_W(w)], lds + w * scant_lds_wave_floats<T>(), tacc);
+            scant_fwd_run<T, N, 1, SP, HAS_Z, HAS_PRE, ROW>(p, unit / gpb, (unit % gpb) * WAVE, d, d ? L - 1 + io : -io, d ? -1 : 1, io, scant_first_half(L, d) + io,
+                                                            d ? p.A_b : p.A, 2.f, x[AUM_W(w)], lds + w * scant_lds_wave_floats<T>(), tacc);
         }
     }
     AUM_WG_BARRIER();
     AUM_FOR_EACH_WAVE(w, NW) {
         const int unit = wg * UPW + (w >> 1), d = w & 1, io = scant_grid_shift(L, d);
-        if (unit < units)
-            scant_fwd_run<T, N, 2, SP, HAS_Z, HAS_PRE>(p, unit / gpb, (unit % gpb) * WAVE, d, d ? L - 1 + io : -io, d ? -1 : 1, scant_first_half(L, d) + io, L + io,
-                                                       d ? p.A_b : p.A, 2.f, x[AUM_W(w)], lds + w * scant_lds_wave_floats<T>(), tacc);
+        const int fh = scant_first_half(L, d) + io;
+        if (unit < units && !(ROW && d))
+            scant_fwd_run<T, N, 2, SP, HAS_Z, HAS_PRE, ROW>(p, unit / gpb, (unit % gpb) * WAVE, d, d ? L - 1 + io : -io, d ? -1 : 1, fh, ROW ? fh + 1 : L + io,
+                                                            d ? p.A_b : p.A, 2.f, x[AUM_W(w)], lds + w * scant_lds_wave_floats<T>(), tacc);
     }
 }
 
diff --git a/audio-mamba-aum_amd/mamba_ssm/modules/mamba_simple.py b/audio-mamba-aum_amd/mamba_ssm/modules/mamba_simple.py
--- a/audio-mamba-aum_amd/mamba_ssm/modules/mamba_simple.py
+++ b/audio-mamba-aum_amd/mamba_ssm/modules/mamba_simple.py
@@ -75,7 +75,14 @@
         p._no_weight_decay = True
         return p
 
-    def forward(self, hidden_states, inference_params=None, *, time_reversed=False, peek_every=None):
+    def takes_only_row(self, hidden_states, row):
+        return (self.bimamba_type == "v1" and self.use_fast_path and isinstance(row, int)
+                and ssi.last_block_row_ok(hidden_states, row, self.d_inner, self.d_state, self.d_conv, self.dt_rank,
+                                          self.in_proj.bias is not None))
+
+    def forward(self, hidden_states, inference_params=None, *, time_reversed=False, peek_every=None, only_row=None):
+        if only_row is not None and (inference_params is not None or time_reversed or peek_every is not None):
+            raise ValueError("forward(only_row=) takes none of inference_params, time_reversed, peek_every")
         if peek_every is not None:
             if inference_params is not None or time_reversed:
                 raise ValueError("forward(peek_every=) takes neither inference_params nor time_reversed")
@@ -99,6 +106,11 @@
                 out, _, _ = self.prefill_chunk(hidden_states, conv_state, ssm_state)
                 return out if self.init_layer_scale is None else out * self.gamma
         batch, seqlen, _ = hidden_states.shape
+        if only_row is not None:
+            out = ssi.bimamba_inner_row_fn(hidden_states, int(only_row), self.in_proj.weight, self.conv1d.weight, self.conv1d.bias,
+                                           self.x_proj.weight, self.dt_proj.weight, self.out_proj.weight, self.out_proj.bias,
+                                           neg_exp(self.A_log), neg_exp(self.A_b_log), self.D.float(), self.dt_proj.bias.float())
+            return out if self.init_layer_scale is None else out * self.gamma
         tm = (ssi.TOKEN_MAJOR and self.use_fast_path and inference_params is None
               and not (ssi._REF_DZ_DROP and self.bimamba_type == "v1")
               and ssi.token_major_preferred(batch, self.d_inner, self.bimamba_type != "none", seqlen=seqlen)
diff --git a/audio-mamba-aum_amd/mamba_ssm/ops/selective_scan_interface.py b/audio-mamba-aum_amd/mamba_ssm/ops/selective_scan_interface.py
--- a/audio-mamba-aum_amd/mamba_ssm/ops/selective_scan_interface.py
+++ b/audio-mamba-aum_amd/mamba_ssm/ops/selective_scan_interface.py
@@ -1006,6 +1006,142 @@
                 g["dC_proj_bias"], None, None, None)
 
 
+_LAST_BLOCK_ROW = _dbg_env("AUM_LAST_BLOCK_CLS", "1") != "0"
+
+
+def last_block_row_ok(hidden, row, d_inner, d_state, d_conv, dt_rank, has_bias):
+    act = _autocast_dtype()
+    if not (_LAST_BLOCK_ROW and TOKEN_MAJOR and not _REF_DZ_DROP and not has_bias and hidden.dim() == 3 and hidden.is_cuda
+            and act in (torch.bfloat16, torch.float16)):
+        return False
+    Bsz, L, _ = hidden.shape
+    return (row == L // 2 and token_major_ok(d_inner, d_state, d_conv, dt_rank, act) and d_inner % 8 == 0
+            and _tm_fills_chip(Bsz, d_inner, True, torch.is_grad_enabled()))
+
+
+class BiMambaInnerRowFn(torch.autograd.Function):
+
+    @staticmethod
+    @_custom_fwd
+    def forward(ctx, hidden, row, in_proj_weight, conv1d_weight, conv1d_bias, x_proj_weight, delta_proj_weight, out_proj_weight,
+                out_proj_bias, A, A_b, D, delta_bias):
+        act = _autocast_dtype()
+        need_bwd = any(ctx.needs_input_grad)
+        Bsz, L, Dm = hidden.shape
+        w_in = _cast(in_proj_weight, act)
+        E, R, N = w_in.shape[0] // 2, delta_proj_weight.shape[1], A.shape[-1]
+        h = hidden.to(w_in.dtype)
+        h = h if h.is_contiguous() else h.contiguous()
+        h2, h_r = h.view(Bsz * L, Dm), h[:, row]
+        w_x, w_dt = _cast(x_proj_weight, act), _cast(delta_proj_weight, act)
+        w_out, b_out = _cast(out_proj_weight, act), _cast(out_proj_bias, act)
+        x = _proj_fwd(h2, w_in[:E], _IN_PROJ).view(Bsz, L, E)
+        z_r = torch.matmul(h_r, w_in[E:].t()).view(Bsz, 1, E)
+        conv_w = conv1d_weight.reshape(E, -1)
+        conv_out = aum_hip.conv1d_tm_fwd(x, conv_w, conv1d_bias, True, False)
+        conv2d = conv_out.view(Bsz * L, E)
+        x_dbl, delta, act_delta = _xdt_fwd(conv2d, w_x.to(conv2d.dtype), w_dt.to(conv2d.dtype), R, delta_bias, True)
+        x3 = x_dbl.view(Bsz, L, R + 2 * N)
+        Bm, Cm, delta3 = x3[:, :, R:R + N], x3[:, :, R + N:], delta.view(Bsz, L, E)
+        out_pre = ckpt = None
+        if not need_bwd and aum_hip.scan_tm_fwd_row_supported(conv_out, delta3, A, Bm, Cm, z_r, A_b, row, act_delta):
+            out_r, _ = aum_hip.scan_tm_fwd_row(conv_out, delta3, A, Bm, Cm, D, z_r, A_b, row)
+        else:
+            ckpt = aum_hip.scan_tm_ckpt(Bsz, L, E, N, True, hidden.device, dtype=conv_out.dtype) if need_bwd else None
+            out_z, out_pre = aum_hip.scan_tm_fwd(conv_out, delta3, A, Bm, Cm, D, z_r.expand(Bsz, L, E), delta_bias, True, False, A_b=A_b,
+                                                 want_out_pre=need_bwd, ckpt=ckpt, delta_activated=act_delta)
+            out_r = out_z[:, row:row + 1].contiguous()
+            del out_z
+        out = _proj_fwd(out_r.view(Bsz, E), w_out.to(out_r.dtype), _OUT_PROJ)
+        if b_out is not None:
+            out = out + b_out
+        if need_bwd:
+            w_x_t = w_dt_t = None
+            if _XDT_BWD_HIP and aum_hip.xdt_tm_bwd_widths(E, R, N, conv2d.dtype):
+                w_x_t, w_dt_t = _cast_t(x_proj_weight, conv2d.dtype), _cast_t(delta_proj_weight, conv2d.dtype)
+            ctx.row, ctx.act_delta, ctx.has_out_bias = row, act_delta, b_out is not None
+            w_out_t = _weight_t_for_dgrad(out_proj_weight, w_out.to(out_r.dtype), True)
+            w_in_t = _weight_t_for_dgrad(in_proj_weight, w_in, True) if ctx.needs_input_grad[0] else None
+            ctx.wdtypes = (in_proj_weight.dtype, out_proj_weight.dtype, hidden.dtype)
+            ctx.A_cached = (A.dtype == torch.float32 and A.is_contiguous() and A.data_ptr() in _A_CACHE_PTRS
+                            and A_b.is_contiguous() and A_b.data_ptr() in _A_CACHE_PTRS)
+            ctx.params = dict(in_proj=in_proj_weight, conv_w=conv1d_weight, conv_b=conv1d_bias, x_proj=x_proj_weight, dt_proj=delta_proj_weight,
+                              out_proj=out_proj_weight, D=D, dt_bias=delta_bias, A_log=_A_OWNER.get(A.data_ptr()), A_b_log=_A_OWNER.get(A_b.data_ptr()))
+            ctx.save_for_backward(h, w_in, x, z_r, conv_w, conv1d_bias, x_dbl, w_x, w_dt, w_out, conv_out, delta, A, A_b, D, delta_bias, out_pre,
+                                  out_r, ckpt, w_x_t, w_dt_t, w_out_t, w_in_t)
+        return out.view(Bsz, 1, -1)
+
+    @staticmethod
+    @_custom_bwd
+    def backward(ctx, dout):
+        (h, w_in, x, z_r, conv_w, conv1d_bias, x_dbl, w_x, w_dt, w_out, conv_out, delta, A, A_b, D, delta_bias, out_pre, out_r, ckpt, w_x_t,
+         w_dt_t, w_out_t, w_in_t) = ctx.saved_tensors
+        Bsz, L, Dm = h.shape
+        E, R, N, row = w_in.shape[0] // 2, w_dt.shape[1], A.shape[-1], ctx.row
+        in_wdtype, out_wdtype, hdtype = ctx.wdtypes
+        pend = _PendingSums()
+        H = {k: grad_home(ctx.params.get(k)) for k in _TM_HOMES + ("in_proj",)}
+        f32 = dict(dtype=torch.float32, device=h.device)
+        kernel_sums = lambda n, k: _HIP_WGRAD and _HIP_GEMM and n % 256 == 0 and (k % 256 == 0 or k in aum_hip.WGRAD_SKINNY_K)
+        if not (kernel_sums(2 * E, Dm) and in_wdtype == torch.float32):
+            H["in_proj"] = None
+        if not (kernel_sums(w_out.shape[0], E) and out_wdtype == torch.float32):
+            H["out_proj"] = None
+        dout2 = dout.reshape(Bsz, -1).to(w_out.dtype).contiguous()
+        dw_out = _sum_out_like(H["out_proj"], (w_out.shape[0], E), f32)
+        with torch.autocast(device_type="cuda", enabled=False):
+            torch.matmul(dout2.t().float(), out_r.view(Bsz, E).float(), out=dw_out)
+        db_out = dout2.sum(0) if ctx.has_out_bias else None
+        dout_z = torch.zeros((Bsz, L, E), dtype=conv_out.dtype, device=h.device)
+        dout_z[:, row] = _proj_bwd(dout2, None, w_out, w_out_t, _OUT_PROJ, None, None, want_w=False)[0]
+        x3 = x_dbl.view(Bsz, L, R + 2 * N)
+        g = aum_hip.scan_tm_bwd(conv_out, delta.view(Bsz, L, E), A, x3[:, :, R:R + N], x3[:, :, R + N:], D, z_r.expand(Bsz, L, E), delta_bias, dout_z,
+                                out_pre, ckpt, True, False, A_b=A_b, want_dA_xA=ctx.A_cached, delta_activated=ctx.act_delta,
+                                param_out=dict(dD=H["D"], ddelta_bias=H["dt_bias"], dA_xA=H["A_log"], dA_b_xA=H["A_b_log"]))
+        if ctx.A_cached:
+            _da_xa_put(g["dA"], g["dA_xA"], A)
+            _da_xa_put(g["dA_b"], g["dA_b_xA"], A_b)
+        dz_r = g["dz"][:, row]
+        _, dx_proj_w, ddt_proj_w = _xdt_bwd(g["ddelta"].view(Bsz * L, E), g["dBC"].view(Bsz * L, 2 * N), g["du"].view(Bsz * L, E), x_dbl,
+                                            conv_out.view(Bsz * L, E), w_x, w_dt, w_x_t, w_dt_t, R, pend, H["x_proj"], H["dt_proj"])
+        dx, dconv_w, dconv_b = aum_hip.conv1d_tm_bwd(x, conv_w, conv1d_bias, g["du"], True, False, partials=True)
+        home_w = None if H["conv_w"] is None else H["conv_w"].view(E, -1)
+        dconv_w, dconv_b = pend.add(dconv_w, out=home_w), (None if dconv_b is None else pend.add(dconv_b, out=H["conv_b"]))
+        dx2, h2 = dx.view(Bsz * L, E), h.view(Bsz * L, Dm)
+        dh = None
+        if ctx.needs_input_grad[0]:
+            w_in_tx = None if w_in_t is None else w_in_t[:, :E]
+            dh = _proj_bwd(dx2, None, w_in[:E], w_in_tx, _IN_PROJ, None, None, want_w=False)[0].view(Bsz, L, Dm)
+            dh[:, row] += torch.matmul(dz_r, w_in[E:])
+            dh = dh.to(hdtype)
+        dw_in = None
+        if ctx.needs_input_grad[2]:
+            dw_in = _sum_out_like(H["in_proj"], (2 * E, Dm), f32)
+            top = _wgrad_tm(dx2, h2, _WGRAD_SPLITS[0], torch.float32, pend, home=dw_in[:E])
+            with torch.autocast(device_type="cuda", enabled=False):
+                torch.matmul(dz_r.t().float(), h[:, row].float(), out=dw_in[E:])
+        sums = pend.run()
+        dx_proj_w, ddt_proj_w, dconv_w, dconv_b = (sums[v] if isinstance(v, _PendingIndex) else v for v in (dx_proj_w, ddt_proj_w, dconv_w, dconv_b))
+        if dw_in is not None:
+            top = sums[top] if isinstance(top, _PendingIndex) else top
+            if top.data_ptr() != dw_in.data_ptr():
+                dw_in[:E].copy_(top)
+            dw_in = dw_in.to(in_wdtype)
+        return (dh, None, _homed(dw_in, H["in_proj"]), _homed(dconv_w.reshape(E, 1, -1), H["conv_w"]), _homed(dconv_b, H["conv_b"]),
+                _homed(dx_proj_w, H["x_proj"]), _homed(ddt_proj_w, H["dt_proj"]), _homed(dw_out.to(out_wdtype), H["out_proj"]), db_out,
+                g["dA"], g["dA_b"], _homed(g["dD"], H["D"]), _homed(g["ddelta_bias"], H["dt_bias"]))
+
+
+def _sum_out_like(home, shape, f32):
+    return home if home is not None and tuple(home.shape) == tuple(shape) else torch.empty(shape, **f32)
+
+
+def bimamba_inner_row_fn(hidden, row, in_proj_weight, conv1d_weight, conv1d_bias, x_proj_weight, delta_proj_weight, out_proj_weight,
+                         out_proj_bias, A, A_b, D, delta_bias):
+    return BiMambaInnerRowFn.apply(hidden, row, in_proj_weight, conv1d_weight, conv1d_bias, x_proj_weight, delta_proj_weight, out_proj_weight,
+                                   out_proj_bias, A, A_b, D, delta_bias)
+
+
 def mamba_inner_fn(xz, conv1d_weight, conv1d_bias, x_proj_weight, delta_proj_weight, out_proj_weight, out_proj_bias,
                    A, B=None, C=None, D=None, delta_bias=None, B_proj_bias=None, C_proj_bias=None,
                    delta_softplus=True, reverse=False):
diff --git a/include/aum_hip.h b/include/aum_hip.h
--- a/include/aum_hip.h
+++ b/include/aum_hip.h
@@ -178,6 +178,7 @@
     uint32_t flags;
 } AumScanTmFwdArgs;
 int aum_scan_tm_fwd(const AumScanTmFwdArgs* args, void* stream);
+int aum_scan_tm_fwd_row(const AumScanTmFwdArgs* args, int32_t row, void* stream);
 int32_t aum_scan_tm_nck(int32_t len);
 int32_t aum_scan_tm_ckpt_rows(int32_t dtype);
 
```

Result: no change. 1108 clips/s (median of 6 runs) (+0.5%).
